# AdaptiveCity/deepdish

Hardware: AMD Instinct MI355X
Metric: end-to-end frames/sec (detect+encode+track) at 640x480 (higher is better)
Workload: dtype i8 (reference: uint8); encoder f16; 1 GPU; SSD-MobileNet-v1 uint8-quantised (300x300) + MARS-64x32x3 + deep_sort on synthetic 640x480 BGR frames, ~20 synthetic detections/frame (BASELINE.json configs[1]); streams_per_gpu=3072, worker_threads_per_gpu=2, parallelism=independent streams, 3072 per GPU in 2 worker groups, weights=seeded synthetic (seed 1234)

## Files before the change

### deepdish_amd/csrc/net_priv.h

```cpp
#pragma once
#include <map>
#include <utility>
#include <vector>
#include "common.h"

struct TensorDesc { int buf, h, w, c, cs, coff, dtype, pad; };

struct dd_net {
    dd_ctx *ctx = nullptr;
    int max_batch = 0;
    std::vector<int32_t> prog;
    std::vector<TensorDesc> tensors;
    std::vector<int64_t> buf_elems;
    std::vector<void *> bufs;
    std::vector<int> buf_dtype;
    int n_ops = 0, ops_off = 0;
    void *arena = nullptr;
    int64_t arena_bytes = 0;
    char *d_weights = nullptr;
    int64_t weight_bytes = 0;
    int in_h = 0, in_w = 0, out_tensor = -1;
    bool profile = false;
    int last_batch = 0;
    DevBuf slab;
    bool ssd_dec = false, yolo_dec = false;
    int dec_anchors = 0; float dec_thr = 0.f;
    float *d_anchors = nullptr, *dec_boxes = nullptr, *dec_score = nullptr, *dec_keys = nullptr; int *dec_cls = nullptr;
    bool slab_moved = false;
    _Float16 *d_zero = nullptr;
    bool use_glds = true;
    bool use_rw = true;
    int tile_mode = 0;
    std::vector<hipEvent_t> events;
    std::vector<int32_t> op_launch;
    std::vector<int32_t> op_variant;
    struct GraphEntry { int calls = 0; hipGraph_t graph = nullptr; hipGraphExec_t exec = nullptr; };
    bool use_graph = false;
    std::map<std::pair<const void *, int>, GraphEntry> graphs;
};

int netq_run_op(dd_net *net, int op_index, const int32_t *o, const uint8_t *input, int nimg, hipStream_t s, int *handled);
int netq_run_front(dd_net *net, const int32_t *o0, const int32_t *o1, const int32_t *o2, const uint8_t *input, int nimg, hipStream_t s, int *ran);
int netq_run_mid(dd_net *net, const int32_t *o3, const int32_t *o4, int nimg, hipStream_t s, int *ran);
int netq_prepare(dd_net *net);
```

### deepdish_amd/csrc/nets.hip

```cpp
#include <algorithm>
#include <cmath>
#include <cstdlib>
#include <map>
#include <string>
#include "common.h"
#include "ssd_dev.h"
#include "net_priv.h"
#include "mars_tail.h"

namespace {

typedef _Float16 h8 __attribute__((ext_vector_type(8)));
typedef _Float16 h4 __attribute__((ext_vector_type(4)));
typedef float f4 __attribute__((ext_vector_type(4)));

enum { OP_INPUT = 1, OP_CONV = 2, OP_DWCONV = 3, OP_MAXPOOL = 4, OP_UPSAMPLE = 5, OP_FC = 6, OP_L2NORM = 7, OP_STEM = 8, OP_DWPW = 9 };
enum { ACT_NONE = 0, ACT_RELU6 = 1, ACT_ELU = 2, ACT_SILU = 3, ACT_RELU = 4, ACT_SIGMOID = 5 };
enum { EPI_F16 = 0, EPI_F32 = 1, EPI_SSD_HEAD = 2, EPI_YOLO = 3 };
enum { OPK_DEFAULT = 0, OPK_FOLDED = 1, OPK_POOL_ROWS = 2, OPK_POOL_ROWS_STEM = 3, OPK_RES_UNIT = 4, OPK_SSD_FRONT = 5, OPK_C64_ROWS = 6, OPK_S2_ROWS = 7, OPK_CONV_WS = 8, OPK_WS_DW = 9, OPK_DWPW_ROWS = 10, OPK_SSD_HEAD_DEC = 11, OPK_RES_PAIR = 12, OPK_YOLO_HEAD_DEC = 13, OPK_MARS_WS = 14, OPK_FOLDED_PREV = 15, OPK_MARS_PAIR = 16, OPK_C64_STRIPS = 18, OPK_Q_FRONT = 19, OPK_Q_MID = 20, OPK_STEM_WIDE = 23 };
enum { DT_F16 = 0, DT_F32 = 1, DT_U8 = 2 };

constexpr int OP_WORDS = 48;
constexpr int TENSOR_WORDS = 8;

// ... 3972 lines not shown
                         int64_t n_weight_bytes, int max_batch, dd_net **out) {
    return net_create(ctx, program_host, n_words, weights_host, n_weight_bytes, max_batch, out, true);
}

static int net_create(dd_ctx *ctx, const int32_t *program_host, int n_words, const void *weights_host,
                      int64_t n_weight_bytes, int max_batch, dd_net **out, bool share) {
    DD_REQUIRE(ctx && program_host && weights_host && out && max_batch > 0 && n_words >= 8, DD_E_ARG,
               "dd_net_create: bad argument");
    DD_REQUIRE(program_host[0] == 0x314E4444, DD_E_ARG, "dd_net_create: bad program magic");
    const int nt = program_host[1], nb = program_host[2], no = program_host[3];
    DD_REQUIRE(n_words == 8 + nt * TENSOR_WORDS + nb * 2 + no * OP_WORDS, DD_E_ARG, "dd_net_create: program size mismatch");
    dd_net *n = new dd_net();
    struct Guard { dd_net *n; ~Guard() { if (n) (void)dd_net_destroy(n); } } guard{n};
    n->ctx = ctx;
    n->max_batch = max_batch;
    n->prog.assign(program_host, program_host + n_words);
    n->in_h = program_host[4];
    n->in_w = program_host[5];
    n->out_tensor = program_host[6];
    const int32_t *p = program_host + 8;
    for (int i = 0; i < nt; ++i, p += TENSOR_WORDS) n->tensors.push_back(TensorDesc{p[0], p[1], p[2], p[3], p[4], p[5], p[6], p[7]});
    DD_HIP(hipSetDevice(ctx->device));
    if (share) {
        const int32_t *ops = p + (size_t)nb * 2;
        std::vector<int> first(nb, -1), last(nb, -1);
        for (int t = 0; t < nt; ++t) DD_REQUIRE(n->tensors[t].buf >= 0 && n->tensors[t].buf < nb, DD_E_ARG, "dd_net_create_shared: tensor %d names buffer %d of %d", t, n->tensors[t].buf, nb);
        for (int i = 0; i < no; ++i)
            DD_REQUIRE((ops + (size_t)i * OP_WORDS)[0] < 16, DD_E_ARG, "dd_net_create_shared: uint8 programs keep one buffer per tensor (their borders are set once)");
        std::vector<int> gs(no), ge(no);
        for (int i = 0; i < no;) {
            int j = i;
            while (j + 1 < no && (ops + (size_t)j * OP_WORDS)[30] != 0) ++j;
            for (int k = i; k <= j; ++k) { gs[k] = i; ge[k] = j; }
            i = j + 1;
        }
        auto touch2 = [&](int t, int i) {
            if (t < 0 || t >= nt) return;
            const int b = n->tensors[t].buf;
            first[b] = first[b] < 0 ? gs[i] : std::min(first[b], gs[i]);
            last[b] = std::max(last[b], ge[i]);
        };
        for (int i = 0; i < no; ++i) {
            const int32_t *o = ops + (size_t)i * OP_WORDS;
            touch2(o[1], i); touch2(o[2], i); touch2(o[3], i); touch2(o[4], i);
        }
        if (n->out_tensor >= 0) last[n->tensors[n->out_tensor].buf] = no;
        std::vector<size_t> bytes(nb), off(nb, 0);
        size_t arena = 0;
        std::vector<int> order(nb);
        for (int b = 0; b < nb; ++b) { order[b] = b; bytes[b] = ((size_t)p[2 * b] * max_batch * dtype_size(p[2 * b + 1] & 0xff) + 256 + 255) & ~(size_t)255; }
        std::stable_sort(order.begin(), order.end(), [&](int a, int b) { return first[a] < first[b]; });
        std::vector<int> placed;
        for (int b : order) {
            if (first[b] < 0) { first[b] = 0; last[b] = no; }
            size_t at = 0;
            for (bool moved = true; moved;) {
                moved = false;
                for (int q : placed)
                    if (!(last[q] < first[b] || last[b] < first[q]) && at < off[q] + bytes[q] && off[q] < at + bytes[b]) { at = off[q] + bytes[q]; moved = true; }
            }
            off[b] = at;
            arena = std::max(arena, at + bytes[b]);
            placed.push_back(b);
        }
        DD_HIP(hipMalloc(&n->arena, arena));
        DD_HIP(hipMemset(n->arena, 0, arena));
        n->arena_bytes = (int64_t)arena;
        for (int i = 0; i < nb; ++i, p += 2) {
            n->buf_elems.push_back(p[0]);
            n->buf_dtype.push_back(p[1] & 0xff);
            n->bufs.push_back(static_cast<char *>(n->arena) + off[i]);
        }
    } else
    for (int i = 0; i < nb; ++i, p += 2) {
        n->buf_elems.push_back(p[0]);
        n->buf_dtype.push_back(p[1] & 0xff);
        void *d = nullptr;
        const size_t bytes = (size_t)p[0] * max_batch * dtype_size(p[1] & 0xff) + 256;
        DD_HIP(hipMalloc(&d, bytes));
        DD_HIP(hipMemset(d, (p[1] >> 8) & 0xff, bytes));
        n->bufs.push_back(d);
    }
    n->n_ops = no;
    n->ops_off = (int)(p - program_host);
    {
        size_t need = 0;
        for (int i = 0; i < no; ++i) {
            const int32_t *o = p + (size_t)i * OP_WORDS;
            if (o[0] != OP_CONV) continue;
            const int bk = o[28] == 32 ? 32 : 64, sk = conv_splitk(o[26], o[27], o[12], o[13] / bk, max_batch);
            if (sk > 1) need = std::max(need, (size_t)sk * max_batch * o[26] * o[27] * o[12] * sizeof(float));
        }
        if (need) { const int rc = n->slab.reserve(need); if (rc != DD_OK) return rc; }
    }
    n->weight_bytes = n_weight_bytes;
    DD_HIP(hipMalloc(&n->d_zero, 256));
    DD_HIP(hipMemset(n->d_zero, 0, 256));
    n->use_glds = getenv("DD_NO_GLDS") == nullptr;
    n->use_rw = getenv("DD_NO_RW") == nullptr;
    n->tile_mode = getenv("DD_TILE_MODE") ? atoi(getenv("DD_TILE_MODE")) : 0;
    DD_HIP(hipMalloc(&n->d_weights, (size_t)n_weight_bytes + 256));
    DD_HIP(hipMemcpy(n->d_weights, weights_host, (size_t)n_weight_bytes, hipMemcpyHostToDevice));
    guard.n = nullptr;
    *out = n;
    return DD_OK;
}

int dd_net_destroy(dd_net *n) {
    if (!n) return DD_OK;
    if (n->arena) (void)hipFree(n->arena);
    else for (void *b : n->bufs) (void)hipFree(b);
    for (hipEvent_t e : n->events) (void)hipEventDestroy(e);
    net_drop_graphs(n);
    n->slab.release();
    (void)hipFree(n->d_zero);
    (void)hipFree(n->d_weights);
    for (void *q : {(void *)n->d_anchors, (void *)n->dec_boxes, (void *)n->dec_score, (void *)n->dec_keys, (void *)n->dec_cls}) (void)hipFree(q);
    delete n;
    return DD_OK;
}

int dd_net_activation_bytes(dd_net *n, int64_t *out_host) {
    DD_REQUIRE(n && out_host, DD_E_ARG, "dd_net_activation_bytes: NULL argument");
    if (n->arena) { *out_host = n->arena_bytes; return DD_OK; }
    int64_t tot = 0;
    for (size_t i = 0; i < n->bufs.size(); ++i) tot += n->buf_elems[i] * n->max_batch * (int64_t)dtype_size(n->buf_dtype[i]) + 256;
    *out_host = tot;
    return DD_OK;
}

int dd_net_last_batch(dd_net *n, int *out_host) {
    DD_REQUIRE(n && out_host, DD_E_ARG, "dd_net_last_batch: NULL argument");
    *out_host = n->last_batch;
    return DD_OK;
}

int dd_net_input_size(dd_net *n, int *h_host, int *w_host) {
    DD_REQUIRE(n && h_host && w_host, DD_E_ARG, "dd_net_input_size: NULL argument");
    *h_host = n->in_h; *w_host = n->in_w;
    return DD_OK;
}

int dd_net_max_batch(dd_net *n, int *out_host) {
    DD_REQUIRE(n && out_host, DD_E_ARG, "dd_net_max_batch: NULL argument");
    *out_host = n->max_batch;
    return DD_OK;
}

int dd_net_output(dd_net *n, int tensor, void **dev_ptr, int *h, int *w, int *c, int *cs, int *dtype) {
    DD_REQUIRE(n, DD_E_ARG, "dd_net_output: NULL net");
    const int t = tensor < 0 ? n->out_tensor : tensor;
    DD_REQUIRE(t >= 0 && t < (int)n->tensors.size(), DD_E_ARG, "dd_net_output: tensor %d out of range", t);
    const TensorDesc &d = n->tensors[t];
    if (dev_ptr) *dev_ptr = static_cast<char *>(n->bufs[d.buf]) + (size_t)d.coff * dtype_size(d.dtype);
    if (h) *h = d.h;
    if (w) *w = d.w;
    if (c) *c = d.c;
    if (cs) *cs = d.cs;
    if (dtype) *dtype = d.dtype;
    return DD_OK;
}

int dd_net_profile(dd_net *n, int enable) {
    DD_REQUIRE(n, DD_E_ARG, "dd_net_profile: NULL net");
    DD_DEVICE(n->ctx);
    if (enable && n->events.empty()) {
        n->events.resize(n->n_ops + 2);
        for (auto &e : n->events) DD_HIP(hipEventCreate(&e));
    }
    n->profile = enable != 0;
    return DD_OK;
}

int dd_net_profile_read(dd_net *n, float *ms_host, int cap, int *n_ops_host) {
    DD_REQUIRE(n && ms_host && n_ops_host, DD_E_ARG, "dd_net_profile_read: NULL argument");
    DD_DEVICE(n->ctx);
    DD_REQUIRE(n->profile && !n->events.empty(), DD_E_STATE, "dd_net_profile_read: profiling is off");
    DD_REQUIRE(cap >= n->n_ops, DD_E_ARG, "dd_net_profile_read: cap %d < %d ops", cap, n->n_ops);
    DD_HIP(hipEventSynchronize(n->events[n->n_ops + 1]));
    float empty = 0.f;
    DD_HIP(hipEventElapsedTime(&empty, n->events[n->n_ops], n->events[n->n_ops + 1]));
    for (int i = 0; i < n->n_ops; ++i) {
        DD_HIP(hipEventElapsedTime(&ms_host[i], n->events[i], n->events[i + 1]));
        ms_host[i] = ms_host[i] > empty ? ms_host[i] - empty : 0.f;
    }
    *n_ops_host = n->n_ops;
    return DD_OK;
}

int dd_net_op_launches(dd_net *n, int32_t *codes_host, int cap, int *n_ops_host) {
    DD_REQUIRE(n && codes_host && n_ops_host, DD_E_ARG, "dd_net_op_launches: NULL argument");
    DD_REQUIRE(cap >= n->n_ops, DD_E_ARG, "dd_net_op_launches: cap %d < %d ops", cap, n->n_ops);
    for (int i = 0; i < n->n_ops; ++i) codes_host[i] = i < (int)n->op_launch.size() ? n->op_launch[i] : OPK_DEFAULT;
    *n_ops_host = n->n_ops;
    return DD_OK;
}

int dd_net_op_variants(dd_net *n, int32_t *codes_host, int cap, int *n_ops_host) {
    DD_REQUIRE(n && codes_host && n_ops_host, DD_E_ARG, "dd_net_op_variants: NULL argument");
    DD_REQUIRE(cap >= n->n_ops, DD_E_ARG, "dd_net_op_variants: cap %d < %d ops", cap, n->n_ops);
    for (int i = 0; i < n->n_ops; ++i) codes_host[i] = i < (int)n->op_variant.size() ? n->op_variant[i] : 0;
    *n_ops_host = n->n_ops;
    return DD_OK;
}

int dd_net_read(dd_net *n, int tensor, int n_img, void *dst, int dst_on_device, void *stream) {
    DD_REQUIRE(n && dst && n_img >= 0 && n_img <= n->max_batch, DD_E_ARG, "dd_net_read: bad argument");
    DD_DEVICE(n->ctx);
    const int t = tensor < 0 ? n->out_tensor : tensor;
    DD_REQUIRE(t >= 0 && t < (int)n->tensors.size(), DD_E_ARG, "dd_net_read: tensor %d out of range", t);
    const TensorDesc &d = n->tensors[t];
    DD_REQUIRE(!n->arena || t == n->out_tensor, DD_E_STATE, "dd_net_read: tensor %d of an engine whose buffers share memory by lifetime "
               "(dd_net_create_shared): only the output tensor outlives the forward", t);
    DD_REQUIRE(d.coff == 0, DD_E_ARG, "dd_net_read: tensor %d is a channel slice", t);
    for (int i = 0; i < n->n_ops && i < (int)n->op_launch.size(); ++i) {
        const int32_t *o = n->prog.data() + n->ops_off + (size_t)i * OP_WORDS;
        DD_REQUIRE(!(o[2] == t && n->op_launch[i] == OPK_SSD_HEAD_DEC), DD_E_STATE,
                   "dd_net_read: tensor %d (the SSD head matrix) was not written: the head layers decoded in their epilogue "
                   "(dd_net_ssd_decode); read dd_net_ssd_decoded instead", t);
        DD_REQUIRE(!(o[2] == t && n->op_launch[i] == OPK_YOLO_HEAD_DEC), DD_E_STATE,
                   "dd_net_read: tensor %d (the Detect matrix) was not written: the head layers reduced their rows in their epilogue "
                   "(dd_net_yolo_decode); read dd_net_yolo_decoded instead", t);
        DD_REQUIRE(!((o[2] == t || o[4] == t) && n->op_launch[i] == OPK_FOLDED), DD_E_STATE,
                   "dd_net_read: tensor %d was not written by the last forward (op %d ran inside the next op's launch at this batch "
                   "size and its output stayed on chip); run a smaller batch or a program compiled without the fusion flags", t, i);
    }
    hipStream_t s = dd_pick_stream(n->ctx, stream);
    const size_t bytes = d.pad ? (size_t)n_img * (d.h + 2) * (d.w + 2) * d.cs
                               : (size_t)n_img * d.h * d.w * d.cs * dtype_size(d.dtype);
    if (!bytes) return DD_OK;
    DD_HIP(hipMemcpyAsync(dst, n->bufs[d.buf], bytes, dst_on_device ? hipMemcpyDeviceToDevice : hipMemcpyDeviceToHost, s));
    if (!dst_on_device) DD_HIP(hipStreamSynchronize(s));
    return DD_OK;
}

static int net_run_ops(dd_net *net, const uint8_t *input, int nimg, hipStream_t s);

int dd_net_use_graph(dd_net *net, int enable) {
    DD_REQUIRE(net, DD_E_ARG, "dd_net_use_graph: NULL net");
    DD_DEVICE(net->ctx);
    net->use_graph = enable != 0;
    if (!net->use_graph) net_drop_graphs(net);
    return DD_OK;
}

int dd_net_ssd_decode(dd_net *net, const float *anchors_host, int n_anchors, float score_thr, int enable) {
    DD_REQUIRE(net, DD_E_ARG, "dd_net_ssd_decode: NULL net");
    DD_DEVICE(net->ctx);
    net_drop_graphs(net);
    if (!enable) { net->ssd_dec = false; return DD_OK; }
    DD_REQUIRE(anchors_host && n_anchors > 0, DD_E_ARG, "dd_net_ssd_decode: anchors missing");
    int heads = 0;
    for (int i = 0; i < net->n_ops; ++i) {
        const int32_t *o = net->prog.data() + net->ops_off + (size_t)i * OP_WORDS;
        if (o[0] == OP_CONV && o[15] == EPI_SSD_HEAD) {
            DD_REQUIRE(o[18] && o[21] == n_anchors && 4 + o[20] <= 96, DD_E_ARG,
                       "dd_net_ssd_decode: head op %d has no per-anchor weight copy, or %d anchors / %d classes do not fit", i, o[21], o[20]);
            ++heads;
        }
        if (o[0] == 20) {
            DD_REQUIRE(o[21] == n_anchors, DD_E_ARG, "dd_net_ssd_decode: the program decodes %d anchors, %d given", o[21], n_anchors);
            ++heads;
        }
    }
    DD_REQUIRE(heads > 0, DD_E_ARG, "dd_net_ssd_decode: the program has no SSD head");
    if (net->dec_anchors != n_anchors) {
        for (void *q : {(void *)net->d_anchors, (void *)net->dec_boxes, (void *)net->dec_score, (void *)net->dec_keys, (void *)net->dec_cls}) (void)hipFree(q);
        net->d_anchors = net->dec_boxes = net->dec_score = net->dec_keys = nullptr; net->dec_cls = nullptr; net->dec_anchors = 0;
        const size_t per = (size_t)net->max_batch * n_anchors;
        DD_HIP(hipMalloc(&net->d_anchors, (size_t)n_anchors * 4 * sizeof(float)));
        DD_HIP(hipMalloc(&net->dec_boxes, per * 4 * sizeof(float)));
        DD_HIP(hipMalloc(&net->dec_score, per * sizeof(float)));
        DD_HIP(hipMalloc(&net->dec_keys, per * sizeof(float)));
        DD_HIP(hipMalloc(&net->dec_cls, per * sizeof(int)));
        net->dec_anchors = n_anchors;
    }
    DD_HIP(hipMemcpy(net->d_anchors, anchors_host, (size_t)n_anchors * 4 * sizeof(float), hipMemcpyHostToDevice));
    net->dec_thr = score_thr;
    net->ssd_dec = true;
    return DD_OK;
}

int dd_net_yolo_decode(dd_net *net, int enable) {
    DD_REQUIRE(net, DD_E_ARG, "dd_net_yolo_decode: NULL net");
    DD_DEVICE(net->ctx);
    net_drop_graphs(net);
    if (!enable) { net->yolo_dec = false; return DD_OK; }
    DD_REQUIRE(!net->ssd_dec, DD_E_STATE, "dd_net_yolo_decode: the SSD decode is on for this network");
    int heads = 0, rows = 0;
    for (int i = 0; i < net->n_ops; ++i) {
        const int32_t *o = net->prog.data() + net->ops_off + (size_t)i * OP_WORDS;
        if (o[0] == OP_CONV && o[15] == EPI_YOLO) {
            DD_REQUIRE(o[18] && !o[19] && o[20] >= 6 && o[20] <= 96, DD_E_ARG,
                       "dd_net_yolo_decode: head op %d has no per-anchor weight copy, or %d columns per row do not fit", i, o[20]);
            DD_REQUIRE(rows == 0 || rows == o[21], DD_E_ARG, "dd_net_yolo_decode: heads disagree on the rows per image");
            rows = o[21];
            ++heads;
        }
    }
    DD_REQUIRE(heads > 0 && rows > 0, DD_E_ARG, "dd_net_yolo_decode: the program has no YOLOv5 Detect head");
    if (net->dec_anchors != rows || !net->dec_boxes) {
        for (void *q : {(void *)net->d_anchors, (void *)net->dec_boxes, (void *)net->dec_score, (void *)net->dec_keys, (void *)net->dec_cls}) (void)hipFree(q);
        net->d_anchors = net->dec_boxes = net->dec_score = net->dec_keys = nullptr; net->dec_cls = nullptr; net->dec_anchors = 0;
        const size_t per = (size_t)net->max_batch * rows;
        DD_HIP(hipMalloc(&net->dec_boxes, per * 4 * sizeof(float)));
        DD_HIP(hipMalloc(&net->dec_score, per * sizeof(float)));
        DD_HIP(hipMalloc(&net->dec_cls, per * sizeof(int)));
        net->dec_anchors = rows;
    }
    net->yolo_dec = true;
    return DD_OK;
}

int dd_net_yolo_decoded(dd_net *net, float **boxes, float **conf, int **classes, int *rows) {
    DD_REQUIRE(net && net->yolo_dec, DD_E_STATE, "dd_net_yolo_decoded: dd_net_yolo_decode is off");
    if (boxes) *boxes = net->dec_boxes;
    if (conf) *conf = net->dec_score;
    if (classes) *classes = net->dec_cls;
    if (rows) *rows = net->dec_anchors;
    return DD_OK;
}

int dd_net_yolo_decoded_read(dd_net *net, int n, float *boxes_host, float *conf_host, int *classes_host) {
    DD_REQUIRE(net && net->yolo_dec && n >= 0 && n <= net->max_batch, DD_E_STATE, "dd_net_yolo_decoded_read: decode is off or n out of range");
    DD_DEVICE(net->ctx);
    DD_HIP(hipStreamSynchronize(net->ctx->stream));
    const size_t per = (size_t)n * net->dec_anchors;
    if (boxes_host) DD_HIP(hipMemcpy(boxes_host, net->dec_boxes, per * 4 * sizeof(float), hipMemcpyDeviceToHost));
    if (conf_host) DD_HIP(hipMemcpy(conf_host, net->dec_score, per * sizeof(float), hipMemcpyDeviceToHost));
    if (classes_host) DD_HIP(hipMemcpy(classes_host, net->dec_cls, per * sizeof(int), hipMemcpyDeviceToHost));
    return DD_OK;
}


int dd_net_ssd_decoded(dd_net *net, float **boxes, float **scores, int **classes, float **keys) {
    DD_REQUIRE(net && net->ssd_dec, DD_E_STATE, "dd_net_ssd_decoded: dd_net_ssd_decode is off");
    if (boxes) *boxes = net->dec_boxes;
    if (scores) *scores = net->dec_score;
    if (classes) *classes = net->dec_cls;
    if (keys) *keys = net->dec_keys;
    return DD_OK;
}

int dd_net_ssd_heads_u8(dd_net *net, const uint8_t **box_q, const uint8_t **cls_q, int *cls_stride, const uint8_t **lut, float *quant4_host,
                        int *n_anchors, int *n_classes) {
    DD_REQUIRE(net && box_q && cls_q && cls_stride && lut && quant4_host && n_anchors && n_classes, DD_E_ARG, "dd_net_ssd_heads_u8: NULL argument");
    DD_REQUIRE(!net->arena, DD_E_STATE, "dd_net_ssd_heads_u8: the engine's buffers share memory by lifetime (dd_net_create_shared): the head "
               "tensors do not outlive the forward");
    for (int i = 0; i < net->n_ops; ++i) {
        const int32_t *o = net->prog.data() + net->ops_off + (size_t)i * OP_WORDS;
        if (o[0] != 20) continue;
        DD_REQUIRE(o[1] >= 0 && o[1] < (int)net->tensors.size() && o[3] >= 0 && o[3] < (int)net->tensors.size(), DD_E_ARG, "dd_net_ssd_heads_u8: head tensors out of range");
        const TensorDesc &tb = net->tensors[o[1]], &tc = net->tensors[o[3]];
        DD_REQUIRE(tb.cs == 4 && tb.h == o[21] && tc.h == o[21] && tb.w == 1 && tc.w == 1 && o[20] <= tc.cs && !tb.pad && !tc.pad && !tb.coff && !tc.coff, DD_E_ARG,
                   "dd_net_ssd_heads_u8: head tensors of %d anchors are not [anchors][4] / [anchors][>= %d] bytes", o[21], o[20]);
        *box_q = static_cast<const uint8_t *>(net->bufs[tb.buf]); *cls_q = static_cast<const uint8_t *>(net->bufs[tc.buf]);
        *cls_stride = tc.cs; *n_anchors = o[21]; *n_classes = o[20];
        *lut = reinterpret_cast<const uint8_t *>(net->d_weights + (size_t)(uint32_t)o[16]);
        const float *of = reinterpret_cast<const float *>(o);
        for (int q = 0; q < 4; ++q) quant4_host[q] = of[32 + q];
        return DD_OK;
    }
    DD_REQUIRE(false, DD_E_ARG, "dd_net_ssd_heads_u8: the program has no uint8 SSD head");
}

int dd_net_ssd_decoded_read(dd_net *net, int n, float *boxes_host, float *scores_host, int *classes_host, float *keys_host) {
    DD_REQUIRE(net && net->ssd_dec && n >= 0 && n <= net->max_batch, DD_E_STATE, "dd_net_ssd_decoded_read: decode is off or n out of range");
    DD_DEVICE(net->ctx);
    hipStream_t s = net->ctx->stream;
    DD_HIP(hipStreamSynchronize(s));
    const size_t per = (size_t)n * net->dec_anchors;
    if (!per) return DD_OK;
    if (boxes_host) DD_HIP(hipMemcpy(boxes_host, net->dec_boxes, per * 4 * sizeof(float), hipMemcpyDeviceToHost));
    if (scores_host) DD_HIP(hipMemcpy(scores_host, net->dec_score, per * sizeof(float), hipMemcpyDeviceToHost));
    if (classes_host) DD_HIP(hipMemcpy(classes_host, net->dec_cls, per * sizeof(int), hipMemcpyDeviceToHost));
    if (keys_host) DD_HIP(hipMemcpy(keys_host, net->dec_keys, per * sizeof(float), hipMemcpyDeviceToHost));
    return DD_OK;
}

int dd_net_forward(dd_net *net, const uint8_t *input, int nimg, void *stream) {
    DD_REQUIRE(net && input && nimg >= 0, DD_E_ARG, "dd_net_forward: bad argument");
    DD_DEVICE(net->ctx);
    DD_REQUIRE(nimg <= net->max_batch, DD_E_CAPACITY, "dd_net_forward: batch %d > max_batch %d", nimg, net->max_batch);
    if (nimg == 0) return DD_OK;
    net->last_batch = nimg;
    hipStream_t s = dd_pick_stream(net->ctx, stream);
    auto eager = [&]() -> int {
        const int rc = net_run_ops(net, input, nimg, s);
        if (net->slab_moved) { net->slab_moved = false; net_drop_graphs(net); }
        return rc;
    };
    if (!net->use_graph || net->profile) return eager();
    if (net->graphs.size() > 256) net_drop_graphs(net);
    dd_net::GraphEntry &g = net->graphs[std::make_pair(static_cast<const void *>(input), nimg)];
    if (g.exec) { DD_HIP(hipGraphLaunch(g.exec, s)); return DD_OK; }
    if (g.calls++ == 0) return eager();
    DD_HIP(hipStreamBeginCapture(s, hipStreamCaptureModeThreadLocal));
    const int rc = net_run_ops(net, input, nimg, s);
    hipGraph_t graph = nullptr;
    const hipError_t e = hipStreamEndCapture(s, &graph);
    if (rc != DD_OK) { if (graph) (void)hipGraphDestroy(graph); return rc; }
    DD_HIP(e);
    g.graph = graph;
    DD_HIP(hipGraphInstantiate(&g.exec, graph, nullptr, nullptr, 0));
    DD_HIP(hipGraphLaunch(g.exec, s));
    return DD_OK;
}

static int net_run_ops(dd_net *net, const uint8_t *input, int nimg, hipStream_t s) {
    auto base = [&](int t) -> char * {
        const TensorDesc &d = net->tensors[t];
        return static_cast<char *>(net->bufs[d.buf]);
    };
    net->op_launch.assign((size_t)net->n_ops, OPK_DEFAULT);
    net->op_variant.assign((size_t)net->n_ops, 0);
    ConvP stem_p;
    bool stem_pending = false;
    bool wide_pending = false, wide_ready = false;
    bool input_pending = false;
    float input_mean = 0.f, input_scale = 1.f;
    int input_op = -1;
    ConvP unit_a;
    bool unit_pending = false;
    ConvP pw_p;
    bool pw_pending = false;
    bool proj_done = false;
    MarsPairP pair64;
    bool pair64_first = false;
    int pair_left = 0;
    ConvP pair_a, pair_b;
    bool pair_pending = false;
    int pair_op = -1;
    auto flush_pair = [&]() -> int {
        pair_pending = false;
        net->op_launch[pair_op] = OPK_RES_UNIT;
        return launch_res_unit(s, pair_a, pair_b, nimg, net->ctx->device);
    };
    auto run_ws = [&](ConvP &P) { return P.cin == 256 ? launch_conv_ws<4>(s, P, net->ctx->device) : launch_conv_ws<8>(s, P, net->ctx->device); };
    int first_op = 0;
    bool mid_on = false;
    {
        static const int chunk_env = getenv("DD_Q_FRONT_CHUNK") ? atoi(getenv("DD_Q_FRONT_CHUNK")) : 0;
        auto opw = [&](int k) { return net->prog.data() + net->ops_off + (size_t)k * OP_WORDS; };
        const char *front_env = getenv("DD_Q_FRONT"), *front_min_env = getenv("DD_Q_FRONT_MIN");
        const int front_min = front_min_env ? atoi(front_min_env) : 24;
        {
            const char *mid_env = getenv("DD_Q_MID");
            mid_on = !(mid_env && atoi(mid_env) == 0) && nimg >= front_min;
        }
        if (!(front_env && atoi(front_env) == 0) && chunk_env <= 0 && nimg >= front_min && net->n_ops > 3 && opw(0)[0] == 16 && opw(1)[0] == 19 && opw(2)[0] == 19) {
            if (net->profile) for (int k = 0; k < 3; ++k) DD_HIP(hipEventRecord(net->events[k], s));
            int ran = 0;
            const int rc = netq_run_front(net, opw(0), opw(1), opw(2), input, nimg, s, &ran);
            if (rc != DD_OK) return rc;
            if (ran) { first_op = 3; net->op_launch[0] = OPK_FOLDED; net->op_launch[1] = OPK_FOLDED; net->op_launch[2] = OPK_Q_FRONT; }
        }
        if (first_op == 0 && chunk_env > 0 && nimg > chunk_env && net->n_ops > 3 && opw(0)[0] == 16 && opw(1)[0] == 19 && opw(2)[0] == 19 && opw(1)[1] == opw(0)[2] && opw(2)[1] == opw(1)[2]) {
            const TensorDesc &t2 = net->tensors[opw(2)[2]];
            const size_t img_out = (size_t)(t2.h + 2) * (t2.w + 2) * t2.cs;
            void *&out_buf = net->bufs[t2.buf];
            void *const out_base = out_buf;
            if (net->profile) for (int k = 0; k < 3; ++k) DD_HIP(hipEventRecord(net->events[k], s));
            for (int c0 = 0; c0 < nimg; c0 += chunk_env) {
                const int nc = std::min(chunk_env, nimg - c0);
                out_buf = static_cast<char *>(out_base) + (size_t)c0 * img_out;
                for (int k = 0; k < 3; ++k) {
                    int handled = 0;
                    const int rc = netq_run_op(net, k, opw(k), input + (size_t)c0 * net->in_h * net->in_w * 3, nc, s, &handled);
                    if (rc != DD_OK || !handled) { out_buf = out_base; return rc != DD_OK ? rc : DD_E_ARG; }
                }
            }
            out_buf = out_base;
            first_op = 3;
        }
    }
    for (int i = first_op; i < net->n_ops; ++i) {
        if (net->profile) DD_HIP(hipEventRecord(net->events[i], s));
        const int32_t *o = net->prog.data() + net->ops_off + (size_t)i * OP_WORDS;
        const float *of = reinterpret_cast<const float *>(o);
        const int kind = o[0], src = o[1], dst = o[2], res = o[3], dst2 = o[4];
        const TensorDesc *ts = src >= 0 ? &net->tensors[src] : nullptr;
        const TensorDesc *td = dst >= 0 ? &net->tensors[dst] : nullptr;
        DD_REQUIRE(!input_pending || (kind == OP_CONV && i == input_op + 1), DD_E_STATE, "dd_net_forward: input op %d was folded into an op that did not take it", input_op);
        if (mid_on && kind == 19 && i + 1 < net->n_ops && net->prog[net->ops_off + (size_t)(i + 1) * OP_WORDS] == 19) {
            const int32_t *o4 = net->prog.data() + net->ops_off + (size_t)(i + 1) * OP_WORDS;
            if (net->profile) DD_HIP(hipEventRecord(net->events[i + 1], s));
            int ran = 0;
            const int rc = netq_run_mid(net, o, o4, nimg, s, &ran);
            if (rc != DD_OK) return rc;
            if (ran) { net->op_launch[i] = OPK_FOLDED; net->op_launch[i + 1] = OPK_Q_MID; ++i; continue; }
        }
        DD_REQUIRE((!wide_pending || kind == OP_CONV) && (!wide_ready || kind == OP_MAXPOOL), DD_E_STATE, "dd_net_forward: op %d does not take the first layer folded into it", i);
        if (pair_pending && kind != OP_CONV) { const int rc = flush_pair(); if (rc != DD_OK) return rc; }
        if (pw_pending && kind != OP_DWCONV) {
            pw_pending = false; net->op_launch[i - 1] = OPK_CONV_WS;
            const int rc = run_ws(pw_p);
            if (rc != DD_OK) return rc;
        }
        if (unit_pending && kind != OP_CONV) {
            unit_pending = false; net->op_launch[i - 1] = OPK_DEFAULT;
            const int rc = launch_conv3x3_rw(s, unit_a, nimg, false, net->ctx->device);
            if (rc != DD_OK) return rc;
        }
        if (stem_pending && !(kind == OP_CONV && o[29]) && kind != OP_DWPW) {
            stem_pending = false; net->op_launch[i - 1] = OPK_DEFAULT;
            const int rc = launch_stem(s, stem_p, nimg);
            if (rc != DD_OK) return rc;
        }
        switch (kind) {
            case OP_INPUT: {
                const int s2d = o[5];
                const int m = nimg * td->h * td->w;
                if (s2d && o[30] && !o[6] && td->cs == 32 && !td->coff && i + 1 < net->n_ops && net->use_rw) {
// ... 403 lines not shown
```

### deepdish_amd/csrc/netsq.hip

```cpp
#include <algorithm>
#include <atomic>
#include <cstdlib>
#include <type_traits>
#include "common.h"
#include "ssd_dev.h"
#include "net_priv.h"
#include "netsq_dev.h"

namespace {


struct QConvP {
    const uint8_t *in; int H, W, c16_in;
    int kh, kw, stride, off_y, off_x;
    int ho, wo, m;
    const i4v *w;
    const int *cbias;
    int kc_per_tap, n_mfrag, mq;
    uint8_t *out; int epi;
    int Ho, Wo, c16_out;
    long long img_bytes_out; int row_bytes, base_off, cout_store;
    int zwc;
    unsigned hw_magic, wo_magic;
    QReq R;
// ... 264 lines not shown
        if (__builtin_amdgcn_ballot_w64(col < 0 || col + 2 >= P.W) != 0ull) {
#pragma unroll
            for (int i = 0; i < 3; ++i) {
                const bool in = col + i >= 0 && col + i < P.W;
                if (!in) {
#pragma unroll
                    for (int b = 3 * i; b < 3 * i + 3; ++b) {
                        const unsigned msk = 0xffu << (8 * (b & 3));
                        d[b >> 2] = (d[b >> 2] & ~msk) | (zp4 & msk);
                    }
                }
            }
        }
        i4v b;
        b[0] = (int)(d[0] ^ 0x80808080u); b[1] = (int)(d[1] ^ 0x80808080u); b[2] = (int)(d[2] ^ 0x80808080u); b[3] = 0;
        int rs = 0;
        if constexpr (!HL) {
            if (fq == 3) { b[0] = 0; b[1] = 0; b[2] = 0; }
            rs = sdot4(b[0], 0x01010101, sdot4(b[1], 0x01010101, sdot4(b[2] & 0xff, 0x01010101, 0)));
            rs += __shfl_xor(rs, 16, 64);
            rs += __shfl_xor(rs, 32, 64);
            rs *= P.zwc;
        }
        i4v acc0 = {0, 0, 0, 0}, acc1 = acc0;
        acc0 = __builtin_amdgcn_mfma_i32_16x16x64_i8(wa, b, acc0, 0, 0, 0);
        acc1 = __builtin_amdgcn_mfma_i32_16x16x64_i8(wb, b, acc1, 0, 0, 0);
        if constexpr (HL) {
            acc0 = __builtin_amdgcn_mfma_i32_16x16x64_i8(wal, b, acc0, 0, 0, 0);
            acc1 = __builtin_amdgcn_mfma_i32_16x16x64_i8(wbl, b, acc1, 0, 0, 0);
        }
        const unsigned lo = q_requant_pack4<SAT>(acc0[0] + rs, acc0[1] + rs, acc0[2] + rs, acc0[3] + rs, M0, CQ[0], CQ[1], CQ[2], CQ[3], sh0, lo0, hi0);
        const unsigned hi = q_requant_pack4<SAT>(acc1[0] + rs, acc1[1] + rs, acc1[2] + rs, acc1[3] + rs, M0, CQ[4], CQ[5], CQ[6], CQ[7], sh0, lo0, hi0);
        typedef unsigned u2v __attribute__((ext_vector_type(2)));
        __builtin_amdgcn_raw_buffer_store_b64(u2v{lo ^ 0x80808080u, hi ^ 0x80808080u}, rdst, (int)so[j], 0, 0);
    }
}

struct QDwP {
    const uint8_t *in; int H, W, c16;
    int stride, off_y, off_x, ho, wo;
    const short *w;
    const int *cbias;
    uint8_t *out;
    long long total;
    QReq R;
};

__global__ __launch_bounds__(256) void q_dw_k(const QDwP P) {
    const long long it = (long long)blockIdx.x * 256 + threadIdx.x;
    if (it >= P.total) return;
    const int x = (int)(it % P.wo);
    long long t = it / P.wo;
    const int pl = (int)(t % P.c16); t /= P.c16;
    const int y = (int)(t % P.ho), n = (int)(t / P.ho);
    const size_t PP = (size_t)(P.W + 2) * 16, RP = PP * P.c16;
    const uint8_t *src = P.in + ((size_t)n * (P.H + 2) + y * P.stride + P.off_y) * RP + (size_t)pl * PP + (size_t)(x * P.stride + P.off_x) * 16;
    int acc[16];
    const i4v *cb = reinterpret_cast<const i4v *>(P.cbias + pl * 16);
#pragma unroll
    for (int i = 0; i < 4; ++i) { const i4v c = cb[i]; acc[4 * i] = c[0]; acc[4 * i + 1] = c[1]; acc[4 * i + 2] = c[2]; acc[4 * i + 3] = c[3]; }
    const int C = P.c16 * 16;
#pragma unroll
    for (int dy = 0; dy < 3; ++dy)
#pragma unroll
        for (int dx = 0; dx < 3; ++dx) {
            const u4v a = *reinterpret_cast<const u4v *>(src + (size_t)dy * RP + (size_t)dx * 16);
            const short *wt = P.w + (size_t)(dy * 3 + dx) * C + pl * 16;
#pragma unroll
            for (int i = 0; i < 16; ++i) acc[i] += ((int)(a[i >> 2] << (24 - 8 * (i & 3))) >> 24) * (int)wt[i];
        }
    u4v o;
#pragma unroll
    for (int d = 0; d < 4; ++d) {
        unsigned wv = 0;
#pragma unroll
        for (int r = 0; r < 4; ++r) wv |= (unsigned)q_requant(acc[4 * d + r], P.R) << (8 * r);
        o[d] = wv ^ 0x80808080u;
    }
    uint8_t *dst = P.out + (((size_t)n * (P.ho + 2) + y + 1) * P.c16 + pl) * ((size_t)(P.wo + 2) * 16) + (size_t)(x + 1) * 16;
    *reinterpret_cast<u4v *>(dst) = o;
}

struct QDwmP {
    const uint8_t *in; int H, W, c16;
    int stride, off_y, off_x, ho, wo, m;
    const uint2 *dw_a; const int *dw_cb;
    uint8_t *out;
    unsigned hw_magic, wo_magic, c16_magic;
    QReq R;
};

template <bool SAT>
__global__ __launch_bounds__(256) void q_dwm_k(const QDwmP P, const int n_items) {
    const int lane = threadIdx.x & 63, wave = threadIdx.x >> 6;
    const int fr = lane & 15, fq = lane >> 4;
    const int item = blockIdx.x * 4 + wave;
    if (item >= n_items) return;
    const int fg = P.hw_magic ? (int)__umulhi((unsigned)item, P.c16_magic) : item / P.c16, cg = item - fg * P.c16;
    const unsigned PP = (unsigned)(P.W + 2) * 16u, RP = PP * (unsigned)P.c16, PPo = (unsigned)(P.wo + 2) * 16u;
    const uint2 ab = P.dw_a[cg * 64 + lane];
    const i4v cbv = *reinterpret_cast<const i4v *>(P.dw_cb + cg * 16 + 4 * fq);
    unsigned dmask[4];
#pragma unroll
    for (int d = 0; d < 4; ++d) dmask[d] = (fr >> 2) == d ? 0xffu << (8 * (fr & 3)) : 0u;
    const uint8_t *src[4]; uint8_t *dst[4]; bool live[4];
    const int hw = P.ho * P.wo;
#pragma unroll
    for (int f = 0; f < 4; ++f) {
        int q = (fg * 4 + f) * 16 + fr;
        live[f] = q < P.m;
        q = min(q, P.m - 1);
        int n, y;
        if (P.hw_magic) { n = (int)__umulhi((unsigned)q, P.hw_magic); y = (int)__umulhi((unsigned)(q - n * hw), P.wo_magic); }
        else { n = q / hw; y = (q - n * hw) / P.wo; }
        const int r = q - n * hw, x = r - y * P.wo;
        src[f] = P.in + (size_t)((unsigned)(n * (P.H + 2) + y * P.stride + P.off_y) * RP + (unsigned)cg * PP + (unsigned)(x * P.stride + P.off_x) * 16u);
        dst[f] = P.out + (size_t)((unsigned)((n * (P.ho + 2) + y + 1) * P.c16 + cg) * PPo + (unsigned)(x + 1) * 16u + 4u * (unsigned)fq);
    }
    i4v acc[4];
#pragma unroll
    for (int f = 0; f < 4; ++f) acc[f] = cbv;
    i4v b[3][4];
#pragma unroll
    for (int ks = 0; ks < 3; ++ks) {
        const int tp = min(4 * ks + fq, 8);
        const unsigned to = (unsigned)(tp / 3) * RP + (unsigned)(tp % 3) * 16u;
#pragma unroll
        for (int f = 0; f < 4; ++f) b[ks][f] = *reinterpret_cast<const i4v *>(src[f] + to);
    }
#pragma unroll
    for (int ks = 0; ks < 3; ++ks) {
        const unsigned sel = 0x01010101u * (unsigned)ks;
        const unsigned rh = __builtin_amdgcn_perm(ab.x, ab.x, sel), rl = __builtin_amdgcn_perm(ab.y, ab.y, sel);
        i4v Ah, Al;
#pragma unroll
        for (int d = 0; d < 4; ++d) { Ah[d] = (int)(rh & dmask[d]); Al[d] = (int)(rl & dmask[d]); }
#pragma unroll
        for (int f = 0; f < 4; ++f) acc[f] = __builtin_amdgcn_mfma_i32_16x16x64_i8(Ah, b[ks][f], acc[f], 0, 0, 0);
#pragma unroll
        for (int f = 0; f < 4; ++f) acc[f] = __builtin_amdgcn_mfma_i32_16x16x64_i8(Al, b[ks][f], acc[f], 0, 0, 0);
    }
    const int M = P.R.M, sh = P.R.e - 1, lo = P.R.lo, hi = P.R.hi;
    const long long C = P.R.C;
#pragma unroll
    for (int f = 0; f < 4; ++f) {
        const unsigned packed = 0x80808080u ^ q_requant_pack4<SAT ? 1 : 0>(acc[f][0], acc[f][1], acc[f][2], acc[f][3], M, C, C, C, C, sh, lo, hi);
        if (live[f]) *reinterpret_cast<unsigned *>(dst[f]) = packed;
    }
}

struct QDecP {
    const uint8_t *box, *cls;
    int n_anchors, n_classes, cls_stride;
    const uint8_t *lut;
    float box_scale, box_zp, sc_scale, sc_zp, thr;
    const float *anchors;
    float *boxes, *score, *keys; int *cls_out;
};

__global__ __launch_bounds__(256) void q_ssd_decode_k(const QDecP P) {
    __shared__ uint8_t lut[256];
    lut[threadIdx.x] = P.lut[threadIdx.x];
    __syncthreads();
    const int a = (blockIdx.x * 256 + threadIdx.x) >> 3, sub = threadIdx.x & 7;
    const size_t z = blockIdx.y;
    const bool live = a < P.n_anchors;
    const uint8_t *c = P.cls + (z * P.n_anchors + (live ? a : 0)) * P.cls_stride;
    int best = -1, bi = 0x7fffffff;
    if (sub * 16 < P.n_classes) {
        const u4v v = *reinterpret_cast<const u4v *>(c + sub * 16);
#pragma unroll
        for (int i = 0; i < 16; ++i) {
            const int k = sub * 16 + i;
            const int q = lut[(v[i >> 2] >> (8 * (i & 3))) & 0xffu];
            if (k >= 1 && k < P.n_classes && q > best) { best = q; bi = k - 1; }
        }
    }
#pragma unroll
    for (int o = 4; o > 0; o >>= 1) {
        const int ob = __shfl_xor(best, o, 64), oi = __shfl_xor(bi, o, 64);
        if (ob > best || (ob == best && oi < bi)) { best = ob; bi = oi; }
    }
    if (live && sub == 0) {
#pragma clang fp contract(off)
        const uint8_t *b = P.box + (z * P.n_anchors + a) * 4;
        float r[4], an[4], bx[4];
#pragma unroll
        for (int q = 0; q < 4; ++q) { r[q] = P.box_scale * ((float)b[q] - P.box_zp); an[q] = P.anchors[a * 4 + q]; }
        (void)ssddev::decode_anchor(r, an, 0.f, bx);
        const float sc = P.sc_scale * ((float)best - P.sc_zp);
        const size_t o = z * P.n_anchors + a;
#pragma unroll
        for (int q = 0; q < 4; ++q) P.boxes[o * 4 + q] = bx[q];
        P.score[o] = sc;
        P.cls_out[o] = bi;
        P.keys[o] = sc >= P.thr ? sc : -1.f;
    }
}

struct QDwpwP {
    const uint8_t *in; int H, W;
    int off_y, off_x, ho, wo, hw, tiles_per_frame;
    uint8_t *out; int c16_out;
    const uint2 *dw_a;
    const long long *dw_cq;
    const i4v *w;
    const i4v *w2;
    const int *cbias;
    const long long *cq;
    int zwc, NR;
    int dup;
    unsigned wo_magic, nr_magic, tpf_magic;
    unsigned long long *dbg;
    QReq Rd, Rp;
};

constexpr int QT = 64;

template <int CIN, int COUT, int WP, int STRIDE, int LPT, bool ROWSUM, int MW = 4, int SAT = 0, bool HL = false, int QTT = QT>
__global__ __launch_bounds__((COUT / (16 * MW)) * WP * 64, (COUT / (16 * MW)) * WP <= 2 ? 3 : QTT > 64 ? 4 : 2) void q_dwpw_k(const QDwpwP P, const int n_tiles, const int tiles_per_block) {
    constexpr int WM = COUT / (16 * MW), NW = WM * WP, NT = NW * 64;
    static_assert(MW == 4 || MW == 2, "fragments per wave");
    static_assert(!(HL && ROWSUM), "the split filter needs no row sums");
    constexpr int KC = (CIN + 63) / 64, CINP = KC * 64, C16 = CIN / 16;
    constexpr int FPT = QTT / 16, UNITS = C16 * (FPT / 4);
    static_assert(QTT % 64 == 0 && UNITS % NW == 0, "depthwise units over waves");
    constexpr int CPW = UNITS / NW;
    static_assert(FPT == 4 || CPW == 1, "several units per wave: one fragment quad only");
    constexpr bool KEEP = CPW <= 2, FOLDP = !ROWSUM && KC <= 4 && QTT == 64;
    extern __shared__ __attribute__((aligned(16))) uint8_t smem[];
    const int tid = threadIdx.x, lane = tid & 63, wave = __builtin_amdgcn_readfirstlane(tid >> 6);
    const int fr = lane & 15, fq = lane >> 4;
    const int wm = wave / WP, wp = wave % WP;
    const int RB = (P.W + 2) * CIN, PP = (P.W + 2) * 16;
    uint8_t *opnd = smem;
    int *rowsum = reinterpret_cast<int *>(opnd + QTT * CINP);
    i4v *pinfo = reinterpret_cast<i4v *>(rowsum + 2 * QTT);
    int *cbl = reinterpret_cast<int *>(pinfo + 2 * QTT);
    uint2 *dwa_l = reinterpret_cast<uint2 *>(cbl + COUT);
    long long *dwq_l = reinterpret_cast<long long *>(dwa_l + (KEEP ? 0 : C16 * 64));
    uint8_t *ring = reinterpret_cast<uint8_t *>(dwq_l + (KEEP ? 0 : CIN));

    i4v Wr[MW][KC];
#pragma unroll
    for (int m = 0; m < MW; ++m)
#pragma unroll
        for (int kc = 0; kc < KC; ++kc) Wr[m][kc] = P.w[((size_t)(wm * MW + m) * KC + kc) * 64 + lane];
    const int mg = (wm * MW) / 4, m0 = (wm * MW) % 4;
    unsigned wlm = 0;
    int kcl = -1;
    i4v Wl1[HL ? MW : 1];
    if constexpr (HL) {
#pragma unroll
        for (int kc = 0; kc < KC; ++kc) {
            int any = 0;
#pragma unroll
            for (int m = 0; m < MW; ++m) {
                const i4v w = P.w2[((size_t)(wm * MW + m) * KC + kc) * 64 + lane];
                any |= w[0] | w[1] | w[2] | w[3];
            }
            if (__builtin_amdgcn_ballot_w64(any != 0) != 0ull) { wlm |= 1u << kc; if (kcl < 0) kcl = kc; }
        }
#pragma unroll
        for (int m = 0; m < MW; ++m) Wl1[m] = P.w2[((size_t)(wm * MW + m) * KC + max(kcl, 0)) * 64 + lane];
    }
    long long CP[FOLDP ? MW : 1][4];
    if constexpr (FOLDP) {
#pragma unroll
        for (int m = 0; m < MW; ++m)
#pragma unroll
            for (int r = 0; r < 4; ++r) CP[m][r] = P.cq[64 * mg + 16 * fq + 4 * (m0 + m) + r];
    } else {
        for (int i = tid; i < COUT; i += NT) cbl[i] = P.cbias[i];
    }
    if constexpr (!KEEP) {
        for (int i = tid; i < C16 * 64; i += NT) dwa_l[i] = P.dw_a[i];
        for (int i = tid; i < CIN; i += NT) dwq_l[i] = P.dw_cq[i];
    }
    if (CIN < CINP) for (int i = tid; i < QTT * CINP / 16; i += NT) reinterpret_cast<u4v *>(opnd)[i] = u4v{0, 0, 0, 0};
    for (int i = tid; i < 2 * QTT; i += NT) rowsum[i] = 0;
    unsigned dmask[4];
#pragma unroll
    for (int d = 0; d < 4; ++d) dmask[d] = (fr >> 2) == d ? 0xffu << (8 * (fr & 3)) : 0u;
    int tap_dx[3];
#pragma unroll
    for (int ks = 0; ks < 3; ++ks) tap_dx[ks] = (min(4 * ks + fq, 8) % 3) * 16;
    const bool row_up0 = fq == 3, row_up1 = fq >= 2;
    auto build_a = [&](int cg, i4v (&Ah)[3], unsigned &lo_w, long long (&Cq)[4], unsigned &lom) {
        const uint2 ab = P.dw_a[cg * 64 + lane];
        lo_w = ab.y;
        lom = (unsigned)__builtin_amdgcn_readfirstlane((int)(ab.y >> 24));
#pragma unroll
        for (int ks = 0; ks < 3; ++ks) {
            const unsigned rh = __builtin_amdgcn_perm(ab.x, ab.x, 0x01010101u * (unsigned)ks);
#pragma unroll
            for (int d = 0; d < 4; ++d) Ah[ks][d] = (int)(rh & dmask[d]);
        }
#pragma unroll
        for (int r = 0; r < 4; ++r) Cq[r] = P.dw_cq[cg * 16 + 4 * fq + r];
    };
    i4v KAh[KEEP ? CPW : 1][3];
    long long KCq[KEEP ? CPW : 1][4];
    unsigned Klom[KEEP ? CPW : 1] = {}, Klow[KEEP ? CPW : 1] = {};
    if constexpr (KEEP) {
#pragma unroll
        for (int ci = 0; ci < CPW; ++ci) build_a((wave * CPW + ci) % C16, KAh[ci], Klow[ci], KCq[ci], Klom[ci]);
    }

    const int t_begin = blockIdx.x * tiles_per_block, t_end = min(n_tiles, t_begin + tiles_per_block);
    if (t_begin >= t_end) return;
    const int Md = P.Rd.M, shd = P.Rd.e - 1, Mp = P.Rp.M, shp = P.Rp.e - 1;
    const long long Cp = P.Rp.C;
    const int lod = P.Rd.lo, hid = P.Rd.hi, lop = P.Rp.lo, hip_ = P.Rp.hi;
    const int out_row = P.c16_out * ((P.wo + 2) * 16);
    const unsigned ring_bytes = (unsigned)P.NR * (unsigned)RB;

    auto tile_rows = [&](int t, int &n, int &q0, int &q1, int &ga, int &gb) {
        n = (int)__umulhi((unsigned)t, P.tpf_magic);
        q0 = (t - n * P.tiles_per_frame) * QTT;
// ... 295 lines not shown
        const int cur = t & 1;
        dw_planes(cur, cur);
        Q_STAMP(0);
        __builtin_amdgcn_s_waitcnt(0xc07f);
        __builtin_amdgcn_s_barrier();
        Q_STAMP(1);
        pf_issue(max(lo, e_hi + 1), hi);
        if (tid < QTT) {
            if (ROWSUM) rowsum[(cur ^ 1) * QTT + tid] = 0;
            if (t + 1 < t_end) geometry(n2, q02, q12, ga2, cur ^ 1);
        }
        matrix(q0, q1, cur, cur);
        Q_STAMP(2);
        {
            const int nf_t = (q1 - q0) / 16 + 1, ns = nf_t > wp ? (nf_t - wp + WP - 1) / WP : 0;
            if (ns >= 4) __builtin_amdgcn_s_waitcnt(0x0f74);
            else if (ns == 3) __builtin_amdgcn_s_waitcnt(0x0f73);
            else if (ns == 2) __builtin_amdgcn_s_waitcnt(0x0f72);
            else if (ns == 1) __builtin_amdgcn_s_waitcnt(0x0f71);
            else __builtin_amdgcn_s_waitcnt(0x0f70);
        }
        Q_STAMP(3);
        __builtin_amdgcn_s_waitcnt(0xc07f);
        __builtin_amdgcn_s_barrier();
        Q_STAMP(4);
        n = n2; q0 = q02; q1 = q12; ga = ga2;
    }
#undef Q_STAMP
    if (P.dbg && lane == 0) for (int k = 0; k < 5; ++k) P.dbg[((size_t)blockIdx.x * NW + wave) * 8 + k] = st[k];
}



enum { QV_CONV = 1, QV_PWS = 2, QV_DW = 3, QV_DWM = 4, QV_DWPW = 5, QV_CONV0 = 6, QV_ADD = 7, QV_DECODE = 8 };

void dwpw_plan(int H, int W, int ho, int wo, int stride, int off_y, int cin, int nt, int qt, int *NR, int *lpt) {
    const int hw = ho * wo, tpf = dd_ceil_div(hw, qt), RB = (W + 2) * cin;
    int span = 0, hi = 0, mx = 0;
    for (int n = 0; n < 2; ++n)
        for (int k = 0; k < tpf; ++k) {
            const int q0 = k * qt, q1 = std::min(q0 + qt, hw) - 1;
            const int ga = n * (H + 2) + (q0 / wo) * stride + off_y, gb = n * (H + 2) + (q1 / wo) * stride + off_y + 2;
            span = std::max(span, gb - ga + 1);
            if (n || k) { const int lo = std::max(hi + 1, ga); mx = std::max(mx, gb - lo + 1); }
            hi = std::max(hi, gb);
        }
    *NR = span;
    *lpt = (int)(((long long)mx * RB + (long long)nt * 16 - 1) / ((long long)nt * 16));
}

template <int CIN, int COUT, int WP, int STRIDE, int LPT, int EXTRA = 0, int MW = 4, int QTT = QT>
int launch_q_dwpw(hipStream_t s, QDwpwP &P, int nimg, int device, bool *ok, bool dry = false, int *variant = nullptr, bool dry_split = false) {
    constexpr int NW = (COUT / (16 * MW)) * WP, NT = NW * 64, CINP = (CIN + 63) / 64 * 64;
    int lpt = 0;
    P.tiles_per_frame = dd_ceil_div(P.hw, QTT);
    dwpw_plan(P.H, P.W, P.ho, P.wo, STRIDE, P.off_y, CIN, NT, QTT, &P.NR, &lpt);
    static const int extra_env = getenv("DD_Q_EXTRA") ? atoi(getenv("DD_Q_EXTRA")) : -1;
    P.NR += extra_env >= 0 ? extra_env : EXTRA;
    const int RB = (P.W + 2) * CIN;
    constexpr bool KEEP = ((CIN / 16) * (QTT / 64)) / NW <= 2;
    const size_t lds = (size_t)P.NR * RB + (size_t)QTT * CINP + (size_t)2 * QTT * sizeof(int) + 2 * QTT * 16 + COUT * sizeof(int) + (KEEP ? 0 : (CIN / 16) * 64 * 8 + CIN * 8);
    P.wo_magic = (unsigned)((1ull << 32) / (unsigned)P.wo) + 1u;
    P.nr_magic = (unsigned)((1ull << 32) / (unsigned)P.NR) + 1u;
    P.tpf_magic = (unsigned)((1ull << 32) / (unsigned)P.tiles_per_frame) + 1u;
    const long long lim24 = 1ll << 23;
    *ok = (long long)nimg * P.tiles_per_frame * P.tiles_per_frame < (1ll << 32) && (long long)P.hw * P.wo < (1ll << 32) &&
          (long long)(nimg + 1) * (P.H + 2) * P.NR < (1ll << 32) && lpt <= LPT && lds <= 160 * 1024 && (long long)LPT * NT * 16 + (long long)P.NR * RB < (1ll << 32) &&
          RB < lim24 && (long long)P.c16_out * (P.wo + 2) * 16 < lim24 && (long long)(nimg + 1) * (P.ho + 2) < lim24 && P.hw < lim24;
    if (!*ok) return DD_OK;
    constexpr bool CAN_HL = CIN <= 128;
    const bool hl = dry ? dry_split : P.w2 != nullptr;
    if (hl && !CAN_HL) { *ok = false; return DD_OK; }
    if (dry) return DD_OK;
    const bool rsum = P.zwc != 0 && !hl;
    const int sat = P.Rd.lo == 0 && P.Rd.hi == 255 && P.Rp.lo == 0 && P.Rp.hi == 255 ? (P.Rd.e <= 8 && P.Rp.e <= 8 ? 2 : 1) : 0;
#define DD_QK(R_, S_, H_) q_dwpw_k<CIN, COUT, WP, STRIDE, LPT, R_, MW, S_, (H_) && CAN_HL, QTT>
#define DD_QS(R_, H_) (sat == 2 ? &DD_QK(R_, 2, H_) : sat == 1 ? &DD_QK(R_, 1, H_) : &DD_QK(R_, 0, H_))
    void (*kern)(const QDwpwP, const int, const int) = hl ? DD_QS(false, true) : rsum ? DD_QS(true, false) : DD_QS(false, false);
    if (variant) *variant = QV_DWPW | (CIN / 32) << 4 | (COUT / 64) << 9 | STRIDE << 13 | (QTT / 64) << 15 | (hl ? 2 : rsum ? 1 : P.dup ? 3 : 0) << 17 | sat << 19;
    static DevOnce once;
    const int rc = once.run(device, [&]() -> int {
        for (const void *f : {reinterpret_cast<const void *>(&DD_QK(false, 0, true)), reinterpret_cast<const void *>(&DD_QK(false, 1, true)), reinterpret_cast<const void *>(&DD_QK(false, 2, true)),
                              reinterpret_cast<const void *>(&DD_QK(true, 0, false)), reinterpret_cast<const void *>(&DD_QK(true, 1, false)), reinterpret_cast<const void *>(&DD_QK(true, 2, false)),
                              reinterpret_cast<const void *>(&DD_QK(false, 0, false)), reinterpret_cast<const void *>(&DD_QK(false, 1, false)), reinterpret_cast<const void *>(&DD_QK(false, 2, false))})
            DD_HIP(hipFuncSetAttribute(f, hipFuncAttributeMaxDynamicSharedMemorySize, 160 * 1024));
        return DD_OK;
    });
#undef DD_QS
#undef DD_QK
    if (rc != DD_OK) return rc;
    static std::atomic<int> per_cu_cache[64];
    int per_cu = per_cu_cache[device & 63].load(std::memory_order_relaxed);
    if (per_cu == 0) {
        int nb = 0;
        DD_HIP(hipOccupancyMaxActiveBlocksPerMultiprocessor(&nb, reinterpret_cast<const void *>(kern), NT, lds));
        per_cu = std::max(1, std::min(8, nb));
        per_cu_cache[device & 63].store(per_cu, std::memory_order_relaxed);
    }
    static const int per_cu_env = getenv("DD_Q_PER_CU") ? atoi(getenv("DD_Q_PER_CU")) : 0;
    if (per_cu_env > 0) per_cu = std::min(per_cu, per_cu_env);
    const int n_tiles = nimg * P.tiles_per_frame;
    const int blocks = std::min(n_tiles, per_cu * 256);
    const int tpb = dd_ceil_div(n_tiles, blocks);
    const dim3 grid((unsigned)dd_ceil_div(n_tiles, tpb));
    static const bool stamps = getenv("DD_Q_STAMPS") && atoi(getenv("DD_Q_STAMPS")) != 0;
    const size_t n_st = (size_t)grid.x * NW * 8;
    if (stamps) { DD_HIP(hipMalloc(&P.dbg, n_st * 8)); DD_HIP(hipMemsetAsync(P.dbg, 0, n_st * 8, s)); }
    hipLaunchKernelGGL(kern, grid, dim3(NT), lds, s, P, n_tiles, tpb);
    DD_LAUNCH_CHECK();
    if (stamps) {
        std::vector<unsigned long long> h(n_st);
        DD_HIP(hipStreamSynchronize(s));
        DD_HIP(hipMemcpy(h.data(), P.dbg, n_st * 8, hipMemcpyDeviceToHost));
        DD_HIP(hipFree(P.dbg));
        double sum[5] = {0, 0, 0, 0, 0};
        for (size_t w = 0; w < n_st / 8; ++w) for (int k = 0; k < 5; ++k) sum[k] += (double)h[w * 8 + k];
        const double nw = (double)(n_st / 8) * tpb;
        fprintf(stderr, "q_dwpw_k<%d,%d,%d> %d blocks/CU %d tiles/block: cycles per wave and tile: depthwise %.0f  barrier A %.0f  matrix stage %.0f  ring write %.0f  barrier B %.0f\n",
                CIN, COUT, STRIDE, per_cu, tpb, sum[0] / nw, sum[1] / nw, sum[2] / nw, sum[3] / nw, sum[4] / nw);
    }
    return DD_OK;
}

int dwpw_dispatch(hipStream_t s, QDwpwP &Q, int nc, int dev, int cin, int cout, int stride, bool *ok, bool dry, int *variant, bool dry_split = false) {
    static const int qt128 = getenv("DD_Q_QT128") ? atoi(getenv("DD_Q_QT128")) : 1;
    *ok = false;
#define DD_QB(CIN_, COUT_, WP_, S_, LPT_) launch_q_dwpw<CIN_, COUT_, WP_, S_, LPT_>(s, Q, nc, dev, ok, dry, variant, dry_split)
    if (cin == 32 && cout == 64 && stride == 1) return qt128 ? launch_q_dwpw<32, 64, 4, 1, 6, 0, 4, 128>(s, Q, nc, dev, ok, dry, variant, dry_split) : DD_QB(32, 64, 2, 1, 8);
    if (cin == 64 && cout == 128 && stride == 2) return DD_QB(64, 128, 2, 2, 8);
    if (cin == 128 && cout == 128 && stride == 1) return DD_QB(128, 128, 2, 1, 8);
    if (cin == 128 && cout == 256 && stride == 2) return DD_QB(128, 256, 2, 2, 8);
    if (cin == 256 && cout == 256 && stride == 1) return DD_QB(256, 256, 2, 1, 6);
    if (cin == 256 && cout == 512 && stride == 2) return DD_QB(256, 512, 1, 2, 12);
    if (cin == 512 && cout == 512 && stride == 1) return DD_QB(512, 512, 1, 1, 8);
#undef DD_QB
    return DD_OK;
}

struct QPwsP {
    const uint8_t *in; int H, W, c16_in;
    int hw, m;
    const i4v *w;
    const int *cbias;
    const long long *cq;
    int n_mfrag, frags_per_group;
    uint8_t *out; int c16_out;
    long long img_bytes_out; int row_bytes, base_off, cout_store;
    int zwc, tiles_per_block;
    unsigned hw_magic, w_magic;
    QReq R;
    int n_frag_a;
    uint8_t *out_b; long long img_bytes_b; int row_bytes_b, base_off_b, cout_store_b, zwc_b;
    QReq Rb;
};

template <int K, int MW, int EPI, bool ROWSUM, int SAT>
__global__ __launch_bounds__(512, 2) void q_pws_k(const QPwsP P, const int n_tiles) {
    constexpr int KC = K / 64, C16 = K / 16;
    static_assert(MW * KC * 4 <= 128, "the wave's filter is 128 registers at most");
    extern __shared__ __attribute__((aligned(16))) uint8_t smem[];
    uint8_t *opnd = smem;
    unsigned *psrc = reinterpret_cast<unsigned *>(smem + 2 * QT * K);
    unsigned *pdst = psrc + 4 * QT;
    int *rowsum = reinterpret_cast<int *>(pdst + 4 * QT);
    unsigned *pdstb = reinterpret_cast<unsigned *>(rowsum + 3 * QT);
    const int tid = threadIdx.x, lane = tid & 63, wave = __builtin_amdgcn_readfirstlane(tid >> 6), NW = blockDim.x >> 6;
    const int fr = lane & 15, fq = lane >> 4;
    const int frag0 = blockIdx.y * P.frags_per_group + wave * MW;
    const unsigned PP = (unsigned)(P.W + 2) * 16u;

    i4v Wr[MW][KC];
#pragma unroll
    for (int m = 0; m < MW; ++m)
#pragma unroll
        for (int kc = 0; kc < KC; ++kc) Wr[m][kc] = frag0 + m < P.n_mfrag ? P.w[((size_t)(frag0 + m) * KC + kc) * 64 + lane] : i4v{0, 0, 0, 0};
    const int M = P.R.M, sh = P.R.e - 1, lo = P.R.lo, hi = P.R.hi;
    const int mg = frag0 / 4, m0 = frag0 % 4;
    long long CQ[MW][4];
#pragma unroll
    for (int m = 0; m < MW; ++m)
#pragma unroll
        for (int r = 0; r < 4; ++r) {
            const int ch = EPI == QEPI_Q16 ? 64 * mg + 16 * fq + 4 * (m0 + m) + r : 16 * (frag0 + m) + 4 * fq + r;
            CQ[m][r] = frag0 + m < P.n_mfrag ? P.cq[ch] : 0ll;
        }
    const int nfa = EPI == QEPI_ROWS && P.n_frag_a ? P.n_frag_a : P.n_mfrag;
    bool hb[MW]; int chm[MW], Mm[MW], em[MW], k1m[MW], zwm[MW];
    int n_store_m = 0;
#pragma unroll
    for (int m = 0; m < MW; ++m) {
        hb[m] = frag0 + m >= nfa;
        chm[m] = 16 * (frag0 + m - (hb[m] ? nfa : 0));
        const QReq &Rm = hb[m] ? P.Rb : P.R;
        Mm[m] = Rm.M; em[m] = Rm.e; k1m[m] = (1 << (Rm.e - 1)) + (Rm.zo << Rm.e); zwm[m] = hb[m] ? P.zwc_b : P.zwc;
        n_store_m += frag0 + m < P.n_mfrag && chm[m] < (hb[m] ? P.cout_store_b : P.cout_store) ? 1 : 0;
    }

    const int t_begin = blockIdx.x * P.tiles_per_block, t_end = min(n_tiles, t_begin + P.tiles_per_block);
    if (t_begin >= t_end) return;
    auto geometry = [&](int t) {
        const int q = t * QT + tid, qc = min(q, P.m - 1);
        const int n = (int)__umulhi((unsigned)qc, P.hw_magic), r = qc - n * P.hw;
        const int y = (int)__umulhi((unsigned)r, P.w_magic), x = r - y * P.W;
        const unsigned row = (unsigned)(n * (P.H + 2) + y + 1);
        psrc[(t & 3) * QT + tid] = row * (unsigned)P.c16_in * PP + (unsigned)(x + 1) * 16u;
        unsigned d;
        if constexpr (EPI == QEPI_Q16) d = row * (unsigned)P.c16_out * PP + (unsigned)(x + 1) * 16u;
        else d = (unsigned)((long long)n * P.img_bytes_out) + (unsigned)P.base_off + (unsigned)r * (unsigned)P.row_bytes;
        pdst[(t & 3) * QT + tid] = q < P.m ? d : 0xffffffffu;
        if (EPI == QEPI_ROWS && P.n_frag_a) pdstb[(t & 3) * QT + tid] = q < P.m ? (unsigned)((long long)n * P.img_bytes_b) + (unsigned)P.base_off_b + (unsigned)r * (unsigned)P.row_bytes_b : 0xffffffffu;
    };
    auto fill = [&](int t) {
        const uint8_t *src = P.in + psrc[(t & 3) * QT + lane];
        uint8_t *dst = opnd + (size_t)(t & 1) * QT * K;
        for (int c = wave; c < C16; c += NW) {
            unsigned keep;
            const unsigned l = (unsigned)__builtin_amdgcn_readfirstlane((int)(unsigned)(uintptr_t)(const __attribute__((address_space(3))) uint8_t *)(dst + (size_t)c * QT * 16));
            const uint8_t *g = src + (size_t)c * PP;
            asm volatile("s_mov_b32 %0, m0\n\ts_mov_b32 m0, %2\n\ts_nop 0\n\tglobal_load_lds_dwordx4 %1, off\n\ts_mov_b32 m0, %0"
                         : "=&s"(keep) : "v"(g), "s"(l) : "memory");
        }
    };

    auto own_rowsum = [&](int t, int slot) {
        const uint8_t *ob = opnd + (size_t)(t & 1) * QT * K;
        int a = 0;
        for (int c = wave; c < C16; c += NW) {
            const i4v v = *reinterpret_cast<const i4v *>(ob + ((size_t)c * QT + lane) * 16);
#pragma unroll
            for (int d = 0; d < 4; ++d) a = sdot4(v[d], 0x01010101, a);
        }
        atomicAdd(&rowsum[slot * QT + lane], a);
    };
    auto wait_landed = [&](int ns) {
        switch (ns) {
#define DD_VMCNT(N_) case N_: __builtin_amdgcn_s_waitcnt(0x0f70 | ((N_) & 15) | (((N_) >> 4) << 14)); break;
            DD_VMCNT(1) DD_VMCNT(2) DD_VMCNT(3) DD_VMCNT(4) DD_VMCNT(5) DD_VMCNT(6) DD_VMCNT(7) DD_VMCNT(8)
            DD_VMCNT(9) DD_VMCNT(10) DD_VMCNT(11) DD_VMCNT(12) DD_VMCNT(13) DD_VMCNT(14) DD_VMCNT(15) DD_VMCNT(16)
#undef DD_VMCNT
            default: __builtin_amdgcn_s_waitcnt(0x0f70);
        }
    };
    if (tid < QT) { geometry(t_begin); if (t_begin + 1 < t_end) geometry(t_begin + 1); }
    for (int i = tid; i < 3 * QT; i += blockDim.x) rowsum[i] = 0;
    __syncthreads();
    fill(t_begin);
    wait_landed(0);
    int slot = 0;
    if constexpr (ROWSUM) own_rowsum(t_begin, 0);
    int ns_prev = 0;
    for (int t = t_begin; t < t_end; ++t) {
        __builtin_amdgcn_s_waitcnt(0xc07f);
        __builtin_amdgcn_s_barrier();
        if (t + 1 < t_end) fill(t + 1);
        if (t + 2 < t_end && tid < QT) geometry(t + 2);
        const int slot1 = slot == 2 ? 0 : slot + 1, slot2 = slot1 == 2 ? 0 : slot1 + 1;
        if (ROWSUM && tid < QT) rowsum[slot2 * QT + tid] = 0;
        const uint8_t *ob = opnd + (size_t)(t & 1) * QT * K;
        const int nf = (min((t + 1) * QT, P.m) - t * QT + 15) / 16;
        constexpr int KB = KC < 4 ? KC : 4;
        i4v b[KB];
        {
            const uint8_t *bp = ob + ((size_t)fq * QT + fr) * 16;
#pragma unroll
            for (int kc = 0; kc < KB; ++kc) b[kc] = *reinterpret_cast<const i4v *>(bp + (size_t)kc * 4 * QT * 16);
        }
        ns_prev = 0;
        for (int f = 0; f < nf; ++f) {
            i4v acc[MW];
#pragma unroll
            for (int m = 0; m < MW; ++m) acc[m] = i4v{0, 0, 0, 0};
            const uint8_t *bp = ob + ((size_t)fq * QT + 16 * f + fr) * 16;
#pragma unroll
            for (int k0 = 0; k0 < KC; k0 += KB) {
#pragma unroll
                for (int kc = 0; kc < KB; ++kc) {
#pragma unroll
                    for (int m = 0; m < MW; ++m) acc[m] = __builtin_amdgcn_mfma_i32_16x16x64_i8(Wr[m][k0 + kc], b[kc], acc[m], 0, 0, 0);
                }
                if (k0 + KB < KC) {
#pragma unroll
                    for (int kc = 0; kc < KB; ++kc) b[kc] = *reinterpret_cast<const i4v *>(bp + (size_t)(k0 + KB + kc) * 4 * QT * 16);
                }
            }
            if (f + 1 < nf) {
                const uint8_t *bn = ob + ((size_t)fq * QT + 16 * (f + 1) + fr) * 16;
#pragma unroll
                for (int kc = 0; kc < KB; ++kc) b[kc] = *reinterpret_cast<const i4v *>(bn + (size_t)kc * 4 * QT * 16);
            }
            const int rsv = ROWSUM ? rowsum[slot * QT + 16 * f + fr] * P.zwc : 0;
            const unsigned po = pdst[(t & 3) * QT + 16 * f + fr];
            if constexpr (EPI == QEPI_Q16) {
                unsigned o[MW];
#pragma unroll
                for (int m = 0; m < MW; ++m)
                    o[m] = 0x80808080u ^ q_requant_pack4<SAT>(acc[m][0] + rsv, acc[m][1] + rsv, acc[m][2] + rsv, acc[m][3] + rsv, M, CQ[m][0], CQ[m][1], CQ[m][2], CQ[m][3], sh, lo, hi);
                if (po != 0xffffffffu && frag0 < P.n_mfrag) {
                    uint8_t *dst = P.out + po + (size_t)(4 * mg + fq) * PP + 4 * m0;
                    if constexpr (MW == 4) *reinterpret_cast<u4v *>(dst) = u4v{o[0], o[1], o[2], o[3]};
                    else *reinterpret_cast<uint2 *>(dst) = make_uint2(o[0], o[1]);
                }
                if (frag0 < P.n_mfrag) ++ns_prev;
            } else {
                const int rs0 = ROWSUM ? rowsum[slot * QT + 16 * f + fr] : 0;
                const unsigned pob = P.n_frag_a ? pdstb[(t & 3) * QT + 16 * f + fr] : 0xffffffffu;
#pragma unroll
                for (int m = 0; m < MW; ++m) {
                    const int ch = chm[m] + 4 * fq;
                    if (frag0 + m >= P.n_mfrag || ch >= (hb[m] ? P.cout_store_b : P.cout_store)) continue;
                    const int rv = rs0 * zwm[m];
                    const unsigned wv = q_requant_linear_pack4(acc[m][0] + rv, acc[m][1] + rv, acc[m][2] + rv, acc[m][3] + rv, Mm[m], CQ[m][0], CQ[m][1], CQ[m][2], CQ[m][3], em[m], k1m[m]);
                    const unsigned pm = hb[m] ? pob : po;
                    if (pm != 0xffffffffu) *reinterpret_cast<unsigned *>((hb[m] ? P.out_b : P.out) + pm + ch) = wv;
                }
                ns_prev += n_store_m;
            }
        }
        if (t + 1 < t_end) {
            wait_landed(ns_prev);
            if constexpr (ROWSUM) own_rowsum(t + 1, slot1);
        }
        slot = slot1;
    }
}

template <int K, int MW>
int launch_q_pws(hipStream_t s, QPwsP &P, int nimg, int device, bool *ok, int *variant) {
    const int n_tiles = dd_ceil_div(P.m, QT);
    const int waves = std::min(8, dd_ceil_div(P.n_mfrag, MW));
    const int groups = dd_ceil_div(P.n_mfrag, waves * MW);
    const int wpb = dd_ceil_div(dd_ceil_div(P.n_mfrag, groups), MW);
    P.frags_per_group = wpb * MW;
    const size_t lds = (size_t)2 * QT * K + 15 * QT * sizeof(unsigned);
    const int blocks_x = std::max(1, std::min(n_tiles, 256 / groups));
    P.tiles_per_block = dd_ceil_div(n_tiles, blocks_x);
    P.hw_magic = (unsigned)((1ull << 32) / (unsigned)P.hw) + 1u;
    P.w_magic = (unsigned)((1ull << 32) / (unsigned)P.W) + 1u;
    const long long in_bytes = (long long)nimg * (P.H + 2) * P.c16_in * (P.W + 2) * 16;
    const long long out_bytes = P.img_bytes_out ? (long long)nimg * P.img_bytes_out : (long long)nimg * (P.H + 2) * P.c16_out * (P.W + 2) * 16;
    *ok = in_bytes < (1ll << 32) && out_bytes < (1ll << 32) && (long long)P.m * P.hw < (1ll << 32) && (long long)P.hw * P.W < (1ll << 32) && P.zwc >= -128 && P.zwc <= 128 &&
          lds <= 160 * 1024 && wpb >= 1 && wpb <= 8;
    if (!*ok) return DD_OK;
    const bool rsum = P.zwc != 0 || (P.n_frag_a && P.zwc_b != 0);
    const bool rows = P.img_bytes_out != 0;
    if (P.n_frag_a && !(P.Rb.linear && P.Rb.e >= 1 && P.Rb.e <= 30 && P.Rb.lo == 0 && P.Rb.hi == 255 && std::abs(P.Rb.zo) < 256 && P.zwc_b >= -128 && P.zwc_b <= 128 &&
                        (long long)nimg * P.img_bytes_b < (1ll << 32))) { *ok = false; return DD_OK; }
    if (rows && !(P.R.linear && P.R.e >= 1 && P.R.e <= 30 && P.R.lo == 0 && P.R.hi == 255 && std::abs(P.R.zo) < 256)) { *ok = false; return DD_OK; }
    const int sat = !rows && P.R.lo == 0 && P.R.hi == 255 ? (P.R.e <= 8 ? 2 : 1) : 0;
    void (*kern)(const QPwsP, const int) = nullptr;
#define DD_PW(E_, R_, S_) q_pws_k<K, MW, E_, R_, S_>
    if (rows) kern = rsum ? &DD_PW(QEPI_ROWS, true, 0) : &DD_PW(QEPI_ROWS, false, 0);
    else if constexpr (MW != 3) {
        if (sat == 2) kern = rsum ? &DD_PW(QEPI_Q16, true, 2) : &DD_PW(QEPI_Q16, false, 2);
        else if (sat == 1) kern = rsum ? &DD_PW(QEPI_Q16, true, 1) : &DD_PW(QEPI_Q16, false, 1);
        else kern = rsum ? &DD_PW(QEPI_Q16, true, 0) : &DD_PW(QEPI_Q16, false, 0);
    }
    if (!kern) { *ok = false; return DD_OK; }
    *variant = QV_PWS | (K / 512) << 4 | MW << 6 | (rows ? QEPI_ROWS : QEPI_Q16) << 9 | (int)rsum << 11 | sat << 12 | (P.n_frag_a ? 1 : 0) << 14;
    static DevOnce once;
    const int rc = once.run(device, [&]() -> int {
        DD_HIP(hipFuncSetAttribute(reinterpret_cast<const void *>(&DD_PW(QEPI_ROWS, true, 0)), hipFuncAttributeMaxDynamicSharedMemorySize, 160 * 1024));
        DD_HIP(hipFuncSetAttribute(reinterpret_cast<const void *>(&DD_PW(QEPI_ROWS, false, 0)), hipFuncAttributeMaxDynamicSharedMemorySize, 160 * 1024));
        if constexpr (MW != 3) {
            for (const void *f : {reinterpret_cast<const void *>(&DD_PW(QEPI_Q16, true, 2)), reinterpret_cast<const void *>(&DD_PW(QEPI_Q16, false, 2)),
                                  reinterpret_cast<const void *>(&DD_PW(QEPI_Q16, true, 1)), reinterpret_cast<const void *>(&DD_PW(QEPI_Q16, false, 1)),
                                  reinterpret_cast<const void *>(&DD_PW(QEPI_Q16, true, 0)), reinterpret_cast<const void *>(&DD_PW(QEPI_Q16, false, 0))})
                DD_HIP(hipFuncSetAttribute(f, hipFuncAttributeMaxDynamicSharedMemorySize, 160 * 1024));
        }
        return DD_OK;
    });
#undef DD_PW
    if (rc != DD_OK) return rc;
    hipLaunchKernelGGL(kern, dim3((unsigned)dd_ceil_div(n_tiles, P.tiles_per_block), (unsigned)groups), dim3((unsigned)wpb * 64), lds, s, P, n_tiles);
    DD_LAUNCH_CHECK();
    return DD_OK;
}

struct QAddP {
    const uint8_t *a, *b; uint8_t *out;
    int H, W, c16, n_items;
    QAdd A;
};

__global__ __launch_bounds__(256) void q_add_k(const QAddP P) {
    const int it = blockIdx.x * 256 + threadIdx.x;
    if (it >= P.n_items) return;
    const unsigned u = (unsigned)it, w = (unsigned)P.W, c = (unsigned)P.c16, h = (unsigned)P.H;
    const unsigned x = u % w, q1 = u / w, p = q1 % c, q2 = q1 / c, y = q2 % h, n = q2 / h;
    const size_t off = (((size_t)n * (P.H + 2) + y + 1) * P.c16 + p) * (size_t)(P.W + 2) * 16 + (size_t)(x + 1) * 16;
    const u4v a = *reinterpret_cast<const u4v *>(P.a + off), b = *reinterpret_cast<const u4v *>(P.b + off);
    u4v o;
#pragma unroll
    for (int d = 0; d < 4; ++d) {
        const unsigned av = a[d] ^ 0x80808080u, bv = b[d] ^ 0x80808080u;
        unsigned wv = 0;
#pragma unroll
        for (int r = 0; r < 4; ++r) wv |= (unsigned)q_add_u8((int)((av >> (8 * r)) & 0xffu), (int)((bv >> (8 * r)) & 0xffu), P.A) << (8 * r);
        o[d] = wv ^ 0x80808080u;
    }
    *reinterpret_cast<u4v *>(P.out + off) = o;
}

}

int netq_prepare(dd_net *) { return DD_OK; }

int dd_netq_dwpw_fits(int cin, int cout, int stride, int h, int w, int split_filter, int *fits_host) {
    DD_REQUIRE(fits_host && cin > 0 && cout > 0 && (stride == 1 || stride == 2) && h > 0 && w > 0 && h < (1 << 20) && w < (1 << 20), DD_E_ARG,
               "dd_netq_dwpw_fits: %d -> %d channels, stride %d, %d x %d", cin, cout, stride, h, w);
    if ((long long)((h + stride - 1) / stride) * ((w + stride - 1) / stride) >= (1ll << 23)) { *fits_host = 0; return DD_OK; }
    QDwpwP Q;
    memset(&Q, 0, sizeof(Q));
    Q.H = h; Q.W = w; Q.ho = (h + stride - 1) / stride; Q.wo = (w + stride - 1) / stride; Q.hw = Q.ho * Q.wo;
    Q.off_y = 1 - std::max((Q.ho - 1) * stride + 3 - h, 0) / 2; Q.off_x = 1 - std::max((Q.wo - 1) * stride + 3 - w, 0) / 2;
    Q.c16_out = cout / 16;
    bool ok = false;
    const int rc = dwpw_dispatch(nullptr, Q, 1, 0, cin, cout, stride, &ok, true, nullptr, split_filter != 0);
    if (rc != DD_OK) return rc;
    *fits_host = ok ? 1 : 0;
    return DD_OK;
}

int netq_run_op(dd_net *net, int i, const int32_t *o, const uint8_t *input, int nimg, hipStream_t s, int *handled) {
    const int kind = o[0], src = o[1], dst = o[2];
    *handled = kind >= OP_QCONV0 && kind <= OP_QADD;
    if (!*handled) return DD_OK;
    auto base = [&](int t) -> uint8_t * { return static_cast<uint8_t *>(net->bufs[net->tensors[t].buf]); };
    const TensorDesc *ts = src >= 0 ? &net->tensors[src] : nullptr;
    const TensorDesc *td = dst >= 0 ? &net->tensors[dst] : nullptr;
    char *W = net->d_weights;
    int variant_none = 0;
    int *const variant = i < (int)net->op_variant.size() ? &net->op_variant[i] : &variant_none;
    switch (kind) {
        case OP_QCONV0: {
            QConv0P P;
            P.src = input; P.H = net->in_h; P.W = net->in_w; P.total_bytes = (long long)nimg * P.H * P.W * 3;
            P.stride = o[7]; P.pad_t = o[8]; P.pad_l = o[9]; P.ho = td->h; P.wo = td->w; P.m = nimg * P.ho * P.wo;
            P.w = reinterpret_cast<const i4v *>(W + (size_t)(uint32_t)o[16]);
            P.w2 = o[18] ? reinterpret_cast<const i4v *>(W + (size_t)(uint32_t)o[18]) : nullptr;
            P.cq = reinterpret_cast<const long long *>(W + (size_t)(uint32_t)o[46]);
            P.out = base(dst); P.in_zp = o[39]; P.zwc = o[38]; P.R = make_req(o);
            P.out_bytes = (long long)nimg * (P.ho + 2) * 2 * (P.wo + 2) * 16;
            DD_REQUIRE(td->w >= 16, DD_E_ARG, "dd_net_forward: uint8 first layer: output narrower than a fragment");
            DD_REQUIRE(td->pad == 1 && td->cs == 32 && o[11] == 32 && (reinterpret_cast<uintptr_t>(input) & 3) == 0 && (P.total_bytes & 3) == 0 && !P.R.linear && P.R.e >= 1,
                       DD_E_ARG, "dd_net_forward: uint8 first layer: 32 channels into a bordered tensor from a 4-byte aligned batch");
            DD_REQUIRE(o[46] != 0, DD_E_ARG, "dd_net_forward: uint8 first layer: no folded requantisation constants in the program");
            const long long in_img = (long long)P.H * P.W * 3, out_img = (long long)(P.ho + 2) * 2 * (P.wo + 2) * 16, lim31 = (1ll << 31) - 17;
            long long lim = std::min(lim31 / in_img, lim31 / out_img);
            if (in_img % 4) lim &= ~3ll;
            DD_REQUIRE(lim >= 1, DD_E_CAPACITY, "dd_net_forward: uint8 first layer: one frame beyond 31-bit offsets");
            const long long n_chunks = (nimg + lim - 1) / lim;
            long long chunk = (nimg + n_chunks - 1) / n_chunks;
            if (in_img % 4) chunk = std::min(lim, (chunk + 3) & ~3ll);
            const int sat0 = P.R.lo == 0 && P.R.hi == 255 ? (P.R.e <= 8 ? 2 : 1) : 0;
            const uint8_t *const src0 = P.src;
            uint8_t *const out0 = P.out;
            *variant = QV_CONV0 | (P.w2 ? 1 : 0) << 4 | sat0 << 5 | (int)std::min(n_chunks, 255ll) << 8;
            for (long long c0 = 0; c0 < nimg; c0 += chunk) {
                const int nc = (int)std::min(chunk, nimg - c0);
                P.src = src0 + c0 * in_img; P.out = out0 + c0 * out_img;
                P.total_bytes = nc * in_img; P.out_bytes = nc * out_img; P.m = nc * P.ho * P.wo;
                const int n_frags = dd_ceil_div(P.m, 16);
                const dim3 grid0(dd_ceil_div(n_frags, 4 * C0F));
#define DD_Q0(H_) do { if (sat0 == 2) hipLaunchKernelGGL((q_conv0_k<H_, 2>), grid0, dim3(256), 0, s, P, n_frags); \
                       else if (sat0 == 1) hipLaunchKernelGGL((q_conv0_k<H_, 1>), grid0, dim3(256), 0, s, P, n_frags); \
                       else hipLaunchKernelGGL((q_conv0_k<H_, 0>), grid0, dim3(256), 0, s, P, n_frags); } while (0)
                if (P.w2) DD_Q0(true); else DD_Q0(false);
#undef DD_Q0
                DD_LAUNCH_CHECK();
            }
            return DD_OK;
        }
        case OP_QCONV: {
            QConvP P;
            memset(&P, 0, sizeof(P));
            DD_REQUIRE(ts->pad == 1 && ts->cs % 16 == 0, DD_E_ARG, "dd_net_forward: uint8 conv %d reads a tensor that is not in the bordered layout", i);
            P.in = base(src); P.H = ts->h; P.W = ts->w; P.c16_in = ts->cs / 16;
            P.kh = o[5]; P.kw = o[6]; P.stride = o[7]; P.off_y = 1 - o[8]; P.off_x = 1 - o[9];
            P.ho = o[26]; P.wo = o[27]; P.m = nimg * P.ho * P.wo;
            P.w = reinterpret_cast<const i4v *>(W + (size_t)(uint32_t)o[16]);
            P.cbias = reinterpret_cast<const int *>(W + (size_t)(uint32_t)o[17]);
            P.kc_per_tap = o[13]; P.n_mfrag = o[12] / 16; P.epi = o[15];
            P.out = base(dst); P.zwc = o[38]; P.R = make_req(o);
            const int n_frag_a = o[14];
            QReq Rb = P.R;
            if (n_frag_a) {
                int32_t d[48] = {0}; d[32] = o[20]; d[33] = o[21]; d[40] = o[22]; d[36] = 0; d[37] = 255; d[41] = o[41]; Rb = make_req(d);
                DD_REQUIRE(o[4] >= 0 && P.epi == QEPI_ROWS && n_frag_a < P.n_mfrag && !net->tensors[o[4]].pad && o[23] % 4 == 0 && o[24] % 4 == 0 && o[25] % 4 == 0 && o[25] <= o[23] &&
                           (long long)o[24] + (long long)P.ho * P.wo * o[23] <= (long long)net->tensors[o[4]].h * net->tensors[o[4]].w * net->tensors[o[4]].cs, DD_E_ARG,
                           "dd_net_forward: uint8 conv %d: second predictor's row geometry", i);
            }
            DD_REQUIRE(P.off_y >= 0 && P.off_x >= 0 && (P.ho - 1) * P.stride + P.kh - 1 + P.off_y <= P.H + 1 && (P.wo - 1) * P.stride + P.kw - 1 + P.off_x <= P.W + 1,
                       DD_E_ARG, "dd_net_forward: uint8 conv %d reaches outside the one-pixel border", i);
            DD_REQUIRE(o[3] < 0 || P.epi == QEPI_Q16N, DD_E_ARG, "dd_net_forward: uint8 conv %d: a residual operand needs the natural bordered epilogue", i);
            if (P.epi == QEPI_Q16) {
                DD_REQUIRE(td->pad == 1 && td->h == P.ho && td->w == P.wo && o[12] % 64 == 0 && td->cs == o[12] && !P.R.linear, DD_E_ARG,
                           "dd_net_forward: uint8 conv %d: bordered output needs a multiple of 64 channels and an activation", i);
                P.Ho = td->h; P.Wo = td->w; P.c16_out = td->cs / 16; P.mq = 4;
            } else if (P.epi == QEPI_Q16N) {
                DD_REQUIRE(td->pad == 1 && td->h == P.ho && td->w == P.wo && o[12] % 16 == 0 && td->cs == o[12] && n_frag_a == 0 && (P.R.linear || P.R.lo >= P.R.zo) &&
                           P.R.e >= 0 && P.R.e <= 30 && P.R.lo >= 0 && P.R.lo <= P.R.hi && P.R.hi <= 255, DD_E_ARG,
                           "dd_net_forward: uint8 conv %d: natural bordered output geometry / requantisation", i);
                P.Ho = td->h; P.Wo = td->w; P.c16_out = td->cs / 16;
                P.mq = P.n_mfrag % 3 == 0 ? 3 : P.n_mfrag % 2 == 0 ? 2 : std::min(3, P.n_mfrag);
                if (o[3] >= 0) {
                    DD_REQUIRE(o[3] < (int)net->tensors.size(), DD_E_ARG, "dd_net_forward: uint8 conv %d: residual tensor %d out of range", i, o[3]);
                    const TensorDesc *tr = &net->tensors[o[3]];
                    P.res = base(o[3]); P.A = make_add(o);
                    DD_REQUIRE(tr->pad == 1 && tr->h == td->h && tr->w == td->w && tr->cs == td->cs && o[3] != dst && add_ok(P.A) && P.R.lo == 0 && P.R.hi == 255, DD_E_ARG,
                               "dd_net_forward: uint8 conv %d: residual operand geometry / ADD parameters", i);
                    if (i < (int)net->op_launch.size()) net->op_launch[i] = 21;
                }
            } else {
                P.img_bytes_out = (long long)td->h * td->w * td->cs; P.row_bytes = o[42]; P.base_off = o[43]; P.cout_store = o[44];
                DD_REQUIRE(!td->pad && P.row_bytes % 4 == 0 && P.base_off % 4 == 0 && P.cout_store % 4 == 0 && P.cout_store <= P.row_bytes &&
                           (long long)P.base_off + (long long)P.ho * P.wo * P.row_bytes <= P.img_bytes_out, DD_E_ARG, "dd_net_forward: uint8 conv %d: row output geometry", i);
                P.mq = std::min(4, P.n_mfrag);
            }
            static const int pws_env = getenv("DD_Q_PWS") ? atoi(getenv("DD_Q_PWS")) : 1;
            if (pws_env && P.epi != QEPI_Q16N && P.kh == 1 && P.kw == 1 && P.stride == 1 && P.off_y == 1 && P.off_x == 1 && (ts->cs == 512 || ts->cs == 1024) && P.m >= 8192 && P.n_mfrag >= 8 &&
                o[46] != 0 && (P.epi == QEPI_ROWS || (!P.R.linear && P.R.e >= 1))) {
                QPwsP Q;
                memset(&Q, 0, sizeof(Q));
                Q.in = P.in; Q.H = P.H; Q.W = P.W; Q.c16_in = P.c16_in; Q.hw = P.ho * P.wo; Q.m = P.m;
                Q.w = P.w; Q.cbias = P.cbias; Q.cq = reinterpret_cast<const long long *>(W + (size_t)(uint32_t)o[46]);
                Q.n_mfrag = P.n_mfrag; Q.out = P.out; Q.c16_out = P.c16_out; Q.zwc = P.zwc; Q.R = P.R;
                if (P.epi == QEPI_ROWS) { Q.img_bytes_out = P.img_bytes_out; Q.row_bytes = P.row_bytes; Q.base_off = P.base_off; Q.cout_store = P.cout_store; }
                if (n_frag_a) {
                    const TensorDesc *tb = &net->tensors[o[4]];
                    Q.n_frag_a = n_frag_a; Q.out_b = base(o[4]); Q.img_bytes_b = (long long)tb->h * tb->w * tb->cs; Q.row_bytes_b = o[23]; Q.base_off_b = o[24]; Q.cout_store_b = o[25];
                    Q.zwc_b = o[28]; Q.Rb = Rb;
                }
                bool ok = false;
                const int rc = ts->cs == 512 ? (P.epi == QEPI_ROWS && (P.n_mfrag + 2) / 3 <= 8 && P.n_mfrag % 4 != 0 ? launch_q_pws<512, 3>(s, Q, nimg, net->ctx->device, &ok, variant) : launch_q_pws<512, 4>(s, Q, nimg, net->ctx->device, &ok, variant))
                                             : launch_q_pws<1024, 2>(s, Q, nimg, net->ctx->device, &ok, variant);
                if (rc != DD_OK) return rc;
                if (ok) return DD_OK;
            }
            auto run_generic = [&](QConvP &P) -> int {
                P.hw_magic = P.wo > 1 && (long long)P.m * (P.ho * P.wo) < (1ll << 32) ? (unsigned)((1ull << 32) / (unsigned)(P.ho * P.wo)) + 1u : 0u;
                P.wo_magic = (unsigned)((1ull << 32) / (unsigned)P.wo) + 1u;
                const int n_mgroups = P.n_frag_a ? P.groups_a + dd_ceil_div(P.n_mfrag - P.n_frag_a, P.mq) : dd_ceil_div(P.n_mfrag, P.mq);
                const long long items2 = (long long)n_mgroups * dd_ceil_div(P.m, 32);
                static const int npf_env = getenv("DD_Q_NPF") ? atoi(getenv("DD_Q_NPF")) : 0;
                const int npf = npf_env ? npf_env : 2;
                (void)items2;
                const long long n_items = (long long)n_mgroups * dd_ceil_div(P.m, 16 * npf);
                DD_REQUIRE(n_items < (1ll << 31), DD_E_CAPACITY, "dd_net_forward: uint8 conv %d: %lld wave items", i, n_items);
                const bool rsum = P.zwc != 0 || (P.n_frag_a && P.zwc_b != 0);
                const bool pipe = n_items < 8192;
                static const int split_env = getenv("DD_Q_SPLITK") ? atoi(getenv("DD_Q_SPLITK")) : 1;
                const bool split = split_env && P.kh * P.kw == 9 && n_items < 1024;
                const dim3 grid(split ? (unsigned)n_items : (unsigned)((n_items + 3) / 4)), block(split ? 192 : 256);
                *variant = QV_CONV | P.mq << 4 | (int)rsum << 7 | npf << 8 | (int)(npf != 4 && (split || pipe)) << 11 | (split ? 3 : 1) << 12 | (P.epi == QEPI_Q16N ? 1 : 0) << 14 |
                           (P.n_frag_a ? 1 : 0) << 15 | (P.hw_magic ? 1 : 0) << 16 | (P.res ? 1 : 0) << 17 | (((*variant & 15) == QV_CONV ? (*variant >> 18 & 3) : 0) + 1) << 18;
#define DD_QC2(MQ_, R_, N_) do { if (npf == 4 && split) hipLaunchKernelGGL((q_conv_k<MQ_, R_, 4, false, 3, N_>), grid, block, 0, s, P, (int)n_items, n_mgroups); \
                                 else if (npf == 4) hipLaunchKernelGGL((q_conv_k<MQ_, R_, 4, false, 1, N_>), grid, block, 0, s, P, (int)n_items, n_mgroups); \
                                 else if (split) hipLaunchKernelGGL((q_conv_k<MQ_, R_, 2, true, 3, N_>), grid, block, 0, s, P, (int)n_items, n_mgroups); \
                                 else if (pipe) hipLaunchKernelGGL((q_conv_k<MQ_, R_, 2, true, 1, N_>), grid, block, 0, s, P, (int)n_items, n_mgroups); \
                                 else hipLaunchKernelGGL((q_conv_k<MQ_, R_, 2, false, 1, N_>), grid, block, 0, s, P, (int)n_items, n_mgroups); } while (0)
#define DD_QC(MQ_, N_) do { if (rsum) DD_QC2(MQ_, true, N_); else DD_QC2(MQ_, false, N_); } while (0)
                if (P.epi == QEPI_Q16N) { if (P.mq == 3) DD_QC(3, true); else if (P.mq == 2) DD_QC(2, true); else DD_QC(1, true); }
                else if (P.mq == 4) DD_QC(4, false); else if (P.mq == 3) DD_QC(3, false); else if (P.mq == 2) DD_QC(2, false); else DD_QC(1, false);
#undef DD_QC2
#undef DD_QC
                DD_LAUNCH_CHECK();
                return DD_OK;
            };
            if (n_frag_a == 0) return run_generic(P);
            const TensorDesc *tb = &net->tensors[o[4]];
            static const int heads_one = getenv("DD_Q_HEADS_ONE") ? atoi(getenv("DD_Q_HEADS_ONE")) : 1;
            if (heads_one) {
                P.mq = std::min(4, n_frag_a);
                P.n_frag_a = n_frag_a; P.groups_a = dd_ceil_div(n_frag_a, P.mq);
                P.out_b = base(o[4]); P.img_bytes_b = (long long)tb->h * tb->w * tb->cs; P.row_bytes_b = o[23]; P.base_off_b = o[24]; P.cout_store_b = o[25];
                P.zwc_b = o[28]; P.Rb = Rb;
                return run_generic(P);
            }
            QConvP P2 = P;
            P.n_mfrag = n_frag_a; P.mq = std::min(4, P.n_mfrag);
            int rc2 = run_generic(P);
            if (rc2 != DD_OK) return rc2;
            P2.w = P.w + (size_t)n_frag_a * (P.kh * P.kw * P.kc_per_tap) * 64; P2.cbias = P.cbias + 16 * n_frag_a;
            P2.n_mfrag -= n_frag_a; P2.mq = std::min(4, P2.n_mfrag);
            P2.out = base(o[4]); P2.img_bytes_out = (long long)tb->h * tb->w * tb->cs; P2.row_bytes = o[23]; P2.base_off = o[24]; P2.cout_store = o[25];
            P2.zwc = o[28]; P2.R = Rb;
            return run_generic(P2);
        }
        case OP_QDW: {
            QDwP P;
            DD_REQUIRE(ts->pad == 1 && td->pad == 1 && ts->cs == td->cs && ts->cs % 16 == 0, DD_E_ARG, "dd_net_forward: uint8 depthwise %d: tensor layouts", i);
            P.in = base(src); P.H = ts->h; P.W = ts->w; P.c16 = ts->cs / 16;
            P.stride = o[7]; P.off_y = 1 - o[8]; P.off_x = 1 - o[9]; P.ho = td->h; P.wo = td->w;
            P.w = reinterpret_cast<const short *>(W + (size_t)(uint32_t)o[16]);
            P.cbias = reinterpret_cast<const int *>(W + (size_t)(uint32_t)o[17]);
            P.out = base(dst); P.R = make_req(o);
            P.total = (long long)nimg * P.ho * P.c16 * P.wo;
            DD_REQUIRE(P.off_y >= 0 && P.off_x >= 0 && (P.ho - 1) * P.stride + 2 + P.off_y <= P.H + 1 && (P.wo - 1) * P.stride + 2 + P.off_x <= P.W + 1 && !P.R.linear,
                       DD_E_ARG, "dd_net_forward: uint8 depthwise %d reaches outside the one-pixel border", i);
            DD_REQUIRE(P.total < (1ll << 31) * 256, DD_E_CAPACITY, "dd_net_forward: uint8 depthwise %d: too many items", i);
            static const bool no_mfma = getenv("DD_Q_DW_VALU") && atoi(getenv("DD_Q_DW_VALU")) != 0;
            if (o[20] && P.R.e >= 1 && !no_mfma) {
                const long long in_img = (long long)(P.H + 2) * P.c16 * (P.W + 2) * 16, out_img = (long long)(P.ho + 2) * P.c16 * (P.wo + 2) * 16;
                auto items = [&](long long nc) { return (long long)P.c16 * ((nc * P.ho * P.wo + 63) / 64); };
                auto fits = [&](long long nc) { return items(nc) < (1ll << 31) && items(nc) * P.c16 < (1ll << 32) && (nc + 1) * in_img < (1ll << 32) && (nc + 1) * out_img < (1ll << 32); };
                DD_REQUIRE(fits(1), DD_E_CAPACITY, "dd_net_forward: uint8 depthwise %d: one frame beyond 32-bit offsets", i);
                long long n_chunks = 1;
                while (!fits((nimg + n_chunks - 1) / n_chunks)) ++n_chunks;
                const long long chunk = (nimg + n_chunks - 1) / n_chunks;
                for (long long c0 = 0; c0 < nimg; c0 += chunk) {
                    const int nc = (int)std::min(chunk, nimg - c0);
                    QDwmP Q;
                    Q.in = P.in + c0 * in_img; Q.H = P.H; Q.W = P.W; Q.c16 = P.c16; Q.stride = P.stride; Q.off_y = P.off_y; Q.off_x = P.off_x; Q.ho = P.ho; Q.wo = P.wo;
                    Q.m = nc * P.ho * P.wo; Q.out = P.out + c0 * out_img; Q.R = P.R;
                    Q.dw_a = reinterpret_cast<const uint2 *>(W + (size_t)(uint32_t)o[20]);
                    Q.dw_cb = reinterpret_cast<const int *>(W + (size_t)(uint32_t)o[21]);
                    const long long n_items = items(nc);
                    *variant = QV_DWM | (P.R.lo == 0 && P.R.hi == 255 ? 1 : 0) << 4 | 0 << 5 | (int)std::min(n_chunks, 255ll) << 8;
                    Q.hw_magic = (unsigned)((1ull << 32) / (unsigned)(P.ho * P.wo)) + 1u; Q.wo_magic = (unsigned)((1ull << 32) / (unsigned)P.wo) + 1u; Q.c16_magic = (unsigned)((1ull << 32) / (unsigned)P.c16) + 1u;
                    if ((long long)Q.m * (P.ho * P.wo) >= (1ll << 32) || P.wo < 2 || P.c16 < 2) Q.hw_magic = 0;
                    *variant |= (Q.hw_magic ? 1 : 0) << 5;
                    if (P.R.lo == 0 && P.R.hi == 255) hipLaunchKernelGGL((q_dwm_k<true>), dim3((unsigned)((n_items + 3) / 4)), dim3(256), 0, s, Q, (int)n_items);
                    else hipLaunchKernelGGL((q_dwm_k<false>), dim3((unsigned)((n_items + 3) / 4)), dim3(256), 0, s, Q, (int)n_items);
                    DD_LAUNCH_CHECK();
                }
                if (i < (int)net->op_launch.size()) net->op_launch[i] = 17;
                return DD_OK;
            }
            *variant = QV_DW | 1 << 8;
            hipLaunchKernelGGL(q_dw_k, dim3((unsigned)((P.total + 255) / 256)), dim3(256), 0, s, P);
            DD_LAUNCH_CHECK();
            return DD_OK;
        }
        case OP_QDWPW: {
            QDwpwP P;
            memset(&P, 0, sizeof(P));
            DD_REQUIRE(ts->pad == 1 && td->pad == 1 && ts->cs % 16 == 0 && td->cs % 64 == 0, DD_E_ARG, "dd_net_forward: uint8 block %d: tensor layouts", i);
            const int stride = o[7], cin = o[10], cout = o[11];
            P.in = base(src); P.H = ts->h; P.W = ts->w;
            P.off_y = 1 - o[8]; P.off_x = 1 - o[9]; P.ho = td->h; P.wo = td->w; P.hw = P.ho * P.wo; P.tiles_per_frame = dd_ceil_div(P.hw, QT);
            P.out = base(dst); P.c16_out = td->cs / 16;
            P.dw_a = reinterpret_cast<const uint2 *>(W + (size_t)(uint32_t)o[20]);
            P.dw_cq = reinterpret_cast<const long long *>(W + (size_t)(uint32_t)o[45]);
            P.cq = reinterpret_cast<const long long *>(W + (size_t)(uint32_t)o[46]);
            P.w = reinterpret_cast<const i4v *>(W + (size_t)(uint32_t)o[16]);
            P.w2 = o[18] ? reinterpret_cast<const i4v *>(W + (size_t)(uint32_t)o[18]) : nullptr;
            P.cbias = reinterpret_cast<const int *>(W + (size_t)(uint32_t)o[17]);
            P.zwc = o[38]; P.Rp = make_req(o); P.dup = o[47];
            { int32_t d[48] = {0}; d[32] = o[22]; d[33] = o[23]; d[36] = o[24]; d[37] = o[25]; d[40] = o[28]; P.Rd = make_req(d); }
            DD_REQUIRE(!P.dup || (cin == 32 && P.zwc == 0 && !P.w2), DD_E_ARG, "dd_net_forward: uint8 block %d: duplicated operand bytes are for 32 input channels", i);
            DD_REQUIRE(o[45] != 0 && o[46] != 0, DD_E_ARG, "dd_net_forward: uint8 block %d: the program carries no folded requantisation constants (compiled by an older netsq.py?)", i);
            DD_REQUIRE(cin == ts->cs && cout == td->cs && P.Rd.e >= 1 && P.Rp.e >= 1 && !P.Rd.linear && !P.Rp.linear && P.off_y >= 0 && P.off_x >= 0 &&
                       (P.ho - 1) * stride + 2 + P.off_y <= P.H + 1 && (P.wo - 1) * stride + 2 + P.off_x <= P.W + 1, DD_E_ARG,
                       "dd_net_forward: uint8 block %d: shapes / multipliers the fused kernel does not take", i);
            const long long in_img = (long long)(P.H + 2) * (P.W + 2) * ts->cs, out_img = (long long)(P.ho + 2) * (P.wo + 2) * td->cs;
            const long long lim = 4294967295ll / out_img, n_chunks = (nimg + lim - 1) / lim, chunk = (nimg + n_chunks - 1) / n_chunks;
            DD_REQUIRE(lim >= 1, DD_E_CAPACITY, "dd_net_forward: uint8 block %d: one frame's output beyond 32-bit offsets", i);
            const int dev = net->ctx->device;
            for (long long c0 = 0; c0 < nimg; c0 += chunk) {
                const int nc = (int)std::min(chunk, nimg - c0);
                QDwpwP Q = P;
                Q.in = P.in + c0 * in_img; Q.out = P.out + c0 * out_img;
                bool ok = false;
                int v = 0;
                const int rc = dwpw_dispatch(s, Q, nc, dev, cin, cout, stride, &ok, false, &v);
                if (rc != DD_OK) return rc;
                if (ok) *variant = v | (int)std::min(n_chunks, 127ll) << 21;
                DD_REQUIRE(ok, DD_E_ARG, "dd_net_forward: uint8 block %d (%d -> %d, stride %d, %d x %d): no fused kernel for this shape -- compile the program with the two-op form", i, cin, cout, stride, P.H, P.W);
            }
            return DD_OK;
        }
        case OP_QADD: {
            DD_REQUIRE(ts && td && o[3] >= 0 && o[3] < (int)net->tensors.size(), DD_E_ARG, "dd_net_forward: uint8 ADD %d: operands", i);
            const TensorDesc *tb = &net->tensors[o[3]];
            QAddP P;
            P.A = make_add(o);
            DD_REQUIRE(ts->pad == 1 && td->pad == 1 && tb->pad == 1 && ts->h == td->h && ts->w == td->w && ts->cs == td->cs && tb->h == td->h && tb->w == td->w &&
                       tb->cs == td->cs && td->cs % 16 == 0 && dst != src && dst != o[3] && add_ok(P.A), DD_E_ARG, "dd_net_forward: uint8 ADD %d: tensor layouts / parameters", i);
            P.H = td->h; P.W = td->w; P.c16 = td->cs / 16;
            const long long per_img = (long long)P.H * P.c16 * P.W, img_bytes = (long long)(P.H + 2) * (P.W + 2) * td->cs;
            DD_REQUIRE(per_img < (1ll << 31) - 256, DD_E_CAPACITY, "dd_net_forward: uint8 ADD %d: one frame beyond 31-bit items", i);
            const long long chunk = ((1ll << 31) - 256) / per_img;
            for (long long c0 = 0; c0 < nimg; c0 += chunk) {
                const long long nc = std::min(chunk, nimg - c0);
                P.a = base(src) + c0 * img_bytes; P.b = base(o[3]) + c0 * img_bytes; P.out = base(dst) + c0 * img_bytes;
                P.n_items = (int)(nc * per_img);
                *variant = QV_ADD | (int)std::min((nimg + chunk - 1) / chunk, 255ll) << 8;
                hipLaunchKernelGGL(q_add_k, dim3((unsigned)dd_ceil_div(P.n_items, 256)), dim3(256), 0, s, P);
                DD_LAUNCH_CHECK();
            }
            if (i < (int)net->op_launch.size()) net->op_launch[i] = 22;
            return DD_OK;
        }
        case OP_QSSD_DECODE: {
            if (!net->ssd_dec) return DD_OK;
            QDecP P;
            const TensorDesc &tb = net->tensors[o[1]], &tc = net->tensors[o[3]];
            P.box = base(o[1]); P.cls = base(o[3]);
            P.n_anchors = o[21]; P.n_classes = o[20]; P.cls_stride = tc.cs;
            DD_REQUIRE(P.n_anchors == net->dec_anchors && tb.cs == 4 && tb.h == P.n_anchors && tc.h == P.n_anchors && P.n_classes <= tc.cs, DD_E_ARG,
                       "dd_net_forward: uint8 decode of %d anchors, set up for %d", P.n_anchors, net->dec_anchors);
            P.lut = reinterpret_cast<const uint8_t *>(W + (size_t)(uint32_t)o[16]);
            const float *of = reinterpret_cast<const float *>(o);
            P.box_scale = of[32]; P.box_zp = of[33]; P.sc_scale = of[34]; P.sc_zp = of[35]; P.thr = net->dec_thr;
            P.anchors = net->d_anchors; P.boxes = net->dec_boxes; P.score = net->dec_score; P.keys = net->dec_keys; P.cls_out = net->dec_cls;
            DD_REQUIRE(P.cls_stride % 16 == 0 && P.n_classes <= 128, DD_E_ARG, "dd_net_forward: uint8 decode: %d classes in rows of %d bytes", P.n_classes, P.cls_stride);
            *variant = QV_DECODE;
            hipLaunchKernelGGL(q_ssd_decode_k, dim3(dd_ceil_div(P.n_anchors * 8, 256), nimg), dim3(256), 0, s, P);
            DD_LAUNCH_CHECK();
            return DD_OK;
        }
        default:
            DD_REQUIRE(false, DD_E_ARG, "dd_net_forward: uint8 op kind %d at %d is not built", kind, i);
    }
    return DD_OK;
}
```

### deepdish_amd/csrc/pipeline.hip

```cpp
#include <algorithm>
#include <cmath>
#include <cstdlib>
#include <map>
#include <string>
#include "common.h"
#include "hostpool.h"
#include "host_phases.h"

struct dd_tracker;
struct dd_mog2;
namespace ddk {
int mog2_apply(dd_mog2 *m, hipStream_t s, const uint8_t *frames, double learning_rate, uint8_t *mask, uint8_t *masked);
int mask_box_count(hipStream_t s, const uint8_t *mask, int H, int W, const int *d_boxes, const int *d_box_stream, int K, int *d_counts);
int yolov5_decode(hipStream_t s, const float *raw, int n_rows, int n_cls, float thr, float img_w, float img_h, float *out_boxes,
                  float *out_scores, int *out_cls, int cap, int *out_n, int batch, void *scratch);
int yolov5_select(hipStream_t s, const float *boxes4, const float *conf, const int *cls, int n_rows, float thr, float img_w, float img_h,
                  float *out_boxes, float *out_scores, int *out_cls, int cap, int *out_n, int batch);
int yolov5_decode_letterbox(hipStream_t s, const float *raw, int n_rows, int n_cls, float thr, int img_w, int img_h, int net_w, int net_h,
                            float *out_boxes, float *out_scores, int *out_cls, int cap, int *out_n, int batch, void *scratch);
int yolov5_select_letterbox(hipStream_t s, const float *boxes4, const float *conf, const int *cls, int n_rows, float thr, int img_w, int img_h,
                            int net_w, int net_h, float *out_boxes, float *out_scores, int *out_cls, int cap, int *out_n, int batch);
int resize_lanczos_letterbox(hipStream_t s, int device, const uint8_t *src, int batch, int H, int W, int src_c, int swap_rb, uint8_t *dst, int h, int w,
                             int pad, uint8_t *tmp);
size_t ssd_post_decoded_scratch_bytes(int n_anchors, int batch);
// ... 387 lines not shown
}

int dd_pipeline_counts(dd_pipeline *p, int64_t *counts_host) {
    DD_REQUIRE(p && counts_host, DD_E_ARG, "dd_pipeline_counts: NULL argument");
    const size_t n = p->wanted.size() * 4;
    for (int s = 0; s < p->S; ++s) memcpy(counts_host + (size_t)s * n, p->st[s].counts.data(), n * sizeof(int64_t));
    return DD_OK;
}

int dd_pipeline_detector_stream(dd_pipeline *p, void **stream_out) {
    DD_REQUIRE(p && stream_out, DD_E_ARG, "dd_pipeline_detector_stream: NULL argument");
    *stream_out = p->det ? reinterpret_cast<void *>(p->det_stream) : nullptr;
    return DD_OK;
}

int dd_pipeline_stage_gpu_ms(dd_pipeline *p, double *out6_host, long long *steps_host) {
    DD_REQUIRE(p && out6_host, DD_E_ARG, "dd_pipeline_stage_gpu_ms: NULL argument");
    DD_DEVICE(p->ctx);
    const int rc = flush_stage_events(p);
    if (rc != DD_OK) return rc;
    out6_host[0] = p->g_det; out6_host[1] = p->g_nms; out6_host[2] = p->g_enc; out6_host[3] = p->g_trk; out6_host[4] = p->g_host; out6_host[5] = p->g_wall;
    if (steps_host) *steps_host = p->steps;
    return DD_OK;
}

int dd_pipeline_detections(dd_pipeline *p, int stream, double *boxes_host, double *scores_host, int *classes_host, int cap, int *n_host) {
    DD_REQUIRE(p && n_host && stream >= 0 && stream < p->S && cap >= 0, DD_E_ARG, "dd_pipeline_detections: bad argument");
    const StreamState &q = p->st[stream];
    const int n = (int)q.scores0.size();
    *n_host = n;
    DD_REQUIRE(n <= cap || (!boxes_host && !scores_host && !classes_host), DD_E_CAPACITY, "dd_pipeline_detections: %d rows, room for %d", n, cap);
    if (boxes_host) memcpy(boxes_host, q.boxes0.data(), (size_t)n * 4 * sizeof(double));
    if (scores_host) memcpy(scores_host, q.scores0.data(), (size_t)n * sizeof(double));
    if (classes_host) memcpy(classes_host, q.cls0.data(), (size_t)n * sizeof(int));
    return DD_OK;
}

int dd_pipeline_overlay(dd_pipeline *p, const int *streams_host, int n, int *sizes_host, const int *caps_host, int64_t *track_ints_host,
                        double *track_tlbr_host, double *points_host, double *cross_host, double *det_tlbr_host, int64_t *counts_host,
                        double *line_host) {
    DD_REQUIRE(p && streams_host && sizes_host && n > 0, DD_E_ARG, "dd_pipeline_overlay: bad argument");
    for (int i = 0; i < n; ++i)
        DD_REQUIRE(streams_host[i] >= 0 && streams_host[i] < p->S, DD_E_ARG, "dd_pipeline_overlay: stream %d of %d", streams_host[i], p->S);
    const bool fill = track_ints_host && track_tlbr_host && points_host && cross_host && det_tlbr_host && counts_host && line_host;
    DD_REQUIRE(!fill || caps_host, DD_E_ARG, "dd_pipeline_overlay: arrays without their capacities");
    const bool stepped = p->steps > 0 && (int)p->doff.size() == p->S + 1;
    size_t nt = 0, np = 0, nc = 0, nd = 0;
    std::vector<int64_t> ints;
    std::vector<double> means;
    for (int i = 0; i < n; ++i) {
        const int z = streams_host[i];
        StreamState &st = p->st[z];
        int nl = 0, rc;
        if ((rc = dd_tracker_count(st.trk, 0, &nl)) != DD_OK) return rc;
        ints.resize((size_t)nl * 6); means.resize((size_t)nl * 8);
        if (nl && stepped && (rc = ddk::tracker_read_host(st.trk, 0, ints.data(), means.data())) != DD_OK) return rc;
        int *sz = sizes_host + (size_t)i * 4;
        sz[0] = sz[1] = sz[2] = 0;
        sz[3] = stepped ? p->doff[z + 1] - p->doff[z] : 0;
        for (int k = 0; stepped && k < nl; ++k) {
            const int64_t *r = ints.data() + (size_t)k * 6;
            if (r[1] != CONFIRMED || r[2] > 1) continue;
            const auto it = st.db.find(r[0]);
            const size_t npts = it == st.db.end() ? 0 : it->second.size();
            bool crossed = false;
            if (npts > 1) {
                const double a[2] = {it->second[npts - 1].first, it->second[npts - 1].second};
                const double b[2] = {it->second[npts - 2].first, it->second[npts - 2].second};
                crossed = seg_intersect(p->line, p->line + 2, a, b);
            }
            if (fill) {
                DD_REQUIRE(nt < (size_t)caps_host[0] && np + npts <= (size_t)caps_host[1] && nc + crossed <= (size_t)caps_host[2], DD_E_CAPACITY,
                           "dd_pipeline_overlay: more rows than the arrays have room for");
                const auto vt = st.votes.find(r[0]);
                const std::string lbl = vt == st.votes.end() ? std::string() : vote_label(p, vt->second);
                int64_t line_no = -1;
                for (size_t li = 0; li < p->labels.size() && line_no < 0 && !lbl.empty(); ++li) if (p->labels[li] == lbl) line_no = (int64_t)li;
                int64_t *ti = track_ints_host + nt * 3;
                ti[0] = r[0]; ti[1] = line_no; ti[2] = (int64_t)npts;
                const double *m = means.data() + (size_t)k * 8;
                const double w = m[2] * m[3];
                double *tb = track_tlbr_host + nt * 4;
                tb[0] = m[0] - w / 2; tb[1] = m[1] - m[3] / 2; tb[2] = tb[0] + w; tb[3] = tb[1] + m[3];
                for (size_t q = 0; q < npts; ++q) { points_host[(np + q) * 2] = it->second[q].first; points_host[(np + q) * 2 + 1] = it->second[q].second; }
                if (crossed) {
                    double *c = cross_host + nc * 4;
                    c[0] = it->second[npts - 2].first; c[1] = it->second[npts - 2].second; c[2] = it->second[npts - 1].first; c[3] = it->second[npts - 1].second;
                }
            }
            ++nt; ++sz[0]; np += npts; sz[1] += (int)npts; nc += crossed; sz[2] += crossed;
        }
        if (fill) {
            DD_REQUIRE(nd + sz[3] <= (size_t)caps_host[3], DD_E_CAPACITY, "dd_pipeline_overlay: more detections than the array has room for");
            for (int j = 0; j < sz[3]; ++j) {
                const double *b = p->tlwh.data() + (size_t)(p->doff[z] + j) * 4;
                double *o = det_tlbr_host + (nd + j) * 4;
                o[0] = b[0]; o[1] = b[1]; o[2] = b[0] + b[2]; o[3] = b[1] + b[3];
            }
            const size_t nw = p->wanted.size() * 4;
            memcpy(counts_host + (size_t)i * nw, st.counts.data(), nw * sizeof(int64_t));
        }
        nd += sz[3];
    }
    if (fill) for (int i = 0; i < 4; ++i) line_host[i] = p->line[i];
    return DD_OK;
}

int dd_pipeline_stage_seconds(dd_pipeline *p, double *out4_host, long long *steps_host) {
    DD_REQUIRE(p && out4_host, DD_E_ARG, "dd_pipeline_stage_seconds: NULL argument");
    out4_host[0] = p->t_det; out4_host[1] = p->t_nms; out4_host[2] = p->t_enc; out4_host[3] = p->t_trk;
    if (steps_host) *steps_host = p->steps;
    return DD_OK;
}

}

namespace {

int flush_stage_events(dd_pipeline *p) {
    if (!p->ev_pending) return DD_OK;
    p->ev_pending = false;
    double *into[6] = {&p->g_trk, &p->g_nms, &p->g_enc, &p->g_trk, &p->g_trk, &p->g_trk};
    for (int k = 0; k < 6; ++k) {
        if (!p->ev_pair[k]) continue;
        p->ev_pair[k] = false;
        float ms = 0.f;
        DD_HIP(hipEventSynchronize(p->ev_main[2 * k + 1]));
        DD_HIP(hipEventElapsedTime(&ms, p->ev_main[2 * k], p->ev_main[2 * k + 1]));
        *into[k] += (double)ms;
    }
    return DD_OK;
}
static const bool g_stage_events = !(getenv("DD_STAGE_EVENTS") && atoi(getenv("DD_STAGE_EVENTS")) == 0);
#define DD_STAGE_BEGIN(k) do { if (g_stage_events) DD_HIP(hipEventRecord(p->ev_main[2 * (k)], s)); } while (0)
#define DD_STAGE_END(k) do { if (g_stage_events) { DD_HIP(hipEventRecord(p->ev_main[2 * (k) + 1], s)); p->ev_pair[k] = true; } } while (0)
#define DD_TIMED_WAIT(expr) do { const double w0_ = now_s(); DD_HIP(expr); p->step_wait += now_s() - w0_; } while (0)

int enqueue_detector(dd_pipeline *p, const uint8_t *frames) {
    hipStream_t s = p->det_stream;
    const int S = p->S, MAX_DET = p->max_det;
    int rc;
    DD_HIP(hipEventRecord(p->main_mark, p->ctx->stream));
    DD_HIP(hipStreamWaitEvent(s, p->main_mark, 0));
    if (g_stage_events) DD_HIP(hipEventRecord(p->ev_det[0], s));
    if (p->det_kind == DET_TFLITE) {
        if ((rc = ddk::crop_resize(s, frames, p->H, p->W, p->d_tfl_boxes.p, S, p->det_in, p->det_in_w, p->d_resized.as<uint8_t>())) != DD_OK) return rc;
    } else if (p->letterbox_pad >= 0) {
        if ((rc = ddk::resize_lanczos_letterbox(s, p->ctx->device, frames, S, p->H, p->W, 3, 1, p->d_resized.as<uint8_t>(), p->det_in, p->det_in_w,
                                                p->letterbox_pad, p->d_tmp.as<uint8_t>())) != DD_OK) return rc;
    } else if ((rc = ddk::resize_lanczos(s, p->ctx->device, frames, p->H, p->W, 3, 1, p->d_resized.as<uint8_t>(), p->det_in,
                                         p->det_in_w, p->d_tmp.as<uint8_t>(), S)) != DD_OK) return rc;
    if ((rc = dd_net_forward(p->det, p->d_resized.as<uint8_t>(), S, s)) != DD_OK) return rc;
    void *raw = nullptr;
    if ((rc = dd_net_output(p->det, -1, &raw, nullptr, nullptr, nullptr, nullptr, nullptr)) != DD_OK) return rc;
    if (p->det_kind == DET_YOLOV5) {
        const size_t cap = (size_t)p->n_anchors;
        float *yb = p->d_fin.as<float>(), *ys = yb + S * cap * 4;
        int *yc = reinterpret_cast<int *>(ys + S * cap), *yn = yc + S * cap;
        if (p->yolo_dec) {
            float *b4 = nullptr, *cf = nullptr; int *cl = nullptr;
            if ((rc = dd_net_yolo_decoded(p->det, &b4, &cf, &cl, nullptr)) != DD_OK) return rc;
            if (p->letterbox_pad >= 0) {
                if ((rc = ddk::yolov5_select_letterbox(s, b4, cf, cl, p->n_anchors, (float)p->det_conf, p->W, p->H, p->det_in_w, p->det_in, yb, ys, yc,
                                                       p->n_anchors, yn, S)) != DD_OK) return rc;
            } else
            if ((rc = ddk::yolov5_select(s, b4, cf, cl, p->n_anchors, (float)p->det_conf, (float)p->W, (float)p->H, yb, ys, yc,
                                         p->n_anchors, yn, S)) != DD_OK) return rc;
        } else if (p->letterbox_pad >= 0) {
            if ((rc = ddk::yolov5_decode_letterbox(s, static_cast<const float *>(raw), p->n_anchors, p->n_classes, (float)p->det_conf, p->W, p->H,
                                                   p->det_in_w, p->det_in, yb, ys, yc, p->n_anchors, yn, S, p->d_post.p)) != DD_OK) return rc;
        } else
        if ((rc = ddk::yolov5_decode(s, static_cast<const float *>(raw), p->n_anchors, p->n_classes, (float)p->det_conf, (float)p->W,
                                     (float)p->H, yb, ys, yc, p->n_anchors, yn, S, p->d_post.p)) != DD_OK) return rc;
        if ((rc = ddk::yolov5_pack(s, yb, ys, yc, yn, p->n_anchors, S, p->d_pack.as<float>())) != DD_OK) return rc;
        const size_t head = ((size_t)S * 4 + 63) / 64 * 64;
        DD_HIP(hipMemcpyAsync(p->h_fin.p, yn, (size_t)S * 4, hipMemcpyDeviceToHost, s));
        DD_HIP(hipMemcpyAsync(p->h_fin.as<char>() + head, p->d_pack.p, p->yolo_host_rows * 24, hipMemcpyDeviceToHost, s));
        if (g_stage_events) DD_HIP(hipEventRecord(p->ev_det[1], s));
        DD_HIP(hipEventRecord(p->det_done, s));
        p->det_pending = frames;
        return DD_OK;
    }
    float *db = p->d_det.as<float>(), *dc = db + (size_t)S * MAX_DET * 4, *ds = dc + (size_t)S * MAX_DET;
    int *dn = reinterpret_cast<int *>(ds + (size_t)S * MAX_DET);
    if (p->ssd_per_class > 0) {
        if (p->q8.cls) rc = ddk::ssd_regular_nms_u8(s, p->q8.box, p->q8.cls, p->q8.stride, p->q8.lut, p->q8.quant, p->d_anchors, p->n_anchors, p->n_classes,
                                                    MAX_DET, p->ssd_per_class, p->ssd_score_thr, p->ssd_iou_thr, db, dc, ds, dn, S);
        else rc = ddk::ssd_regular_nms_raw(s, static_cast<const float *>(raw), p->d_anchors, p->n_anchors, p->n_classes, MAX_DET, p->ssd_per_class,
                                           p->ssd_score_thr, p->ssd_iou_thr, db, dc, ds, dn, S);
        if (rc != DD_OK) return rc;
    } else if (p->ssd_dec) {
        float *eb = nullptr, *es = nullptr, *ek = nullptr;
        int *ec = nullptr;
        if ((rc = dd_net_ssd_decoded(p->det, &eb, &es, &ec, &ek)) != DD_OK) return rc;
        if ((rc = ddk::ssd_postprocess_decoded(s, eb, es, ec, ek, p->n_anchors, MAX_DET, p->ssd_score_thr, p->ssd_iou_thr, db, dc, ds, dn, S,
                                               p->d_post.p, p->d_post.cap)) != DD_OK) return rc;
    } else if ((rc = ddk::ssd_postprocess(s, static_cast<const float *>(raw), p->d_anchors, p->n_anchors, p->n_classes, MAX_DET,
                                          p->ssd_score_thr, p->ssd_iou_thr, db, dc, ds, dn, S, p->d_post.p, p->d_post.cap)) != DD_OK) return rc;
    if (p->det_kind == DET_TFLITE) {
        const size_t dbytes = (size_t)S * MAX_DET * 6 * sizeof(float) + (size_t)S * sizeof(int);
        DD_HIP(hipMemcpyAsync(p->h_fin.p, p->d_det.p, dbytes, hipMemcpyDeviceToHost, s));
        if (g_stage_events) DD_HIP(hipEventRecord(p->ev_det[1], s));
        DD_HIP(hipEventRecord(p->det_done, s));
        p->det_pending = frames;
        return DD_OK;
    }
    double *fb = p->d_fin.as<double>(), *fs = fb + (size_t)S * MAX_DET * 4;
    int *fc = reinterpret_cast<int *>(fs + (size_t)S * MAX_DET), *fn = fc + (size_t)S * MAX_DET;
    if ((rc = ddk::ssd_finish(s, db, dc, ds, S, MAX_DET, p->det_conf, 0.5, (double)p->W, (double)p->H, fb, fc, fs, fn)) != DD_OK)
        return rc;
    const size_t fbytes = (size_t)S * (MAX_DET * (4 * 8 + 8 + 4) + 4);
    DD_HIP(hipMemcpyAsync(p->h_fin.p, p->d_fin.p, fbytes, hipMemcpyDeviceToHost, s));
    if (g_stage_events) DD_HIP(hipEventRecord(p->ev_det[1], s));
    DD_HIP(hipEventRecord(p->det_done, s));
    p->det_pending = frames;
    return DD_OK;
}

__global__ void __launch_bounds__(256) skip_gather_rows_k(const float4 *__restrict__ src, float4 *__restrict__ dst,
                                                          const int *__restrict__ dst_off, const int *__restrict__ src_off) {
    const int z = blockIdx.x;
    const int a = dst_off[z], n = dst_off[z + 1] - a;
    const float4 *sp = src + (size_t)src_off[z] * 32;
    float4 *dp = dst + (size_t)a * 32;
    for (int i = threadIdx.x; i < n * 32; i += blockDim.x) dp[i] = sp[i];
}

void count_line_one_stream(dd_pipeline *p, StreamState &st) {
    int nd = 0, nl = 0;
    dd_tracker_count(st.trk, 1, &nd);
    dd_tracker_count(st.trk, 0, &nl);
    std::vector<int64_t> &ints = st.ints;
    std::vector<double> &means = st.means;
    std::map<std::string, int> delcounts;
    if (nd) {
        ints.resize((size_t)nd * 6);
        ddk::tracker_read_host(st.trk, 1, ints.data(), nullptr);
        for (int i = 0; i < nd; ++i) {
            const int64_t id = ints[(size_t)i * 6];
            delcounts.clear();
            auto it = st.db.find(id);
            if (it != st.db.end() && it->second.size() > 1) {
                bool hit = false;
                for (size_t q = 0; q + 1 < it->second.size() && !hit; ++q) {
                    const double a[2] = {it->second[q].first, it->second[q].second};
                    const double b[2] = {it->second[q + 1].first, it->second[q + 1].second};
                    hit = seg_intersect(p->line, p->line + 2, a, b);
                }
                if (hit) delcounts[vote_label(p, st.votes[id])] += 1;
                it->second.clear();
            }
            st.votes.erase(id);
        }
    }
    if (nl) {
        ints.resize((size_t)nl * 6);
        means.resize((size_t)nl * 8);
        ddk::tracker_read_host(st.trk, 0, ints.data(), means.data());
    }
    std::vector<std::pair<std::string, double>> events;
    for (int i = 0; i < nl; ++i) {
        const int64_t *r = ints.data() + (size_t)i * 6;
        const int64_t id = r[0];
        if (r[5] >= 0) st.votes[id].add(st.det_cls[r[5]], st.det_conf[r[5]]);
        if (r[1] != CONFIRMED || r[2] > 1) continue;
        const double *m = means.data() + (size_t)i * 8;
        const double w = m[2] * m[3];
        const double x1 = m[0] - w / 2, y1 = m[1] - m[3] / 2;
        const double x2 = x1 + w, y2 = y1 + m[3];
        auto &pts = st.db[id];
        pts.emplace_back((x1 + x2) / 2.0, y2);
        if (pts.size() > 1) {
            const double p2[2] = {pts.back().first, pts.back().second};
            const double q2[2] = {pts[pts.size() - 2].first, pts[pts.size() - 2].second};
            const double cp = cross2(p->line[2] - p->line[0], p->line[3] - p->line[1], q2[0] - p2[0], q2[1] - p2[1]);
            if (seg_intersect(p->line, p->line + 2, p2, q2)) events.emplace_back(vote_label(p, st.votes[id]), cp);
        }
    }
    for (auto &e : events) {
        const int wi = wanted_index(p, e.first);
        if (wi < 0) continue;
        st.counts[wi * 4 + (e.second >= 0 ? 0 : 1)] += 1;
        st.counts[wi * 4 + 2] += 1;
    }
    for (auto &d : delcounts) {
        const int wi = wanted_index(p, d.first);
        if (wi >= 0) st.counts[wi * 4 + 3] += d.second;
    }
}

}

extern "C" {

int dd_pipeline_step2(dd_pipeline *p, const uint8_t *frames, const uint8_t *frames_next, const double *inj_boxes_host,
                      const double *inj_scores_host, const int *inj_cls_host, const int *inj_offsets_host);

int dd_pipeline_step(dd_pipeline *p, const uint8_t *frames, const double *inj_boxes_host, const double *inj_scores_host,
                     const int *inj_cls_host, const int *inj_offsets_host) {
    return dd_pipeline_step2(p, frames, nullptr, inj_boxes_host, inj_scores_host, inj_cls_host, inj_offsets_host);
}

int dd_pipeline_step2(dd_pipeline *p, const uint8_t *frames_in, const uint8_t *frames_next, const double *inj_boxes_host,
                      const double *inj_scores_host, const int *inj_cls_host, const int *inj_offsets_host) {
    DD_REQUIRE(p && frames_in, DD_E_ARG, "dd_pipeline_step: NULL argument");
    DD_REQUIRE(frames_next != frames_in, DD_E_ARG,
               "dd_pipeline_step2: frames_next must be a different buffer from frames (its detector run is queued while "
// ... 310 lines not shown
```

### deepdish_amd/engine.py

```python
import ctypes
import numpy as np
import torch

from ._lib import lib, check, P
from .runtime import default_context, ptr
from . import nets


class Net:
    def __init__(self, program, max_batch, context=None, shared=False):
        self.ctx = context or default_context()
        self.program = program
        self.max_batch = int(max_batch)
        words, blob = program.serialize()
        self._words = words
        blob_arr = np.frombuffer(blob, dtype=np.uint8)
        h = P()
        create = lib().dd_net_create_shared if shared else lib().dd_net_create
        check(create(self.ctx.handle, ptr(words), len(words), ptr(blob_arr), len(blob), self.max_batch, ctypes.byref(h)), 'dd_net_create')
        self._h = h
        t = program.tensors[program.out_tensor]
        self.out_shape = (t['h'], t['w'], t['cs'])
        self.out_dtype = {nets.DT_F16: torch.float16, nets.DT_F32: torch.float32, nets.DT_U8: torch.uint8}[t['dtype']]
        self.weight_bytes = len(blob)

    def __del__(self):
        try:
            if self._h:
                lib().dd_net_destroy(self._h)
                self._h = None
        except Exception:
            pass

    def activation_bytes(self):
        v = ctypes.c_int64()
        check(lib().dd_net_activation_bytes(self._h, ctypes.byref(v)), 'dd_net_activation_bytes')
        return v.value

    def use_graph(self, enable=True):
        check(lib().dd_net_use_graph(self._h, int(bool(enable))), 'dd_net_use_graph')

    def ssd_decode(self, anchors, score_thr, enable=True):
        if not enable:
            check(lib().dd_net_ssd_decode(self._h, None, 0, 0.0, 0), 'dd_net_ssd_decode')
            self._dec_anchors = 0
            return
        a = np.ascontiguousarray(anchors, dtype=np.float32)
        check(lib().dd_net_ssd_decode(self._h, ptr(a), len(a), float(score_thr), int(bool(enable))), 'dd_net_ssd_decode')
        self._dec_anchors = len(a) if enable else 0

    def ssd_heads_u8(self):
        box, cls, lut = P(), P(), P()
        stride, na, nc = ctypes.c_int(), ctypes.c_int(), ctypes.c_int()
        quant = np.zeros(4, np.float32)
        check(lib().dd_net_ssd_heads_u8(self._h, ctypes.byref(box), ctypes.byref(cls), ctypes.byref(stride), ctypes.byref(lut), ptr(quant),
                                        ctypes.byref(na), ctypes.byref(nc)), 'dd_net_ssd_heads_u8')
        return dict(box=box.value, cls=cls.value, lut=lut.value, cls_stride=stride.value, n_anchors=na.value, n_classes=nc.value, quant=quant)

    def ssd_decoded(self, n=None):
        n = self._last_n if n is None else n
        A = self._dec_anchors
        out = (np.zeros((n, A, 4), np.float32), np.zeros((n, A), np.float32), np.zeros((n, A), np.int32), np.zeros((n, A), np.float32))
        check(lib().dd_net_ssd_decoded_read(self._h, n, *[ptr(o) for o in out]), 'dd_net_ssd_decoded_read')
        return out

    def yolo_decode(self, enable=True):
        check(lib().dd_net_yolo_decode(self._h, int(bool(enable))), 'dd_net_yolo_decode')
        self._yolo_rows = int(self.program.meta['rows']) if enable else 0

    def yolo_decoded(self, n=None):
        n = self._last_n if n is None else n
        R = self._yolo_rows
        out = (np.zeros((n, R, 4), np.float32), np.zeros((n, R), np.float32), np.zeros((n, R), np.int32))
        check(lib().dd_net_yolo_decoded_read(self._h, n, *[ptr(o) for o in out]), 'dd_net_yolo_decoded_read')
        return out

    def forward(self, images, stream=None):
        if isinstance(images, np.ndarray):
            images = self.ctx.to_device(images, np.uint8)
        n = int(images.shape[0])
        assert images.dtype == torch.uint8 and tuple(images.shape[1:]) == (self.program.in_h, self.program.in_w, 3)
        check(lib().dd_net_forward(self._h, ptr(images), n, stream), 'dd_net_forward')
        self._last_n = n
        return n

    def read(self, n=None, tensor=-1, to_host=True):
        n = self._last_n if n is None else n
        t = self.program.tensors[self.program.out_tensor if tensor < 0 else tensor]
        shape = (t['h'] + 2, t['cs'] // 16, t['w'] + 2, 16) if t.get('q16') else (t['h'], t['w'], t['cs'])
        dt = {nets.DT_F16: torch.float16, nets.DT_F32: torch.float32, nets.DT_U8: torch.uint8}[t['dtype']]
        if to_host:
            out = np.zeros((n,) + shape, dtype={torch.float16: np.float16, torch.float32: np.float32, torch.uint8: np.uint8}[dt])
            check(lib().dd_net_read(self._h, tensor, n, ptr(out), 0, None), 'dd_net_read')
            return out
        out = self.ctx.empty((n,) + shape, dt)
        check(lib().dd_net_read(self._h, tensor, n, ptr(out), 1, None), 'dd_net_read')
        return out

    def output_ptr(self, tensor=-1):
        p = P()
        check(lib().dd_net_output(self._h, tensor, ctypes.byref(p), None, None, None, None, None), 'dd_net_output')
        return p.value
```

### deepdish_amd/netsq.py

```python
import os
import numpy as np

from . import nets, quantize
from .nets import Program, same_pad, DT_U8

OP_QCONV0, OP_QCONV, OP_QDW, OP_QDWPW, OP_QSSD_DECODE, OP_QADD = 16, 17, 18, 19, 20, 21
QEPI_Q16, QEPI_ROWS, QEPI_Q16N = 0, 1, 2
FUSE_BLOCKS = os.environ.get('DD_Q_FUSE', '1') != '0'
ADD_FUSE = os.environ.get('DD_Q_ADD_FUSE', '1') != '0'
SPLIT_PW = os.environ.get('DD_Q_SPLIT_PW', '1') != '0'
SPLIT_PW_MAX_CIN = int(os.environ.get('DD_Q_SPLIT_PW_MAX_CIN', '128'))
SPLIT_PW_MIN_CIN = int(os.environ.get('DD_Q_SPLIT_PW_MIN_CIN', '64'))
DUP32 = os.environ.get('DD_Q_DUP32', '1') != '0'
MERGE_HEADS = os.environ.get('DD_Q_MERGE_HEADS', '1') != '0'
FUSED_SHAPES = {(32, 64, 1), (64, 128, 2), (128, 128, 1), (128, 256, 2), (256, 256, 1), (256, 512, 2), (512, 512, 1)}
FEATURE_LAYERS = ['pw11', 'pw13', 'extra1_2', 'extra2_2', 'extra3_2', 'extra4_2']


def _req_words(L):
    m, shift = quantize.conv_multiplier(L)
    if shift > 0:
        raise ValueError('uint8 layer with a multiplier >= 1 (shift %d): not built' % shift)
    lo, hi = quantize.activation_range(L)
    linear = int(L['act'] == 'none')
    if not linear and lo < L['out_zp']:
        raise ValueError('activation clamp below the zero point')
    return {32: m, 33: -shift, 36: lo, 37: hi, 40: int(L['out_zp']), 41: linear}


def folded_addends(cb, rw):
    m, e, zo = int(rw[32]), int(rw[33]), int(rw[40])
    c = (1 << 30) + ((1 << (30 + e)) if e > 0 else 0) + (zo << (31 + e))
    out = [int(v) * m + c for v in np.asarray(cb).reshape(-1)]
    _model_need(all(-(1 << 62) < v < (1 << 62) for v in out), 'a requantisation addend (folded bias x multiplier + zero point << %d) leaves 62 bits' % (31 + e), 'uint8 layer')
    return np.array(out, dtype=np.int64)


def _cbias(L, w_i8_ck):
    za, zw = int(L['in_zp']) - 128, int(L['w_zp']) - 128
    k = w_i8_ck.shape[1]
    return (L['bias'].astype(np.int64) - za * w_i8_ck.sum(axis=1) + k * za * zw).astype(np.int64)


def pack_conv(L, epi, chan_map=None, cout_pad=None):
    w = L['w'].astype(np.int64) - 128
    kh, kw, cin, cout = w.shape
    if chan_map is None:
        chan_map = np.arange(cout)
    cout_pad = cout_pad or (len(chan_map) + 15) // 16 * 16
    cmap = np.full(cout_pad, -1, np.int64)
    cmap[:len(chan_map)] = chan_map
    kcpt = (cin + 63) // 64
    wk = np.zeros((cout_pad, kh * kw, kcpt * 64), np.int64)
    src = np.transpose(w, (3, 0, 1, 2)).reshape(cout, kh * kw, cin)
    valid = cmap >= 0
    wk[valid, :, :cin] = src[cmap[valid]]
    cb = np.zeros(cout_pad, np.int64)
    cb[valid] = _cbias(L, src.reshape(cout, -1))[cmap[valid]]
    _model_need(np.abs(cb).max() < 2 ** 31, 'a folded bias (bias - za * sum w + K za zw) leaves 32 bits', 'uint8 layer')
    n_mfrag = cout_pad // 16
    ksteps = kh * kw * kcpt
    if epi == QEPI_Q16:
        assert cout_pad % 64 == 0
        f = np.arange(n_mfrag)[:, None]
        row = np.arange(16)[None, :]
        chan = 64 * (f // 4) + 16 * (row // 4) + 4 * (f % 4) + (row % 4)
    else:
        chan = 16 * np.arange(n_mfrag)[:, None] + np.arange(16)[None, :]
    wf = wk[chan]
    wf = wf.reshape(n_mfrag, 16, kh * kw, kcpt, 4, 16)
    packed = np.transpose(wf, (0, 2, 3, 4, 1, 5)).reshape(n_mfrag, ksteps, 64, 16)
    return packed.astype(np.int8), cb.astype(np.int32), kcpt


def pack_conv0(L):
    def frags(w333o):
        src = np.transpose(w333o, (3, 0, 1, 2)).reshape(32, 3, 9)
        wk = np.zeros((32, 4, 16), np.int64)
        wk[:, :3, :9] = src
        f = np.arange(2)[:, None]
        row = np.arange(16)[None, :]
        chan = 8 * (row // 4) + 4 * f + (row % 4)
        return np.transpose(wk[chan], (0, 2, 1, 3)).reshape(2, 64, 16).astype(np.int8)
    w = L['w'].astype(np.int64)
    _model_need(w.shape == (3, 3, 3, 32), 'first layer with a filter of shape %s (3x3 over 3 colours into 32 channels is built)' % (tuple(w.shape),), 'uint8 layer')
    x = w - int(L['w_zp'])
    hi = np.clip(x, -128, 127)
    if int(L['w_zp']) != 128 and (x - hi).max() <= 127:
        cb = L['bias'].astype(np.int64) + (128 - int(L['in_zp'])) * x.reshape(27, 32).sum(axis=0)
        return frags(hi), frags(x - hi), cb.astype(np.int32)
    return frags(w - 128), None, _cbias(L, np.transpose(w - 128, (3, 0, 1, 2)).reshape(32, 27)).astype(np.int32)


def pack_dw(L):
    w = L['w'].astype(np.int64) - int(L['w_zp'])
    c = w.shape[2]
    cb = L['bias'].astype(np.int64) - (int(L['in_zp']) - 128) * w.reshape(9, c).sum(axis=0)
    return w.reshape(9, c).astype(np.int16), cb.astype(np.int32)


def pack_dw_mfma(L):
    w9 = (L['w'].astype(np.int64) - int(L['w_zp'])).reshape(9, -1)
    c = w9.shape[1]
    hi = np.clip(w9, -128, 127)
    lo = w9 - hi
    if lo.max() > 127:
        return None
    tab = np.zeros((c // 16, 64, 2, 4), np.uint8)
    for ks in range(3):
        for g in range(4):
            t = 4 * ks + g
            if t < 9:
                tab[:, g * 16:(g + 1) * 16, 0, ks] = (hi[t].reshape(c // 16, 16) & 0xff).astype(np.uint8)
                tab[:, g * 16:(g + 1) * 16, 1, ks] = (lo[t].reshape(c // 16, 16) & 0xff).astype(np.uint8)
    lo9 = np.zeros((12, c), np.int64)
    lo9[:9] = lo
    mask = sum(((lo9[4 * ks:4 * ks + 4].reshape(4, c // 16, 16) != 0).any(axis=(0, 2)).astype(np.uint8) << ks) for ks in range(3))
    tab[:, :, 1, 3] = mask[:, None]
    cb = L['bias'].astype(np.int64) - (int(L['in_zp']) - 128) * w9.sum(axis=0)
    return tab.reshape(c // 16, 64, 8).view(np.uint32).reshape(c // 16, 64, 2), cb.astype(np.int32)


def _model_need(cond, what, model='uint8 SSD-MobileNet-v1'):
    if not cond:
        from .tools.tflite_reader import UnsupportedModel
        raise UnsupportedModel('%s: %s' % (model, what))


def add_words(a):
    m1, e1, m2, e2, mo, eo = quantize.add_multipliers(a)
    return {20: m1, 21: e1, 22: m2, 23: e2, 24: mo, 25: eo, 28: int(a['in1_zp']), 29: int(a['in2_zp']), 31: int(a['out_zp']),
            34: int(a['lo']), 35: int(a['hi'])}


def pad_channels(L, cin=None, cout=None):
    w = L['w']
    pads = [(0, 0)] * 4
    if cin is not None:
        pads[2] = (0, cin - w.shape[2])
    if cout is not None:
        pads[3] = (0, cout - w.shape[3])
    if not any(p[1] for p in pads):
        return L
    w = np.pad(w, pads, constant_values=int(L['w_zp']))
    return dict(L, w=w, bias=np.pad(L['bias'], (0, w.shape[3] - len(L['bias']))))


def dwpw_fits(cin, cout, stride, h, w, split_filter=False):
    import ctypes
    from ._lib import lib, check
    ok = ctypes.c_int(0)
    check(lib().dd_netq_dwpw_fits(int(cin), int(cout), int(stride), int(h), int(w), int(bool(split_filter)), ctypes.byref(ok)), 'dd_netq_dwpw_fits')
    return bool(ok.value)


class QBuilder:

    def __init__(self, P, model='uint8 SSD-MobileNet-v1', pad=False):
        self.P, self.model, self.pad = P, model, pad
        self.layer_t = {}

    def need(self, cond, what):
        _model_need(cond, what, self.model)

    def geom(self, t, k, stride):
        d = self.P.T(t)
        ho, pt = same_pad(d['h'], k, stride)
        wo, pl = same_pad(d['w'], k, stride)
        return ho, wo, pt, pl

    def info(self, kernel, flops, nbytes, wbytes, src_bytes=0):
        self.P.info[-1] = dict(kernel=kernel, flops=flops, bytes=nbytes, wbytes=wbytes, src_bytes=src_bytes)

    def conv0(self, L):
        P = self.P
        ho, pt = same_pad(P.in_h, 3, L['stride'])
        wo, pl = same_pad(P.in_w, 3, L['stride'])
        x = P.qtensor(ho, wo, 32, L['out_zp'])
        wp, wl, cb = pack_conv0(L)
        raw = _req_words(L)
        P.add_blob(np.zeros(16, np.uint8))
        raw.update({38: 0 if wl is not None else 128 - int(L['w_zp']), 39: int(L['in_zp']), 46: P.add_blob(folded_addends(cb, raw))})
        P._op(OP_QCONV0, dst=x, kh=3, kw=3, stride=L['stride'], pad_t=pt, pad_l=pl, cin=3, cout=32, cout_pad=32,
              w_off=P.add_blob(wp), b_off=P.add_blob(cb), aff_off=P.add_blob(wl) if wl is not None else 0, ho=ho, wo=wo, raw=raw)
        self.info('q_conv0_k', 2 * ho * wo * 27 * 32, 3 * P.in_h * P.in_w + ho * wo * 32, 27 * 32 + 4 * 32, 3 * P.in_h * P.in_w)
        return x

    def conv(self, src, L0, name='?', epi=None, res=-1, add=None, dst=None, chan_map=None, cout_pad=None, row_bytes=0, base_off=0, cout_store=0):
        P = self.P
        s = P.T(src)
        L = pad_channels(L0, cin=s['c'], cout=(L0['w'].shape[3] + 15) // 16 * 16 if epi != QEPI_ROWS else None) if self.pad else L0
        kh = L['w'].shape[0]
        ho, wo, pt, pl = self.geom(src, kh, L['stride'])
        self.need(s['zp'] == L['in_zp'] and L0['w'].shape[2] <= s['c'] and L['w'].shape[2] == s['c'],
                  '%s: input zero point %s / channels %s, its producer writes %s / %s' % (name, L['in_zp'], L0['w'].shape[2], s['zp'], s['c']))
        if epi is None:
            epi = QEPI_Q16 if not self.pad or (L['act'] == 'relu6' and res < 0 and L['w'].shape[3] % 64 == 0) else QEPI_Q16N
        wp, cb, kcpt = pack_conv(L, epi, chan_map, cout_pad)
        if epi != QEPI_ROWS:
            dst = P.qtensor(ho, wo, L['w'].shape[3], add['out_zp'] if add is not None else L['out_zp'])
        raw = _req_words(L)
        raw.update({38: 128 - int(L['w_zp']), 39: int(L['in_zp']), 42: row_bytes, 43: base_off, 44: cout_store})
        raw[46] = P.add_blob(folded_addends(cb, raw) if not raw[41] else np.array([int(v) * int(raw[32]) + (1 << 30) for v in cb], dtype=np.int64))
        if add is not None:
            r = P.T(res)
            self.need(r['zp'] == add['in2_zp'] and L['out_zp'] == add['in1_zp'] and (r['h'], r['w'], r['c']) == (ho, wo, L['w'].shape[3]),
                      '%s: the residual ADD reads tensors of other geometry or zero points' % name)
            raw.update(add_words(add))
        if self.pad and epi != QEPI_ROWS and add is None:
            self.layer_t[name] = dst
        P._op(OP_QCONV, src=src, dst=dst, res=res, kh=kh, kw=kh, stride=L['stride'], pad_t=pt, pad_l=pl, cin=s['c'], cout=L['w'].shape[3],
              cout_pad=len(cb), kpad=kcpt, epi=epi, w_off=P.add_blob(wp), b_off=P.add_blob(cb), ho=ho, wo=wo, raw=raw)
        cin, cout = L0['w'].shape[2:]
        pws = not self.pad and kh == 1 and L['stride'] == 1 and cin in (512, 1024) and len(cb) >= 128
        self.info('q_pws_k' if pws else 'q_conv_k', 2 * ho * wo * kh * kh * cin * cout, s['h'] * s['w'] * cin + ho * wo * cout, kh * kh * cin * cout + 4 * cout)
        return dst

    def conv_heads(self, src, Lc, Lb, cls_args, box_args, name='?'):
        P = self.P
        s = P.T(src)
        ho, wo, pt, pl = self.geom(src, 1, 1)
        self.need(s['zp'] == Lc['in_zp'] == Lb['in_zp'] and Lc['w'].shape[:3] == Lb['w'].shape[:3] == (1, 1, s['c']), '%s: 1x1 predictors on one feature map with one input zero point' % name)
        wc, cbc, kcpt = pack_conv(Lc, QEPI_ROWS, cls_args['chan_map'], cls_args['cout_pad'])
        wb, cbb, _ = pack_conv(Lb, QEPI_ROWS, None, None)
        rc, rb = _req_words(Lc), _req_words(Lb)
        self.need(rc[41] and rb[41], '%s: predictors carry no activation' % name)
        lin = lambda cb, r: np.array([int(v) * int(r[32]) + (1 << 30) for v in cb], dtype=np.int64)
        raw = dict(rc)
        raw.update({38: 128 - int(Lc['w_zp']), 39: int(Lc['in_zp']), 42: cls_args['row_bytes'], 43: cls_args['base_off'], 44: cls_args['cout_store'],
                    46: P.add_blob(np.concatenate([lin(cbc, rc), lin(cbb, rb)])),
                    20: rb[32], 21: rb[33], 22: rb[40], 23: box_args['row_bytes'], 24: box_args['base_off'], 25: box_args['cout_store'], 28: 128 - int(Lb['w_zp'])})
        P._op(OP_QCONV, src=src, dst=cls_args['dst'], dst2=box_args['dst'], kh=1, kw=1, stride=1, pad_t=pt, pad_l=pl, cin=s['c'], cout=Lc['w'].shape[3] + Lb['w'].shape[3],
              cout_pad=len(cbc) + len(cbb), kpad=kcpt, act=len(cbc) // 16, epi=QEPI_ROWS, w_off=P.add_blob(np.concatenate([wc, wb])), b_off=P.add_blob(np.concatenate([cbc, cbb])),
              ho=ho, wo=wo, raw=raw)
        cin = s['c']
        cout = Lc['w'].shape[3] + Lb['w'].shape[3]
        self.info('q_pws_k', 2 * ho * wo * cin * cout, s['h'] * s['w'] * cin + ho * wo * cout, cin * cout + 4 * cout)

    def dw(self, src, L, name='?'):
        P = self.P
        ho, wo, pt, pl = self.geom(src, 3, L['stride'])
        s = P.T(src)
        self.need(s['zp'] == L['in_zp'] and L['w'].shape[2] == s['c'], '%s: input zero point %s / channels %s, its producer writes %s / %s' % (name, L['in_zp'], L['w'].shape[2], s['zp'], s['c']))
        w16, cb = pack_dw(L)
        dst = P.qtensor(ho, wo, s['c'], L['out_zp'])
        if self.pad:
            self.layer_t[name] = dst
        mf = pack_dw_mfma(L)
        P._op(OP_QDW, src=src, dst=dst, kh=3, kw=3, stride=L['stride'], pad_t=pt, pad_l=pl, cin=s['c'], cout=s['c'], cout_pad=s['c'],
              w_off=P.add_blob(w16), b_off=P.add_blob(cb), ho=ho, wo=wo, raw=_req_words(L),
              p=[P.add_blob(mf[0]), P.add_blob(mf[1])] if mf is not None else [0, 0])
        self.info('q_dw_k', 2 * ho * wo * 9 * s['c'], s['h'] * s['w'] * s['c'] + ho * wo * s['c'], 9 * s['c'] + 4 * s['c'])
        return dst

    def dwpw_fused(self, src, Ld, Lp):
        s = self.P.T(src)
        cin, cout, stride = s['c'], Lp['w'].shape[3], Ld['stride']
        ho, wo, pt, pl = self.geom(src, 3, stride)
        if not FUSE_BLOCKS or (cin, cout, stride) not in FUSED_SHAPES or wo < 19:
            return False
        return dwpw_fits(cin, cout, stride, s['h'], s['w'], SPLIT_PW and SPLIT_PW_MIN_CIN <= cin <= SPLIT_PW_MAX_CIN)

    def dwpw(self, src, Ld, Lp, dname='?', pname='?'):
        P = self.P
        s = P.T(src)
        cin, cout, stride = s['c'], Lp['w'].shape[3], Ld['stride']
        ho, wo, pt, pl = self.geom(src, 3, stride)
        if not self.dwpw_fused(src, Ld, Lp):
            return self.conv(self.dw(src, Ld, dname), Lp, pname)
        self.need(s['zp'] == Ld['in_zp'] and Ld['out_zp'] == Lp['in_zp'] and Ld['w'].shape[2] == cin and Lp['w'].shape[2] == cin, '%s / %s: zero points and channel counts along the block do not agree' % (dname, pname))
        packed_dw = pack_dw_mfma(Ld)
        rd, rp = _req_words(Ld), _req_words(Lp)
        if packed_dw is None or rd[33] < 1 or rp[33] < 1:
            return self.conv(self.dw(src, Ld, dname), Lp, pname)
        dwa, dcb = packed_dw
        wp, cb, kcpt = pack_conv(Lp, QEPI_Q16)
        zwc = 128 - int(Lp['w_zp'])
        w_lo = 0
        dup = 0
        if DUP32 and cin == 32 and zwc != 0:
            x = Lp['w'].astype(np.int64) - int(Lp['w_zp'])
            hi = np.clip(x, -128, 127)
            if (x - hi).max() <= 127:
                wp, _, kcpt = pack_conv(dict(Lp, w=np.concatenate([hi + 128, x - hi + 128], axis=2).astype(np.int64)), QEPI_Q16)
                cb = (Lp['bias'].astype(np.int64) + (128 - int(Lp['in_zp'])) * x.reshape(cin, cout).sum(axis=0)).astype(np.int32)
                zwc, dup = 0, 1
        if SPLIT_PW and SPLIT_PW_MIN_CIN <= cin <= SPLIT_PW_MAX_CIN and zwc != 0:
            x = Lp['w'].astype(np.int64) - int(Lp['w_zp'])
            hi = np.clip(x, -128, 127)
            if (x - hi).max() <= 127:
                wp, _, _ = pack_conv(dict(Lp, w=(hi + 128).astype(np.int64)), QEPI_Q16)
                wl, _, _ = pack_conv(dict(Lp, w=(x - hi + 128).astype(np.int64)), QEPI_Q16)
                w_lo = P.add_blob(wl)
                cb = (Lp['bias'].astype(np.int64) + (128 - int(Lp['in_zp'])) * x.reshape(cin, cout).sum(axis=0)).astype(np.int32)
                zwc = 0
        dst = P.qtensor(ho, wo, cout, Lp['out_zp'])
        raw = dict(rp)
        raw.update({38: zwc, 39: int(Lp['in_zp']), 45: P.add_blob(folded_addends(dcb, rd)), 46: P.add_blob(folded_addends(cb, rp)), 47: dup})
        P._op(OP_QDWPW, src=src, dst=dst, kh=1, kw=1, stride=stride, pad_t=pt, pad_l=pl, cin=cin, cout=cout, cout_pad=cout, kpad=kcpt,
              w_off=P.add_blob(wp), b_off=P.add_blob(cb), aff_off=w_lo, ho=ho, wo=wo,
              p=[P.add_blob(dwa), P.add_blob(dcb), rd[32], rd[33], rd[36], rd[37]], bk=rd[40], raw=raw)
        self.info('q_dwpw_k', 2 * ho * wo * cin * (9 + cout), s['h'] * s['w'] * cin + ho * wo * cout, cin * (9 + cout) + 4 * (cin + cout), s['h'] * s['w'] * cin)
        return dst

    def add_op(self, a_t, b_t, add):
        P = self.P
        t1, t2 = P.T(a_t), P.T(b_t)
        self.need(t1['zp'] == add['in1_zp'] and t2['zp'] == add['in2_zp'] and (t1['h'], t1['w'], t1['c']) == (t2['h'], t2['w'], t2['c']),
                  'ADD of tensors with other geometry or zero points')
        dst = P.qtensor(t1['h'], t1['w'], t1['c'], add['out_zp'])
        P._op(OP_QADD, src=a_t, dst=dst, res=b_t, cin=t1['c'], cout=t1['c'], ho=t1['h'], wo=t1['w'], raw=add_words(add))
        nb = t1['h'] * t1['w'] * t1['c']
        self.info('q_add_k', 0, 3 * nb, 0, 2 * nb)
        return dst

    def rows_tensors(self, n_anchors, n_cls):
        cls_row = (n_cls + 15) // 16 * 16
        box_t = self.P.tensor(n_anchors, 1, 4, cs=4, dtype=DT_U8)
        cls_t = self.P.tensor(n_anchors, 1, n_cls, cs=cls_row, dtype=DT_U8)
        return box_t, cls_t, cls_row

    @staticmethod
    def head_args(box_t, cls_t, a, n_cls, cls_row, base):
        cmap = np.full(a * cls_row, -1, np.int64)
        for an in range(a):
            cmap[an * cls_row:an * cls_row + n_cls] = an * n_cls + np.arange(n_cls)
        box_args = dict(dst=box_t, row_bytes=4 * a, base_off=4 * base, cout_store=4 * a)
        cls_args = dict(dst=cls_t, chan_map=cmap, cout_pad=(a * cls_row + 15) // 16 * 16, row_bytes=a * cls_row, base_off=cls_row * base, cout_store=a * cls_row)
        return box_args, cls_args

    def decode(self, box_t, cls_t, Lb, Lc, logistic, n_cls, n_anchors, cls_row):
        P = self.P
        lut = quantize.logistic_table(Lc['out_scale'], Lc['out_zp'], logistic['out_scale'], logistic['out_zp'])
        P._op(OP_QSSD_DECODE, src=box_t, res=cls_t, w_off=P.add_blob(lut), p=[n_cls, n_anchors],
              rawf={32: float(Lb['out_scale']), 33: float(Lb['out_zp']), 34: float(logistic['out_scale']), 35: float(logistic['out_zp'])})
        self.info('q_ssd_decode_k', 0, n_anchors * (4 + cls_row + 24), 256)


def compile_ssd_mobilenet_quant(qm):
    if qm.get('kind') == 'ssd_mobilenet_v2_uint8':
        return compile_ssd_mobilenet_v2_quant(qm)
    size = int(qm['input']['size'])
    P = Program(size, size)
    B = QBuilder(P)
    Ls = qm['layers']
    anchors, maps = nets.ssd_anchors(size)
    if qm.get('anchors') is not None:
        B.need(tuple(qm['anchors'].shape) == tuple(anchors.shape), 'anchors %s (this input size gives %s)' % (tuple(qm['anchors'].shape), tuple(anchors.shape)))
        anchors = np.ascontiguousarray(qm['anchors'], dtype=np.float32)
    n_anchors = len(anchors)
    x = B.conv0(Ls['conv0'])
    conv = lambda src, name, **kw: B.conv(src, Ls[name], name, **kw)
    feats = {}
    for i in range(1, 14):
        x = B.dwpw(x, Ls[f'dw{i}'], Ls[f'pw{i}'], f'dw{i}', f'pw{i}')
        feats[f'pw{i}'] = x
    for j in range(1, 5):
        x = conv(conv(x, f'extra{j}_1'), f'extra{j}_2')
        feats[f'extra{j}_2'] = x
    n_cls = Ls['cls0']['w'].shape[3] // nets.SSD_ANCHORS_PER_MAP[0]
    box_t, cls_t, cls_row = B.rows_tensors(n_anchors, n_cls)
    base = 0
    for k, (fname, a) in enumerate(zip(FEATURE_LAYERS, nets.SSD_ANCHORS_PER_MAP)):
        ft = feats[fname]
        fm = P.T(ft)['h']
        B.need(fm == maps[k], 'feature map %d is %dx%d (the anchors are laid out for %d)' % (k, fm, fm, maps[k]))
        for other in (f'box{k}', f'cls{k}'):
            B.need((Ls[other]['out_scale'], Ls[other]['out_zp']) == (Ls[other[:3] + '0']['out_scale'], Ls[other[:3] + '0']['out_zp']),
                   'the six %s tensors are concatenated: they need one (scale, zero point)' % other[:3])
        box_args, cls_args = B.head_args(box_t, cls_t, a, n_cls, cls_row, base)
        if MERGE_HEADS and P.T(ft)['c'] in (512, 1024):
            B.conv_heads(ft, Ls[f'cls{k}'], Ls[f'box{k}'], cls_args, box_args, f'cls{k} / box{k}')
        else:
            conv(ft, f'box{k}', epi=QEPI_ROWS, **box_args)
            conv(ft, f'cls{k}', epi=QEPI_ROWS, **cls_args)
        base += fm * fm * a
    B.need(base == n_anchors, '%d anchors for predictors that emit %d rows' % (n_anchors, base))
    B.decode(box_t, cls_t, Ls['box0'], Ls['cls0'], qm['logistic'], n_cls, n_anchors, cls_row)
    P.out_tensor = cls_t
    P.meta = dict(kind='ssd_mobilenet_v1_uint8', anchors=anchors, n_classes=n_cls, box_tensor=box_t, cls_tensor=cls_t, cls_row=cls_row,
                  feats=feats, quant=True)
    return P


def compile_ssd_mobilenet_v2_quant(qm):
    size = int(qm['input']['size'])
    P = Program(size, size)
    B = QBuilder(P, 'uint8 SSD-MobileNet-v2', pad=True)
    need = B.need
    Ls = qm['layers']
    anchors, maps = nets.ssd_anchors(size)
    if qm.get('anchors') is not None:
        need(tuple(qm['anchors'].shape) == tuple(anchors.shape), 'anchors %s (this input size gives %s)' % (tuple(qm['anchors'].shape), tuple(anchors.shape)))
        anchors = np.ascontiguousarray(qm['anchors'], dtype=np.float32)
    n_anchors = len(anchors)
    layer_t = B.layer_t

    L = Ls['conv0']
    need(L['w'].shape == (3, 3, 3, 32) and L['act'] == 'relu6', 'conv0: a 3x3 layer of 32 channels with ReLU6')
    x = layer_t['conv0'] = B.conv0(L)
    conv = lambda src, name, **kw: B.conv(src, Ls[name], name, **kw)

    feats = {}
    blocks = []
    while 'b%d_dw' % len(blocks) in Ls:
        blocks.append('b%d' % len(blocks))
    need(len(blocks) == 17, '%d inverted-residual blocks (MobileNet-v2 has 17)' % len(blocks))
    for b in blocks:
        h = x
        if b + '_expand' in Ls:
            h = conv(x, b + '_expand')
            feats[b + '_expand'] = h
        h = B.dw(h, Ls[b + '_dw'], b + '_dw')
        add = qm.get('add', {}).get(b)
        if add is None:
            x = conv(h, b + '_project')
        elif ADD_FUSE:
            x = layer_t[b] = conv(h, b + '_project', res=x, add=add)
        else:
            x = layer_t[b] = B.add_op(conv(h, b + '_project'), x, add)
        feats[b] = x
    x = conv(x, 'conv_last')
    feats['conv_last'] = x
    for j in range(1, 5):
        x = conv(conv(x, f'extra{j}_1'), f'extra{j}_2')
        feats[f'extra{j}_2'] = x
    n_cls = Ls['cls0']['w'].shape[3] // nets.SSD_ANCHORS_PER_MAP[0]
    box_t, cls_t, cls_row = B.rows_tensors(n_anchors, n_cls)
    base = 0
    for k, (fname, a) in enumerate(zip(quantize.V2_FEATURE_LAYERS, nets.SSD_ANCHORS_PER_MAP)):
        ft = feats[fname]
        fm = P.T(ft)['h']
        need(fm == maps[k], 'feature map %d is %dx%d (the anchors are laid out for %d)' % (k, fm, fm, maps[k]))
        for other in (f'box{k}', f'cls{k}'):
            need((Ls[other]['out_scale'], Ls[other]['out_zp']) == (Ls[other[:3] + '0']['out_scale'], Ls[other[:3] + '0']['out_zp']),
                 'the six %s tensors are concatenated: they need one (scale, zero point)' % other[:3])
        box_args, cls_args = B.head_args(box_t, cls_t, a, n_cls, cls_row, base)
        conv(ft, f'box{k}', epi=QEPI_ROWS, **box_args)
        conv(ft, f'cls{k}', epi=QEPI_ROWS, **cls_args)
        base += fm * fm * a
    need(base == n_anchors, '%d anchors for predictors that emit %d rows' % (n_anchors, base))
    B.decode(box_t, cls_t, Ls['box0'], Ls['cls0'], qm['logistic'], n_cls, n_anchors, cls_row)
    P.out_tensor = cls_t
    P.meta = dict(kind='ssd_mobilenet_v2_uint8', anchors=anchors, n_classes=n_cls, box_tensor=box_t, cls_tensor=cls_t, cls_row=cls_row,
                  feats=feats, quant=True, layer_tensors=layer_t)
    return P


def unpack_q16(raw, h, w, c):
    n = raw.size // ((h + 2) * (w + 2) * c)
    a = np.asarray(raw, dtype=np.uint8).reshape(n, h + 2, c // 16, w + 2, 16)[:, 1:-1, :, 1:-1, :] ^ 0x80
    return np.ascontiguousarray(np.transpose(a, (0, 1, 3, 2, 4)).reshape(n, h, w, c))


def borders_q16(raw, h, w, c):
    n = raw.size // ((h + 2) * (w + 2) * c)
    a = np.asarray(raw, dtype=np.uint8).reshape(n, h + 2, c // 16, w + 2, 16) ^ 0x80
    return np.concatenate([a[:, 0].reshape(-1), a[:, -1].reshape(-1), a[:, :, :, 0].reshape(-1), a[:, :, :, -1].reshape(-1)])
```

### deepdish_amd/profile.py

```python
import collections
import ctypes
import numpy as np

from ._lib import lib, check
from .runtime import ptr

PEAK_F16_TFLOPS = 2500.0
PEAK_HBM_GBS = 8000.0
PEAK_I8_TOPS = 5000.0


def last_batch(net):
    n = ctypes.c_int()
    check(lib().dd_net_last_batch(net._h, ctypes.byref(n)), 'dd_net_last_batch')
    return n.value


def net_op_times(net):
    n = len(net.program.ops)
    ms = np.zeros(n, dtype=np.float32)
    cnt = ctypes.c_int()
    check(lib().dd_net_profile_read(net._h, ptr(ms), n, ctypes.byref(cnt)), 'dd_net_profile_read')
    return ms


OPK_FOLDED = 1
OPK_NAMES = {2: 'conv3x3_pool_rows_k', 3: 'conv3x3_pool_rows_k<STEM>', 4: 'res_unit_rows_k', 5: 'ssd_front_k', 6: 'conv3x3_c64_rows_k', 7: 'conv3x3_s2_rows_k', 8: 'conv_ws_k', 9: 'conv_ws_dw_k', 10: 'dwpw_rows_k', 11: 'conv_glds_k<ssd_head_decode>', 12: 'res_pair_rows_k', 13: 'conv_glds_k<yolo_head_decode>', 14: 'mars_ws128_k', 16: 'mars_pair64_k', 17: 'q_dwm_k', 18: 'conv3x3_c64_rows_k<strips>', 19: 'q_front_k', 20: 'q_mid_k', 21: 'q_conv_k<add>', 22: 'q_add_k', 23: 'stem_conv_pool_wide_k'}
OPK_FOLDED_PREV = 15


def net_op_launches(net):
    n = len(net.program.ops)
    codes = np.zeros(n, dtype=np.int32)
    cnt = ctypes.c_int(0)
    check(lib().dd_net_op_launches(net._h, ptr(codes), n, ctypes.byref(cnt)), 'dd_net_op_launches')
    return codes


CONV_MODES = {0: 'conv_glds_k<general>', 1: 'conv_glds_k<pointwise>', 2: 'conv_glds_k<taps>', 3: 'conv_mfma_k'}


def net_op_variants(net):
    n = len(net.program.ops)
    codes = np.zeros(n, dtype=np.int32)
    cnt = ctypes.c_int(0)
    check(lib().dd_net_op_variants(net._h, ptr(codes), n, ctypes.byref(cnt)), 'dd_net_op_variants')
    return [None if not c else (c & 15, c >> 4 & 15, c >> 8 & 15, c >> 12 & 15, (c >> 16 & 15) * 16, c >> 20 & 15, c >> 24 & 127)
            for c in (int(v) for v in codes)]


QConvV = collections.namedtuple('QConvV', 'kernel MQ ROWSUM NPF PIPE SPLIT Q16N merged magic add launches')
QPwsV = collections.namedtuple('QPwsV', 'kernel K MW epi ROWSUM SAT merged')
QDwV = collections.namedtuple('QDwV', 'kernel SAT magic chunks')
QDwpwV = collections.namedtuple('QDwpwV', 'kernel CIN COUT STRIDE QTT form SAT chunks')
QConv0V = collections.namedtuple('QConv0V', 'kernel HL SAT chunks')
QOtherV = collections.namedtuple('QOtherV', 'kernel chunks')
Q_EPI_NAMES = {0: 'q16', 1: 'rows'}
Q_DWPW_FORMS = {0: 'plain', 1: 'rowsum', 2: 'hilo', 3: 'dup'}


def q_variant(c):
    c = int(c)
    k = c & 15
    if k == 1:
        return QConvV('q_conv_k', c >> 4 & 7, bool(c >> 7 & 1), c >> 8 & 7, bool(c >> 11 & 1), c >> 12 & 3, bool(c >> 14 & 1), bool(c >> 15 & 1),
                      bool(c >> 16 & 1), bool(c >> 17 & 1), c >> 18 & 3)
    if k == 2:
        return QPwsV('q_pws_k', 512 * (c >> 4 & 3), c >> 6 & 7, Q_EPI_NAMES[c >> 9 & 3], bool(c >> 11 & 1), c >> 12 & 3, bool(c >> 14 & 1))
    if k == 3:
        return QDwV('q_dw_k', 0, False, c >> 8 & 255)
    if k == 4:
        return QDwV('q_dwm_k', c >> 4 & 1, bool(c >> 5 & 1), c >> 8 & 255)
    if k == 5:
        return QDwpwV('q_dwpw_k', 32 * (c >> 4 & 31), 64 * (c >> 9 & 15), c >> 13 & 3, 64 * (c >> 15 & 3), Q_DWPW_FORMS[c >> 17 & 3], c >> 19 & 3, c >> 21 & 127)
    if k == 6:
        return QConv0V('q_conv0_k', bool(c >> 4 & 1), c >> 5 & 3, c >> 8 & 255)
    if k == 7:
        return QOtherV('q_add_k', c >> 8 & 255)
    if k == 8:
        return QOtherV('q_ssd_decode_k', 1)
    return None


def q_op_variants(net):
    n = len(net.program.ops)
    codes = np.zeros(n, dtype=np.int32)
    cnt = ctypes.c_int(0)
    check(lib().dd_net_op_variants(net._h, ptr(codes), n, ctypes.byref(cnt)), 'dd_net_op_variants')
    return [q_variant(c) for c in codes]


def launches_of(net, ms, batch):
    out, pend = [], None
    for t, info, code in zip(ms, net.program.info, net_op_launches(net)):
        fl, by = info['flops'] * batch, info['bytes'] * batch + info.get('wbytes', 0)
        if code == OPK_FOLDED:
            if pend is None:
                pend = [float(t), fl, info.get('src_bytes', 0) * batch + info.get('wbytes', 0)]
            else:
                pend[0] += float(t); pend[1] += fl; pend[2] += info.get('wbytes', 0)
            continue
        if code == OPK_FOLDED_PREV and out:
            k0, t0, f0, b0 = out[-1]
            out[-1] = (k0, t0 + float(t), f0 + fl, b0 + by)
            continue
        if pend is not None:
            t, fl, by = float(t) + pend[0], fl + pend[1], by - info.get('src_bytes', 0) * batch + pend[2]
            pend = None
        out.append((OPK_NAMES.get(int(code), info['kernel']), float(t), fl, by))
    return out


def profile_nets(run_once, nets_with_batch, reps=20):
    for _, net, _ in nets_with_batch:
        check(lib().dd_net_profile(net._h, 1), 'dd_net_profile')
    acc = {}
    try:
        for _ in range(reps):
            run_once()
            for name, net, batch in nets_with_batch:
                ms = net_op_times(net)
                b = batch() if callable(batch) else batch
                for kname, t, fl, by in launches_of(net, ms, b):
                    k = acc.setdefault(kname, dict(ms=0.0, flops=0.0, bytes=0.0, launches=0))
                    k['ms'] += t; k['flops'] += fl; k['bytes'] += by; k['launches'] += 1
    finally:
        for _, net, _ in nets_with_batch:
            check(lib().dd_net_profile(net._h, 0), 'dd_net_profile')
    for k in acc.values():
        for f in ('ms', 'flops', 'bytes'):
            k[f] /= reps
        k['launches'] /= reps
    return acc


def pmc_traffic(kernel, streams):
    import json, os
    root = os.path.join(os.path.dirname(os.path.dirname(os.path.abspath(__file__))), 'profiles')
    path = next((p for p in (os.path.join(root, 'r%02d_pmc_traffic_s%d.json' % (r, streams)) for r in (6, 5, 4, 3, 2, 1)) if os.path.exists(p)), None)
    if path is None:
        return None, None
    keys = [part.replace(',', ', ') for part in kernel.split('+')]
    tot_b = tot_n = 0.0
    for k, v in json.load(open(path)).items():
        if any(key in k for key in keys):
            tot_b += (v['hbm_read_bytes_corrected'] + v['hbm_write_bytes']) * v['launches']
            tot_n += v['launches']
    src = 'profiles/%s (rocprofv3 --pmc FETCH_SIZE and WRITE_SIZE passes of `bench.py --groups 1 --streams %d`, committed; not measured in this run)' % (os.path.basename(path), streams)
    return (tot_b / tot_n, src) if tot_n else (None, None)


def dominant_kernel_roofline(pipes, step_group, args, reps=20):
    f0 = args.warmup
    p = pipes[0]
    nets = [('mars', p.enc, lambda: last_batch(p.enc))]
    if p.det is not None:
        nets.append(('ssd', p.det, p.S))
    state = dict(f=f0)

    def run_once():
        step_group(0, state['f'])
        state['f'] = f0 + (state['f'] + 1 - f0) % max(1, args.steps)

    acc = profile_nets(run_once, nets, reps)
    per_kernel = {n: round(v['ms'], 5) for n, v in sorted(acc.items(), key=lambda kv: -kv[1]['ms'])}
    fam = [n for n in ('conv_glds_k', 'conv_ws_k', 'conv_ws_dw_k', 'conv_glds_k<ssd_head_decode>') if n in acc]
    if len(fam) > 1:
        parts = [acc.pop(n) for n in fam]
        acc['+'.join(fam)] = {f: sum(p[f] for p in parts) for f in ('ms', 'flops', 'bytes', 'launches')}
    name, k = max(acc.items(), key=lambda kv: kv[1]['ms'])
    sec = k['ms'] * 1e-3
    avg_us = 1e3 * k['ms'] / max(k['launches'], 1e-9)
    if name.startswith('q_'):
        achieved = k['bytes'] / sec / 1e9
        out = dict(bound='hbm', achieved=achieved, peak=PEAK_HBM_GBS, unit='GB/s', frac=achieved / PEAK_HBM_GBS,
                   mfma_i8=dict(achieved=k['flops'] / sec / 1e12, peak=PEAK_I8_TOPS, unit='TOP/s', frac=k['flops'] / sec / 1e12 / PEAK_I8_TOPS))
    elif name.startswith('conv') or name.startswith('res_unit'):
        achieved = k['flops'] / sec / 1e12
        out = dict(bound='mfma', achieved=achieved, peak=PEAK_F16_TFLOPS, unit='TFLOP/s', frac=achieved / PEAK_F16_TFLOPS)
    else:
        achieved = k['bytes'] / sec / 1e9
        out = dict(bound='hbm', achieved=achieved, peak=PEAK_HBM_GBS, unit='GB/s', frac=achieved / PEAK_HBM_GBS)
    traffic, traffic_source = pmc_traffic(name, p.S)
    out.update(kernel=name, traffic=traffic, traffic_source=traffic_source, launches_per_step=k['launches'], avg_launch_us=avg_us,
               frames_per_launch=p.S,
               algorithmic_per_launch=dict(flops=k['flops'] / max(k['launches'], 1e-9), bytes=k['bytes'] / max(k['launches'], 1e-9)),
               measured='HIP events on the launch stream, one worker group (%d streams) alone on the GPU' % p.S,
               per_kernel_ms_per_step=per_kernel)
    return out
```

Baseline: 146,000 frames/s.

## Fuse uint8 SSD anchor decode into the predictor pointwise conv epilogue

Adds a decode epilogue to the quantised pointwise-conv kernel for the SSD class/box heads. Weights are regrouped offline so that each block holds whole anchors, and each block reduces the best class per anchor with LDS atomics and a logistic LUT. A dedicated wave then decodes boxes and writes boxes, scores and keys directly. This skips writing the uint8 head tensors and the separate q_ssd_decode launch. The pipeline also stops fetching the raw output pointer when it is unused. The cost is extra LDS, an extra pass by the last wave per tile, and a fallback path when the shapes do not fit.

Measured after the change: 147,000 frames/s (median of 2 runs). About the same (+0.7%).

```diff
diff --git a/deepdish_amd/csrc/net_priv.h b/deepdish_amd/csrc/net_priv.h
--- a/deepdish_amd/csrc/net_priv.h
+++ b/deepdish_amd/csrc/net_priv.h
@@ -26,6 +26,7 @@
     bool ssd_dec = false, yolo_dec = false;
     int dec_anchors = 0; float dec_thr = 0.f;
     float *d_anchors = nullptr, *dec_boxes = nullptr, *dec_score = nullptr, *dec_keys = nullptr; int *dec_cls = nullptr;
+    bool q_dec_fuse = true, q_heads_exposed = false;
     bool slab_moved = false;
     _Float16 *d_zero = nullptr;
     bool use_glds = true;
@@ -39,6 +40,9 @@
     std::map<std::pair<const void *, int>, GraphEntry> graphs;
 };
 
+constexpr int DD_OP_WORDS = 48;
+constexpr int DD_OPK_Q_HEAD_DEC = 24;
+
 int netq_run_op(dd_net *net, int op_index, const int32_t *o, const uint8_t *input, int nimg, hipStream_t s, int *handled);
 int netq_run_front(dd_net *net, const int32_t *o0, const int32_t *o1, const int32_t *o2, const uint8_t *input, int nimg, hipStream_t s, int *ran);
 int netq_run_mid(dd_net *net, const int32_t *o3, const int32_t *o4, int nimg, hipStream_t s, int *ran);
diff --git a/deepdish_amd/csrc/nets.hip b/deepdish_amd/csrc/nets.hip
--- a/deepdish_amd/csrc/nets.hip
+++ b/deepdish_amd/csrc/nets.hip
@@ -4148,6 +4148,13 @@
     const int t = tensor < 0 ? n->out_tensor : tensor;
     DD_REQUIRE(t >= 0 && t < (int)n->tensors.size(), DD_E_ARG, "dd_net_output: tensor %d out of range", t);
     const TensorDesc &d = n->tensors[t];
+    if (dev_ptr)
+        for (int i = 0; i < n->n_ops && i < (int)n->op_launch.size(); ++i) {
+            const int32_t *o = n->prog.data() + n->ops_off + (size_t)i * OP_WORDS;
+            DD_REQUIRE(!((o[2] == t || o[4] == t) && n->op_launch[i] == DD_OPK_Q_HEAD_DEC), DD_E_STATE,
+                       "dd_net_output: tensor %d (a uint8 SSD head tensor) was not written in full by the last forward: predictor op %d decoded its anchors "
+                       "in its epilogue (dd_net_ssd_decode); take dd_net_ssd_decoded, or switch the engine with enable = 2", t, i);
+        }
     if (dev_ptr) *dev_ptr = static_cast<char *>(n->bufs[d.buf]) + (size_t)d.coff * dtype_size(d.dtype);
     if (h) *h = d.h;
     if (w) *w = d.w;
@@ -4217,6 +4224,9 @@
         DD_REQUIRE(!(o[2] == t && n->op_launch[i] == OPK_YOLO_HEAD_DEC), DD_E_STATE,
                    "dd_net_read: tensor %d (the Detect matrix) was not written: the head layers reduced their rows in their epilogue "
                    "(dd_net_yolo_decode); read dd_net_yolo_decoded instead", t);
+        DD_REQUIRE(!((o[2] == t || o[4] == t) && n->op_launch[i] == DD_OPK_Q_HEAD_DEC), DD_E_STATE,
+                   "dd_net_read: tensor %d (a uint8 SSD head tensor) was not written in full: predictor op %d decoded its anchors in its epilogue "
+                   "(dd_net_ssd_decode); read dd_net_ssd_decoded, or switch the engine with enable = 2", t, i);
         DD_REQUIRE(!((o[2] == t || o[4] == t) && n->op_launch[i] == OPK_FOLDED), DD_E_STATE,
                    "dd_net_read: tensor %d was not written by the last forward (op %d ran inside the next op's launch at this batch "
                    "size and its output stayed on chip); run a smaller batch or a program compiled without the fusion flags", t, i);
@@ -4274,6 +4284,8 @@
     DD_HIP(hipMemcpy(net->d_anchors, anchors_host, (size_t)n_anchors * 4 * sizeof(float), hipMemcpyHostToDevice));
     net->dec_thr = score_thr;
     net->ssd_dec = true;
+    static const bool fuse_env = !(getenv("DD_Q_DEC_FUSE") && atoi(getenv("DD_Q_DEC_FUSE")) == 0);
+    net->q_dec_fuse = enable != 2 && fuse_env;
     return DD_OK;
 }
 
@@ -4355,6 +4367,8 @@
         *lut = reinterpret_cast<const uint8_t *>(net->d_weights + (size_t)(uint32_t)o[16]);
         const float *of = reinterpret_cast<const float *>(o);
         for (int q = 0; q < 4; ++q) quant4_host[q] = of[32 + q];
+        DD_DEVICE(net->ctx);
+        if (!net->q_heads_exposed) { net->q_heads_exposed = true; net_drop_graphs(net); }
         return DD_OK;
     }
     DD_REQUIRE(false, DD_E_ARG, "dd_net_ssd_heads_u8: the program has no uint8 SSD head");
diff --git a/deepdish_amd/csrc/netsq.hip b/deepdish_amd/csrc/netsq.hip
--- a/deepdish_amd/csrc/netsq.hip
+++ b/deepdish_amd/csrc/netsq.hip
@@ -440,6 +440,7 @@
 struct QDecP {
     const uint8_t *box, *cls;
     int n_anchors, n_classes, cls_stride;
+    int a_begin, a_end;
     const uint8_t *lut;
     float box_scale, box_zp, sc_scale, sc_zp, thr;
     const float *anchors;
@@ -450,9 +451,9 @@
     __shared__ uint8_t lut[256];
     lut[threadIdx.x] = P.lut[threadIdx.x];
     __syncthreads();
-    const int a = (blockIdx.x * 256 + threadIdx.x) >> 3, sub = threadIdx.x & 7;
+    const int a = P.a_begin + ((blockIdx.x * 256 + threadIdx.x) >> 3), sub = threadIdx.x & 7;
     const size_t z = blockIdx.y;
-    const bool live = a < P.n_anchors;
+    const bool live = a < P.a_end;
     const uint8_t *c = P.cls + (z * P.n_anchors + (live ? a : 0)) * P.cls_stride;
     int best = -1, bi = 0x7fffffff;
     if (sub * 16 < P.n_classes) {
@@ -1054,11 +1055,20 @@
     int n_frag_a;
     uint8_t *out_b; long long img_bytes_b; int row_bytes_b, base_off_b, cout_store_b, zwc_b;
     QReq Rb;
+    int dec_ag, dec_fa, dec_gf, n_classes;
+    const uint8_t *lut;
+    float box_scale, box_zp, sc_scale, sc_zp, thr;
+    const float *anchors;
+    float *boxes, *score, *keys; int *cls_out;
 };
+
+constexpr int QEPI_DEC = 3;
+constexpr int QDEC_AG = 4;
 
 template <int K, int MW, int EPI, bool ROWSUM, int SAT>
 __global__ __launch_bounds__(512, 2) void q_pws_k(const QPwsP P, const int n_tiles) {
     constexpr int KC = K / 64, C16 = K / 16;
+    constexpr bool DEC = EPI == QEPI_DEC;
     static_assert(MW * KC * 4 <= 128, "the wave's filter is 128 registers at most");
     extern __shared__ __attribute__((aligned(16))) uint8_t smem[];
     uint8_t *opnd = smem;
@@ -1066,16 +1076,20 @@
     unsigned *pdst = psrc + 4 * QT;
     int *rowsum = reinterpret_cast<int *>(pdst + 4 * QT);
     unsigned *pdstb = reinterpret_cast<unsigned *>(rowsum + 3 * QT);
+    unsigned *keymax = pdstb + 4 * QT;
+    unsigned *boxw = keymax + 2 * QT * QDEC_AG;
+    uint8_t *lut_s = reinterpret_cast<uint8_t *>(boxw + 2 * QT * QDEC_AG);
     const int tid = threadIdx.x, lane = tid & 63, wave = __builtin_amdgcn_readfirstlane(tid >> 6), NW = blockDim.x >> 6;
     const int fr = lane & 15, fq = lane >> 4;
-    const int frag0 = blockIdx.y * P.frags_per_group + wave * MW;
+    const int frag0 = DEC ? blockIdx.y * P.dec_gf + wave * MW : blockIdx.y * P.frags_per_group + wave * MW;
+    const int frag_end = DEC ? (blockIdx.y + 1) * P.dec_gf : P.n_mfrag;
     const unsigned PP = (unsigned)(P.W + 2) * 16u;
 
     i4v Wr[MW][KC];
 #pragma unroll
     for (int m = 0; m < MW; ++m)
 #pragma unroll
-        for (int kc = 0; kc < KC; ++kc) Wr[m][kc] = frag0 + m < P.n_mfrag ? P.w[((size_t)(frag0 + m) * KC + kc) * 64 + lane] : i4v{0, 0, 0, 0};
+        for (int kc = 0; kc < KC; ++kc) Wr[m][kc] = frag0 + m < frag_end ? P.w[((size_t)(frag0 + m) * KC + kc) * 64 + lane] : i4v{0, 0, 0, 0};
     const int M = P.R.M, sh = P.R.e - 1, lo = P.R.lo, hi = P.R.hi;
     const int mg = frag0 / 4, m0 = frag0 % 4;
     long long CQ[MW][4];
@@ -1084,19 +1098,27 @@
 #pragma unroll
         for (int r = 0; r < 4; ++r) {
             const int ch = EPI == QEPI_Q16 ? 64 * mg + 16 * fq + 4 * (m0 + m) + r : 16 * (frag0 + m) + 4 * fq + r;
-            CQ[m][r] = frag0 + m < P.n_mfrag ? P.cq[ch] : 0ll;
+            CQ[m][r] = frag0 + m < frag_end ? P.cq[ch] : 0ll;
         }
     const int nfa = EPI == QEPI_ROWS && P.n_frag_a ? P.n_frag_a : P.n_mfrag;
-    bool hb[MW]; int chm[MW], Mm[MW], em[MW], k1m[MW], zwm[MW];
+    bool hb[MW]; int chm[MW], Mm[MW], em[MW], k1m[MW], zwm[MW], agm[MW];
     int n_store_m = 0;
 #pragma unroll
     for (int m = 0; m < MW; ++m) {
-        hb[m] = frag0 + m >= nfa;
-        chm[m] = 16 * (frag0 + m - (hb[m] ? nfa : 0));
+        if constexpr (DEC) {
+            const int slot = wave * MW + m;
+            hb[m] = slot == P.dec_gf - 1;
+            agm[m] = slot / P.dec_fa; chm[m] = 16 * (slot - agm[m] * P.dec_fa);
+        } else {
+            hb[m] = frag0 + m >= nfa;
+            chm[m] = 16 * (frag0 + m - (hb[m] ? nfa : 0));
+            agm[m] = 0;
+        }
         const QReq &Rm = hb[m] ? P.Rb : P.R;
         Mm[m] = Rm.M; em[m] = Rm.e; k1m[m] = (1 << (Rm.e - 1)) + (Rm.zo << Rm.e); zwm[m] = hb[m] ? P.zwc_b : P.zwc;
-        n_store_m += frag0 + m < P.n_mfrag && chm[m] < (hb[m] ? P.cout_store_b : P.cout_store) ? 1 : 0;
-    }
+        n_store_m += !DEC && frag0 + m < P.n_mfrag && chm[m] < (hb[m] ? P.cout_store_b : P.cout_store) ? 1 : 0;
+    }
+    const bool dec_wave = DEC && wave == NW - 1;
 
     const int t_begin = blockIdx.x * P.tiles_per_block, t_end = min(n_tiles, t_begin + P.tiles_per_block);
     if (t_begin >= t_end) return;
@@ -1111,6 +1133,37 @@
         else d = (unsigned)((long long)n * P.img_bytes_out) + (unsigned)P.base_off + (unsigned)r * (unsigned)P.row_bytes;
         pdst[(t & 3) * QT + tid] = q < P.m ? d : 0xffffffffu;
         if (EPI == QEPI_ROWS && P.n_frag_a) pdstb[(t & 3) * QT + tid] = q < P.m ? (unsigned)((long long)n * P.img_bytes_b) + (unsigned)P.base_off_b + (unsigned)r * (unsigned)P.row_bytes_b : 0xffffffffu;
+        if constexpr (DEC) pdstb[(t & 3) * QT + tid] = (unsigned)P.base_off + (unsigned)r * (unsigned)P.row_bytes;
+    };
+    auto decode_tile = [&](int tt) {
+#pragma clang fp contract(off)
+        const unsigned po = pdst[(tt & 3) * QT + lane], pb = pdstb[(tt & 3) * QT + lane];
+        float4 a4s[QDEC_AG];
+#pragma unroll
+        for (int da = 0; da < QDEC_AG; ++da)
+            a4s[da] = *reinterpret_cast<const float4 *>(P.anchors + 4 * (size_t)(pb + (unsigned)(blockIdx.y * P.dec_ag + min(da, P.dec_ag - 1))));
+#pragma unroll
+        for (int da = 0; da < QDEC_AG; ++da) {
+            if (da >= P.dec_ag) break;
+            unsigned *kp = &keymax[((tt & 1) * QT + lane) * QDEC_AG + da];
+            const unsigned key = *kp, bw = boxw[((tt & 1) * QT + lane) * QDEC_AG + da];
+            *kp = 0u;
+            const unsigned ai = (unsigned)(blockIdx.y * P.dec_ag + da);
+            const float4 a4 = a4s[da];
+            if (po == 0xffffffffu) continue;
+            const int best = (int)(key >> 8), bi = 255 - (int)(key & 255u);
+            float r[4], bx[4];
+            const float an[4] = {a4.x, a4.y, a4.z, a4.w};
+#pragma unroll
+            for (int q = 0; q < 4; ++q) r[q] = P.box_scale * ((float)((bw >> (8 * q)) & 255u) - P.box_zp);
+            (void)ssddev::decode_anchor(r, an, 0.f, bx);
+            const float sc = P.sc_scale * ((float)best - P.sc_zp);
+            const size_t o = (size_t)po + ai;
+            *reinterpret_cast<float4 *>(P.boxes + o * 4) = make_float4(bx[0], bx[1], bx[2], bx[3]);
+            P.score[o] = sc;
+            P.cls_out[o] = bi;
+            P.keys[o] = sc >= P.thr ? sc : -1.f;
+        }
     };
     auto fill = [&](int t) {
         const uint8_t *src = P.in + psrc[(t & 3) * QT + lane];
@@ -1145,6 +1198,10 @@
     };
     if (tid < QT) { geometry(t_begin); if (t_begin + 1 < t_end) geometry(t_begin + 1); }
     for (int i = tid; i < 3 * QT; i += blockDim.x) rowsum[i] = 0;
+    if constexpr (DEC) {
+        for (int i = tid; i < 2 * QT * QDEC_AG; i += blockDim.x) keymax[i] = 0u;
+        if (tid < 256) lut_s[tid] = P.lut[tid];
+    }
     __syncthreads();
     fill(t_begin);
     wait_landed(0);
@@ -1154,6 +1211,7 @@
     for (int t = t_begin; t < t_end; ++t) {
         __builtin_amdgcn_s_waitcnt(0xc07f);
         __builtin_amdgcn_s_barrier();
+        if (DEC && dec_wave && t > t_begin) decode_tile(t - 1);
         if (t + 1 < t_end) fill(t + 1);
         if (t + 2 < t_end && tid < QT) geometry(t + 2);
         const int slot1 = slot == 2 ? 0 : slot + 1, slot2 = slot1 == 2 ? 0 : slot1 + 1;
@@ -1203,6 +1261,29 @@
                     else *reinterpret_cast<uint2 *>(dst) = make_uint2(o[0], o[1]);
                 }
                 if (frag0 < P.n_mfrag) ++ns_prev;
+            } else if constexpr (DEC) {
+                const int rs0 = ROWSUM ? rowsum[slot * QT + 16 * f + fr] : 0;
+                unsigned *const kw = keymax + ((t & 1) * QT + 16 * f + fr) * QDEC_AG;
+                unsigned best = 0u;
+                int cur = -1;
+#pragma unroll
+                for (int m = 0; m < MW; ++m) {
+                    if (frag0 + m >= frag_end) continue;
+                    const int rv = rs0 * zwm[m];
+                    const unsigned wv = q_requant_linear_pack4(acc[m][0] + rv, acc[m][1] + rv, acc[m][2] + rv, acc[m][3] + rv, Mm[m], CQ[m][0], CQ[m][1], CQ[m][2], CQ[m][3], em[m], k1m[m]);
+                    if (hb[m]) {
+                        if (fq < P.dec_ag) boxw[((t & 1) * QT + 16 * f + fr) * QDEC_AG + fq] = wv;
+                        continue;
+                    }
+                    if (cur != agm[m]) {
+                        if (cur >= 0) atomicMax(kw + cur, best);
+                        best = 0u; cur = agm[m];
+                    }
+                    const int k0 = (int)lut_s[wv & 255u] << 8, k1 = ((int)lut_s[(wv >> 8) & 255u] << 8) - 1;
+                    const int k2 = ((int)lut_s[(wv >> 16) & 255u] << 8) - 2, k3 = ((int)lut_s[wv >> 24] << 8) - 3;
+                    best = max(best, (unsigned)(max(max(k0, k1), max(k2, k3)) + (255 - chm[m] - 4 * fq)));
+                }
+                if (cur >= 0) atomicMax(kw + cur, best);
             } else {
                 const int rs0 = ROWSUM ? rowsum[slot * QT + 16 * f + fr] : 0;
                 const unsigned pob = P.n_frag_a ? pdstb[(t & 3) * QT + 16 * f + fr] : 0xffffffffu;
@@ -1224,6 +1305,11 @@
         }
         slot = slot1;
     }
+    if constexpr (DEC) {
+        __builtin_amdgcn_s_waitcnt(0xc07f);
+        __builtin_amdgcn_s_barrier();
+        if (dec_wave) decode_tile(t_end - 1);
+    }
 }
 
 template <int K, int MW>
@@ -1233,7 +1319,8 @@
     const int groups = dd_ceil_div(P.n_mfrag, waves * MW);
     const int wpb = dd_ceil_div(dd_ceil_div(P.n_mfrag, groups), MW);
     P.frags_per_group = wpb * MW;
-    const size_t lds = (size_t)2 * QT * K + 15 * QT * sizeof(unsigned);
+    const bool dec = P.dec_ag != 0;
+    const size_t lds = (size_t)2 * QT * K + 15 * QT * sizeof(unsigned) + (dec ? 4 * QT * QDEC_AG * sizeof(unsigned) + 256 : 0);
     const int blocks_x = std::max(1, std::min(n_tiles, 256 / groups));
     P.tiles_per_block = dd_ceil_div(n_tiles, blocks_x);
     P.hw_magic = (unsigned)((1ull << 32) / (unsigned)P.hw) + 1u;
@@ -1251,18 +1338,23 @@
     const int sat = !rows && P.R.lo == 0 && P.R.hi == 255 ? (P.R.e <= 8 ? 2 : 1) : 0;
     void (*kern)(const QPwsP, const int) = nullptr;
 #define DD_PW(E_, R_, S_) q_pws_k<K, MW, E_, R_, S_>
-    if (rows) kern = rsum ? &DD_PW(QEPI_ROWS, true, 0) : &DD_PW(QEPI_ROWS, false, 0);
+    if (dec) {
+        if (!(rows && P.n_frag_a && groups * P.dec_gf == P.n_mfrag && wpb * MW >= P.dec_gf && P.dec_ag <= QDEC_AG)) { *ok = false; return DD_OK; }
+        kern = rsum ? &DD_PW(QEPI_DEC, true, 0) : &DD_PW(QEPI_DEC, false, 0);
+    } else if (rows) kern = rsum ? &DD_PW(QEPI_ROWS, true, 0) : &DD_PW(QEPI_ROWS, false, 0);
     else if constexpr (MW != 3) {
         if (sat == 2) kern = rsum ? &DD_PW(QEPI_Q16, true, 2) : &DD_PW(QEPI_Q16, false, 2);
         else if (sat == 1) kern = rsum ? &DD_PW(QEPI_Q16, true, 1) : &DD_PW(QEPI_Q16, false, 1);
         else kern = rsum ? &DD_PW(QEPI_Q16, true, 0) : &DD_PW(QEPI_Q16, false, 0);
     }
     if (!kern) { *ok = false; return DD_OK; }
-    *variant = QV_PWS | (K / 512) << 4 | MW << 6 | (rows ? QEPI_ROWS : QEPI_Q16) << 9 | (int)rsum << 11 | sat << 12 | (P.n_frag_a ? 1 : 0) << 14;
+    *variant = QV_PWS | (K / 512) << 4 | MW << 6 | (dec ? QEPI_DEC : rows ? QEPI_ROWS : QEPI_Q16) << 9 | (int)rsum << 11 | sat << 12 | (P.n_frag_a ? 1 : 0) << 14;
     static DevOnce once;
     const int rc = once.run(device, [&]() -> int {
         DD_HIP(hipFuncSetAttribute(reinterpret_cast<const void *>(&DD_PW(QEPI_ROWS, true, 0)), hipFuncAttributeMaxDynamicSharedMemorySize, 160 * 1024));
         DD_HIP(hipFuncSetAttribute(reinterpret_cast<const void *>(&DD_PW(QEPI_ROWS, false, 0)), hipFuncAttributeMaxDynamicSharedMemorySize, 160 * 1024));
+        DD_HIP(hipFuncSetAttribute(reinterpret_cast<const void *>(&DD_PW(QEPI_DEC, true, 0)), hipFuncAttributeMaxDynamicSharedMemorySize, 160 * 1024));
+        DD_HIP(hipFuncSetAttribute(reinterpret_cast<const void *>(&DD_PW(QEPI_DEC, false, 0)), hipFuncAttributeMaxDynamicSharedMemorySize, 160 * 1024));
         if constexpr (MW != 3) {
             for (const void *f : {reinterpret_cast<const void *>(&DD_PW(QEPI_Q16, true, 2)), reinterpret_cast<const void *>(&DD_PW(QEPI_Q16, false, 2)),
                                   reinterpret_cast<const void *>(&DD_PW(QEPI_Q16, true, 1)), reinterpret_cast<const void *>(&DD_PW(QEPI_Q16, false, 1)),
@@ -1321,6 +1413,19 @@
     if (rc != DD_OK) return rc;
     *fits_host = ok ? 1 : 0;
     return DD_OK;
+}
+
+static const int32_t *q_fused_decode_op(const dd_net *net, int i, const int32_t *o) {
+    const int cls_t = o[2], box_t = o[4];
+    const int32_t *dec = nullptr;
+    for (int k = 0; k < net->n_ops; ++k) {
+        const int32_t *u = net->prog.data() + net->ops_off + (size_t)k * DD_OP_WORDS;
+        if (u[0] == OP_QSSD_DECODE && u[1] == box_t && u[3] == cls_t) {
+            if (dec || k < i) return nullptr;
+            dec = u;
+        } else if (u[1] == cls_t || u[1] == box_t || u[3] == cls_t || u[3] == box_t) return nullptr;
+    }
+    return dec;
 }
 
 int netq_run_op(dd_net *net, int i, const int32_t *o, const uint8_t *input, int nimg, hipStream_t s, int *handled) {
@@ -1434,6 +1539,30 @@
                     Q.zwc_b = o[28]; Q.Rb = Rb;
                 }
                 bool ok = false;
+                const int32_t *dop = n_frag_a && o[29] > 0 && net->ssd_dec && net->q_dec_fuse && !net->q_heads_exposed ? q_fused_decode_op(net, i, o) : nullptr;
+                if (dop) {
+                    const TensorDesc *tb = &net->tensors[o[4]];
+                    const int a = o[23] / 4, ag = o[29], cls_row = a ? o[42] / a : 0, n_cls = dop[20], A = dop[21];
+                    const float *df = reinterpret_cast<const float *>(dop);
+                    if (a >= 1 && ag >= 1 && ag <= QDEC_AG && a % ag == 0 && cls_row % 16 == 0 && cls_row * a == o[42] && o[44] == o[42] && o[25] == o[23] && n_cls >= 2 && n_cls <= cls_row && dop[22] == 1 &&
+                        cls_row <= 240 && td->cs == cls_row && tb->cs == 4 && td->h == A && tb->h == A && td->w == 1 && tb->w == 1 && A == net->dec_anchors && o[43] == o[45] * cls_row &&
+                        o[24] == o[45] * 4 && o[45] >= 0 && (long long)o[45] + (long long)P.ho * P.wo * a <= A && (long long)nimg * A < (1ll << 32)) {
+                        QPwsP D = Q;
+                        D.dec_ag = ag; D.dec_fa = cls_row / 16; D.dec_gf = ag * D.dec_fa + 1; D.n_mfrag = a / ag * D.dec_gf; D.n_classes = n_cls;
+                        D.w = reinterpret_cast<const i4v *>(W + (size_t)(uint32_t)o[30]); D.cq = reinterpret_cast<const long long *>(W + (size_t)(uint32_t)o[31]);
+                        D.img_bytes_out = A; D.base_off = o[45]; D.row_bytes = a; D.img_bytes_b = 0;
+                        D.lut = reinterpret_cast<const uint8_t *>(W + (size_t)(uint32_t)dop[16]);
+                        D.box_scale = df[32]; D.box_zp = df[33]; D.sc_scale = df[34]; D.sc_zp = df[35]; D.thr = net->dec_thr;
+                        D.anchors = net->d_anchors; D.boxes = net->dec_boxes; D.score = net->dec_score; D.keys = net->dec_keys; D.cls_out = net->dec_cls;
+                        const int rcd = ts->cs == 512 ? (a == ag && dd_ceil_div(D.dec_gf, 3) <= 8 ? launch_q_pws<512, 3>(s, D, nimg, net->ctx->device, &ok, variant) : launch_q_pws<512, 4>(s, D, nimg, net->ctx->device, &ok, variant))
+                                                      : launch_q_pws<1024, 2>(s, D, nimg, net->ctx->device, &ok, variant);
+                        if (rcd != DD_OK) return rcd;
+                        if (ok) {
+                            if (i < (int)net->op_launch.size()) net->op_launch[i] = DD_OPK_Q_HEAD_DEC;
+                            return DD_OK;
+                        }
+                    }
+                }
                 const int rc = ts->cs == 512 ? (P.epi == QEPI_ROWS && (P.n_mfrag + 2) / 3 <= 8 && P.n_mfrag % 4 != 0 ? launch_q_pws<512, 3>(s, Q, nimg, net->ctx->device, &ok, variant) : launch_q_pws<512, 4>(s, Q, nimg, net->ctx->device, &ok, variant))
                                              : launch_q_pws<1024, 2>(s, Q, nimg, net->ctx->device, &ok, variant);
                 if (rc != DD_OK) return rc;
@@ -1607,9 +1736,25 @@
             P.box_scale = of[32]; P.box_zp = of[33]; P.sc_scale = of[34]; P.sc_zp = of[35]; P.thr = net->dec_thr;
             P.anchors = net->d_anchors; P.boxes = net->dec_boxes; P.score = net->dec_score; P.keys = net->dec_keys; P.cls_out = net->dec_cls;
             DD_REQUIRE(P.cls_stride % 16 == 0 && P.n_classes <= 128, DD_E_ARG, "dd_net_forward: uint8 decode: %d classes in rows of %d bytes", P.n_classes, P.cls_stride);
-            *variant = QV_DECODE;
-            hipLaunchKernelGGL(q_ssd_decode_k, dim3(dd_ceil_div(P.n_anchors * 8, 256), nimg), dim3(256), 0, s, P);
-            DD_LAUNCH_CHECK();
+            std::vector<char> done((size_t)P.n_anchors, 0);
+            for (int k = 0; k < i && k < (int)net->op_launch.size(); ++k) {
+                const int32_t *u = net->prog.data() + net->ops_off + (size_t)k * DD_OP_WORDS;
+                if (net->op_launch[k] != DD_OPK_Q_HEAD_DEC || u[0] != OP_QCONV || u[2] != o[3] || u[4] != o[1]) continue;
+                const long long b = u[45], e = b + (long long)u[26] * u[27] * (u[23] / 4);
+                DD_REQUIRE(b >= 0 && e <= P.n_anchors, DD_E_STATE, "dd_net_forward: uint8 decode: predictor op %d decoded anchors %lld .. %lld of %d", k, b, e, P.n_anchors);
+                std::fill(done.begin() + b, done.begin() + e, (char)1);
+            }
+            int launches = 0;
+            for (int a0 = 0; a0 < P.n_anchors;) {
+                if (done[a0]) { ++a0; continue; }
+                int a1 = a0;
+                while (a1 < P.n_anchors && !done[a1]) ++a1;
+                P.a_begin = a0; P.a_end = a1;
+                hipLaunchKernelGGL(q_ssd_decode_k, dim3(dd_ceil_div((a1 - a0) * 8, 256), nimg), dim3(256), 0, s, P);
+                DD_LAUNCH_CHECK();
+                ++launches; a0 = a1;
+            }
+            if (launches) *variant = QV_DECODE;
             return DD_OK;
         }
         default:
diff --git a/deepdish_amd/csrc/pipeline.hip b/deepdish_amd/csrc/pipeline.hip
--- a/deepdish_amd/csrc/pipeline.hip
+++ b/deepdish_amd/csrc/pipeline.hip
@@ -563,7 +563,8 @@
                                          p->det_in_w, p->d_tmp.as<uint8_t>(), S)) != DD_OK) return rc;
     if ((rc = dd_net_forward(p->det, p->d_resized.as<uint8_t>(), S, s)) != DD_OK) return rc;
     void *raw = nullptr;
-    if ((rc = dd_net_output(p->det, -1, &raw, nullptr, nullptr, nullptr, nullptr, nullptr)) != DD_OK) return rc;
+    const bool raw_unused = p->det_kind != DET_YOLOV5 && p->ssd_per_class <= 0 && p->ssd_dec;
+    if (!raw_unused && (rc = dd_net_output(p->det, -1, &raw, nullptr, nullptr, nullptr, nullptr, nullptr)) != DD_OK) return rc;
     if (p->det_kind == DET_YOLOV5) {
         const size_t cap = (size_t)p->n_anchors;
         float *yb = p->d_fin.as<float>(), *ys = yb + S * cap * 4;
diff --git a/deepdish_amd/engine.py b/deepdish_amd/engine.py
--- a/deepdish_amd/engine.py
+++ b/deepdish_amd/engine.py
@@ -4,7 +4,7 @@
 
 from ._lib import lib, check, P
 from .runtime import default_context, ptr
-from . import nets
+from . import nets, netsq
 
 
 class Net:
@@ -12,7 +12,7 @@
         self.ctx = context or default_context()
         self.program = program
         self.max_batch = int(max_batch)
-        words, blob = program.serialize()
+        words, blob = netsq.engine_image(program) if program.meta.get('quant') else program.serialize()
         self._words = words
         blob_arr = np.frombuffer(blob, dtype=np.uint8)
         h = P()
@@ -40,13 +40,13 @@
     def use_graph(self, enable=True):
         check(lib().dd_net_use_graph(self._h, int(bool(enable))), 'dd_net_use_graph')
 
-    def ssd_decode(self, anchors, score_thr, enable=True):
+    def ssd_decode(self, anchors, score_thr, enable=True, fused=True):
         if not enable:
             check(lib().dd_net_ssd_decode(self._h, None, 0, 0.0, 0), 'dd_net_ssd_decode')
             self._dec_anchors = 0
             return
         a = np.ascontiguousarray(anchors, dtype=np.float32)
-        check(lib().dd_net_ssd_decode(self._h, ptr(a), len(a), float(score_thr), int(bool(enable))), 'dd_net_ssd_decode')
+        check(lib().dd_net_ssd_decode(self._h, ptr(a), len(a), float(score_thr), 1 if fused else 2), 'dd_net_ssd_decode')
         self._dec_anchors = len(a) if enable else 0
 
     def ssd_heads_u8(self):
diff --git a/deepdish_amd/netsq.py b/deepdish_amd/netsq.py
--- a/deepdish_amd/netsq.py
+++ b/deepdish_amd/netsq.py
@@ -73,6 +73,36 @@
     return packed.astype(np.int8), cb.astype(np.int32), kcpt
 
 
+def head_groups(a, cls_row, cin, n_cls):
+    fa = cls_row // 16
+    max_frags = 16 if cin == 1024 else 32
+    ag = next((g for g in (4, 3, 2, 1) if a % g == 0 and g * fa + 1 <= max_frags), 0)
+    if cls_row % 16 or not ag:
+        return 0, np.zeros(0, np.int64)
+    gf = ag * fa + 1
+    rows = np.full((a // ag, gf * 16), -1, np.int64)
+    for g in range(a // ag):
+        for j in range(ag):
+            an = g * ag + j
+            rows[g, j * cls_row:j * cls_row + n_cls - 1] = an * cls_row + 1 + np.arange(n_cls - 1)
+            rows[g, ag * cls_row + 4 * j:ag * cls_row + 4 * j + 4] = a * cls_row + 4 * an + np.arange(4)
+    return ag, rows.reshape(-1)
+
+
+NO_ROW_ADDEND = -(1 << 58)
+
+
+def regroup_heads(packed, cq, rows):
+    n_mfrag, ksteps = packed.shape[:2]
+    by_row = np.transpose(packed.reshape(n_mfrag, ksteps, 4, 16, 16), (0, 3, 1, 2, 4)).reshape(n_mfrag * 16, ksteps, 4, 16)
+    out = np.zeros((len(rows),) + by_row.shape[1:], packed.dtype)
+    out[rows >= 0] = by_row[rows[rows >= 0]]
+    cq_out = np.full(len(rows), NO_ROW_ADDEND, cq.dtype)
+    cq_out[rows >= 0] = cq[rows[rows >= 0]]
+    w = np.transpose(out.reshape(len(rows) // 16, 16, ksteps, 4, 16), (0, 2, 3, 1, 4)).reshape(len(rows) // 16, ksteps, 64, 16)
+    return np.ascontiguousarray(w), cq_out
+
+
 def pack_conv0(L):
     def frags(w333o):
         src = np.transpose(w333o, (3, 0, 1, 2)).reshape(32, 3, 9)
@@ -159,6 +189,9 @@
     def __init__(self, P, model='uint8 SSD-MobileNet-v1', pad=False):
         self.P, self.model, self.pad = P, model, pad
         self.layer_t = {}
+        if not hasattr(P, 'dec_heads'):
+            P.dec_heads = []
+        self.dec_heads = P.dec_heads
 
     def need(self, cond, what):
         _model_need(cond, what, self.model)
@@ -230,8 +263,17 @@
         raw.update({38: 128 - int(Lc['w_zp']), 39: int(Lc['in_zp']), 42: cls_args['row_bytes'], 43: cls_args['base_off'], 44: cls_args['cout_store'],
                     46: P.add_blob(np.concatenate([lin(cbc, rc), lin(cbb, rb)])),
                     20: rb[32], 21: rb[33], 22: rb[40], 23: box_args['row_bytes'], 24: box_args['base_off'], 25: box_args['cout_store'], 28: 128 - int(Lb['w_zp'])})
+        w_all, cq_all = np.concatenate([wc, wb]), np.concatenate([lin(cbc, rc), lin(cbb, rb)])
+        a = box_args['row_bytes'] // 4
+        cls_row = cls_args['row_bytes'] // max(a, 1)
+        if (Lb['w'].shape[3] == 4 * a and len(cbc) == a * cls_row == cls_args['row_bytes'] == cls_args['cout_store'] and box_args['cout_store'] == 4 * a
+                and cls_args['base_off'] * 4 == box_args['base_off'] * cls_row and Lc['w'].shape[3] % a == 0 and Lc['w'].shape[3] // a >= 2):
+            ag, rows = head_groups(a, cls_row, s['c'], Lc['w'].shape[3] // a)
+            if ag:
+                w_dec, cq_dec = regroup_heads(w_all, cq_all, rows)
+                self.dec_heads.append(dict(op=len(P.ops), ag=ag, w=w_dec, cq=cq_dec, base=box_args['base_off'] // 4))
         P._op(OP_QCONV, src=src, dst=cls_args['dst'], dst2=box_args['dst'], kh=1, kw=1, stride=1, pad_t=pt, pad_l=pl, cin=s['c'], cout=Lc['w'].shape[3] + Lb['w'].shape[3],
-              cout_pad=len(cbc) + len(cbb), kpad=kcpt, act=len(cbc) // 16, epi=QEPI_ROWS, w_off=P.add_blob(np.concatenate([wc, wb])), b_off=P.add_blob(np.concatenate([cbc, cbb])),
+              cout_pad=len(cbc) + len(cbb), kpad=kcpt, act=len(cbc) // 16, epi=QEPI_ROWS, w_off=P.add_blob(w_all), b_off=P.add_blob(np.concatenate([cbc, cbb])),
               ho=ho, wo=wo, raw=raw)
         cin = s['c']
         cout = Lc['w'].shape[3] + Lb['w'].shape[3]
@@ -335,6 +377,31 @@
         P._op(OP_QSSD_DECODE, src=box_t, res=cls_t, w_off=P.add_blob(lut), p=[n_cls, n_anchors],
               rawf={32: float(Lb['out_scale']), 33: float(Lb['out_zp']), 34: float(logistic['out_scale']), 35: float(logistic['out_zp'])})
         self.info('q_ssd_decode_k', 0, n_anchors * (4 + cls_row + 24), 256)
+        self.dec_heads.append(dict(op=len(P.ops) - 1, lut_ok=int(lut[0] == lut.min())))
+
+
+def engine_image(program):
+    words, blob = program.serialize()
+    extra = getattr(program, 'dec_heads', None)
+    if not extra:
+        return words, blob
+    words, blob = words.copy(), bytearray(blob)
+    ops0 = len(words) - len(program.ops) * nets.OP_WORDS
+
+    def add(arr):
+        while len(blob) % 256:
+            blob.append(0)
+        off = len(blob)
+        blob.extend(np.ascontiguousarray(arr).tobytes())
+        return off
+
+    for e in extra:
+        o = words[ops0 + e['op'] * nets.OP_WORDS:ops0 + (e['op'] + 1) * nets.OP_WORDS]
+        if 'lut_ok' in e:
+            o[22] = e['lut_ok']
+        else:
+            o[29], o[30], o[31], o[45] = e['ag'], add(e['w']), add(e['cq']), e['base']
+    return words, bytes(blob)
 
 
 def compile_ssd_mobilenet_quant(qm):
diff --git a/deepdish_amd/profile.py b/deepdish_amd/profile.py
--- a/deepdish_amd/profile.py
+++ b/deepdish_amd/profile.py
@@ -25,7 +25,7 @@
 
 
 OPK_FOLDED = 1
-OPK_NAMES = {2: 'conv3x3_pool_rows_k', 3: 'conv3x3_pool_rows_k<STEM>', 4: 'res_unit_rows_k', 5: 'ssd_front_k', 6: 'conv3x3_c64_rows_k', 7: 'conv3x3_s2_rows_k', 8: 'conv_ws_k', 9: 'conv_ws_dw_k', 10: 'dwpw_rows_k', 11: 'conv_glds_k<ssd_head_decode>', 12: 'res_pair_rows_k', 13: 'conv_glds_k<yolo_head_decode>', 14: 'mars_ws128_k', 16: 'mars_pair64_k', 17: 'q_dwm_k', 18: 'conv3x3_c64_rows_k<strips>', 19: 'q_front_k', 20: 'q_mid_k', 21: 'q_conv_k<add>', 22: 'q_add_k', 23: 'stem_conv_pool_wide_k'}
+OPK_NAMES = {2: 'conv3x3_pool_rows_k', 3: 'conv3x3_pool_rows_k<STEM>', 4: 'res_unit_rows_k', 5: 'ssd_front_k', 6: 'conv3x3_c64_rows_k', 7: 'conv3x3_s2_rows_k', 8: 'conv_ws_k', 9: 'conv_ws_dw_k', 10: 'dwpw_rows_k', 11: 'conv_glds_k<ssd_head_decode>', 12: 'res_pair_rows_k', 13: 'conv_glds_k<yolo_head_decode>', 14: 'mars_ws128_k', 16: 'mars_pair64_k', 17: 'q_dwm_k', 18: 'conv3x3_c64_rows_k<strips>', 19: 'q_front_k', 20: 'q_mid_k', 21: 'q_conv_k<add>', 22: 'q_add_k', 23: 'stem_conv_pool_wide_k', 24: 'q_pws_k<ssd_decode>'}
 OPK_FOLDED_PREV = 15
 
 
@@ -55,7 +55,7 @@
 QDwpwV = collections.namedtuple('QDwpwV', 'kernel CIN COUT STRIDE QTT form SAT chunks')
 QConv0V = collections.namedtuple('QConv0V', 'kernel HL SAT chunks')
 QOtherV = collections.namedtuple('QOtherV', 'kernel chunks')
-Q_EPI_NAMES = {0: 'q16', 1: 'rows'}
+Q_EPI_NAMES = {0: 'q16', 1: 'rows', 3: 'decode'}
 Q_DWPW_FORMS = {0: 'plain', 1: 'rowsum', 2: 'hilo', 3: 'dup'}
 
 
```
